# Jingliang-Duan/DSAC-v2

Measured on AMD Instinct MI355X. Metric: DSAC-T gradient steps/sec, batch=256 Humanoid (obs376/act17), higher is better.
Workload: dtype f32

## Files before the change

### dsac-v2_amd/csrc/dsact_api.hip

```cpp
#include <hip/hip_runtime.h>
#include <hip/hip_ext.h>
#include <dlfcn.h>
#include <chrono>
#include <stdarg.h>
#include <stdio.h>
#include <math.h>
#include <stdlib.h>
#include <string.h>

#include <algorithm>
#include <atomic>
#include <string>
#include <vector>

#include "../../include/dsact.h"
#include "dsact_kernels.h"
#include "dsact_chain.h"
#include "dsact_fat.h"
#include "dsact_act.h"
#include "dsact_act_batch.h"
#include "dsact_host_act.h"
#include "dsact_conv.h"

#define DSACT_KERNEL(group, ...) extern template __global__ void __VA_ARGS__;
// ... 194 lines not shown
  int debug_withhold = 0;
  unsigned long long* act_out_host = nullptr; unsigned long long* act_out_dev = nullptr;
  unsigned long long* act_h = nullptr;
  int act_call = 0;
  double act_launch_us = 0.0, act_wait_us = 0.0;
  bool env_no_fast_act = false;
  bool host_act = true;
  float* pol_host = nullptr;
  hipEvent_t pol_ev = nullptr;
  bool pol_pending = false;
  unsigned long long pol_epoch = 1;
  unsigned long long pol_copied = 0;
  float* act_buf = nullptr;
  hostact::Pool* act_pool = nullptr;
  std::vector<int> act_pin;
  int act_cpu = -1;
  unsigned act_repins = 0;
  int act_threads = 0;
  float act_scale_h[32] = {0}, act_center_h[32] = {0};
  float act_lo_h[32] = {0}, act_hi_h[32] = {0};
  double act_host_us = 0.0, act_copy_wait_us = 0.0;
  float* ab_stage = nullptr; float* ab_in = nullptr; float* ab_h[2] = {nullptr, nullptr};
  float* ab_out_host = nullptr; float* ab_out_dev = nullptr;
  unsigned long long ab_calls = 0;
  unsigned long long ab_mode_calls = 0;
  uint64_t act_seed = 0;
  unsigned long long act_dev_calls = 0;
  unsigned long long ring_commit_rows = 0;
  unsigned long long* digest_dev = nullptr;
  unsigned long long act_dev_syncs = 0;
  int* ev_ep = nullptr; double* ev_acc = nullptr; int* ev_len = nullptr;
  double* ev_returns = nullptr; int* ev_lengths = nullptr;
  int* ev_remaining = nullptr;
  int* ev_remaining_host = nullptr;
  int ev_cap_n = 0, ev_cap_e = 0;
  int ev_n = 0, ev_e = 0;
  unsigned long long act_mode_dev_calls = 0;
  unsigned long long eval_commit_calls = 0, eval_polls = 0;
  unsigned char* tk_dev = nullptr; unsigned char* tk_host = nullptr;
  int tk_cap = 0, tk_n = 0;
  unsigned long long track_commit_calls = 0, track_reads = 0;
  int mode_host_rows = kModeHostRows;
  unsigned long long act_host_calls = 0, act_copies = 0;
  bool beh_held = false;
  float* beh_dev = nullptr;
  hipEvent_t beh_ev = nullptr;
  hipStream_t act_stream = nullptr;
  float* beh_host = nullptr;
  hipEvent_t beh_host_ev = nullptr;
  bool beh_host_pending = false;
  bool beh_host_ok = false;
  bool beh_live_copy = false;
  unsigned long long beh_holds = 0, beh_acts = 0;
  bool fwd_merge = false;
  bool pi_merge = false;
  float* zobs[4];
  float* dAq[4];
  bool twin = false;
  float* X0t_net[3] = {nullptr, nullptr, nullptr};
  float* dz0row[3] = {nullptr, nullptr, nullptr};
  float* twin_part[8];
  bool twin_par = false;
  bool env_twin_seq = false;
  bool twin_merged = false;
  PipeFwd* d_fwdt[2] = {nullptr, nullptr};
  PipeFwd* fwdt_host[2] = {nullptr, nullptr};
  float* doutT[3];
  int dw2_off[4] = {0, 0, 0, 0};
  int dw2_mid = 0;
  int n_heads_parts = 0;
  static constexpr int kPipePhases = 4;
  char* pipe_ws = nullptr;
  unsigned long long* pipe_hand[2] = {nullptr, nullptr};
  int* bqt_cnt = nullptr;
  int* bqt_tab = nullptr; int bqt_tab_blocks = 0;
  bool env_no_bqt = false;
  unsigned long long* bqp_pairs[2] = {nullptr, nullptr};
  bool env_no_bqp = false;
  struct GraphSet {
    hipGraph_t graph = nullptr; hipGraphExec_t exec = nullptr;
    hipGraph_t pgraph[kPipePhases] = {nullptr, nullptr, nullptr, nullptr};
    hipGraphExec_t pexec[kPipePhases] = {nullptr, nullptr, nullptr, nullptr};
    PipeFwd* pargs[kPipePhases] = {nullptr, nullptr, nullptr, nullptr};
    bool pipe = false;
    bool merged = false;
    bool noise_table = false;
    int steps = 0; uint32_t flags = 0;
    bool present() const { return exec != nullptr || pipe; }
  };
  GraphSet active;
  std::vector<GraphSet> graph_cache;
  bool env_no_pipe_defer = false;
  std::string env_pipe_map;
  void* comm = nullptr;
  int comm_rank = 0, comm_world = 1;
  bool use_std_sums = false;
  bool auto_std_sums = false;
  float* std_sums_own = nullptr;
};

extern "C" {
static int build_graph(dsact_handle* h, int steps_per_graph, uint32_t flags, bool noise_table, bool keep_cache);
}

namespace {


struct NcclUid { char internal[128]; };
struct RcclApi {
  void* lib = nullptr;
  int (*GetUniqueId)(NcclUid*) = nullptr;
  int (*CommInitRank)(void**, int, NcclUid, int) = nullptr;
  int (*AllReduce)(const void*, void*, size_t, int, int, void*, hipStream_t) = nullptr;
  int (*CommDestroy)(void*) = nullptr;
  const char* (*GetErrorString)(int) = nullptr;
};
RcclApi g_rccl;
constexpr int kNcclFloat = 7, kNcclSum = 0, kNcclAvg = 4;

const char* rccl_load(const char* path) {
  if (g_rccl.lib) return nullptr;
  const char* cand[3] = {path && path[0] ? path : "librccl.so", "librccl.so.1", "/opt/rocm/lib/librccl.so"};
  void* lib = nullptr;
  for (int i = 0; i < 3 && !lib; ++i) lib = dlopen(cand[i], RTLD_NOW | RTLD_GLOBAL);
  if (!lib) return "librccl.so not found";
  g_rccl.GetUniqueId = (int (*)(NcclUid*))dlsym(lib, "ncclGetUniqueId");
  g_rccl.CommInitRank = (int (*)(void**, int, NcclUid, int))dlsym(lib, "ncclCommInitRank");
  g_rccl.AllReduce = (int (*)(const void*, void*, size_t, int, int, void*, hipStream_t))dlsym(lib, "ncclAllReduce");
  g_rccl.CommDestroy = (int (*)(void*))dlsym(lib, "ncclCommDestroy");
  g_rccl.GetErrorString = (const char* (*)(int))dlsym(lib, "ncclGetErrorString");
  if (!g_rccl.GetUniqueId || !g_rccl.CommInitRank || !g_rccl.AllReduce || !g_rccl.CommDestroy) return "librccl.so lacks the nccl* entry points";
  g_rccl.lib = lib;
  return nullptr;
}
const char* rccl_err(int rc) { return g_rccl.GetErrorString ? g_rccl.GetErrorString(rc) : "rccl error"; }

int fail(dsact_handle* h, int code, const char* fmt, ...) {
  if (h) {
    va_list ap;
    va_start(ap, fmt);
    vsnprintf(h->err, sizeof(h->err), fmt, ap);
    va_end(ap);
  }
  return code;
}

#define HIPCHK(h, call)                                                                          \
  do {                                                                                           \
    hipError_t e_ = (call);                                                                      \
    if (e_ != hipSuccess) return fail(h, DSACT_E_HIP, "%s failed: %s (%s:%d)", #call, hipGetErrorString(e_), __FILE__, __LINE__); \
  } while (0)

void build_net(NetDesc& d, int in0, const int* hidden, int L, int n_out, int nblk, int n_conv, const ConvGeom* cg) {
  d.n_lin = L + 1;
  d.nblk = nblk;
  d.n_conv = n_conv;
  size_t off = 0;
  for (int j = 0; j < n_conv; ++j) {
    d.cw_off[j] = off; off += (size_t)cg[j].Cout * cg[j].K;
    d.cb_off[j] = off; off += cg[j].Cout;
  }
  int in = in0;
  for (int l = 0; l <= L; ++l) {
    const int out = l < L ? nblk * hidden[l] : n_out;
    d.in[l] = in; d.out[l] = out;
    d.w_off[l] = off;
    off += (nblk == 2 && l > 0 && l < L) ? (size_t)2 * (out / 2) * (in / 2) : (size_t)in * out;
    d.b_off[l] = off; off += out;
    in = out;
  }
  d.count = off;
}

int net_act(const dsact_handle* h, int net);
// ... 2227 lines not shown
    HeadsBwdArgs a;
    a.dZ1[0] = h->dZ[kDzSlot[C_Q1P]][0]; a.dZ1[1] = h->dZ[kDzSlot[C_Q2P]][0];
    a.W1aT[0] = h->W1aT[0]; a.W1aT[1] = h->W1aT[1]; a.W0 = h->wq[0];
    a.logits_pi = h->logits_pi; a.eps_new = h->eps_new; a.log_alpha = h->online + h->n_online - 1;
    a.Wout_pi = net_params(h, N_POL) + h->pd.w_off[Lp];
    a.G_pi = h->Gb[C_PI][Lp - 1]; a.dZ_pi = h->dZ[kDzSlot[C_PI]][Lp - 1];
    a.dout_pi = h->dout_pi; a.d_new_act = h->d_new_act;
    a.WL = h->wp[Lp - 1]; a.B = B; a.O = h->F; a.A = A;
    a.inv_B = 1.0f / (float)B; a.auto_alpha = h->cfg.auto_alpha; a.alpha_fixed = h->cfg.alpha_fixed;
    a.act_scale = h->act_scale; a.lo_ls = h->cfg.min_log_std; a.hi_ls = h->cfg.max_log_std;
    a.part_loss = h->part_loss; a.n_part = B; a.target_entropy = -(float)A;
    a.grad_log_alpha = h->grads + h->n_online - 1;
    a.pi_out_act = h->cfg.policy_out_act; a.pi_out_n = h->cfg.policy_std_param ? A : 2 * A;
    a.pi_dact = h->pi_dact;
    a.timeline = tl_for(h, "heads_bwd");
    a.n_row_blocks = (B + 3) / 4;
    a.extra = h->d_tiles; a.n_extra = 0;
    a.fo = fused_opt(h, fused);
    if (ride_hb > 0) { a.extra = h->d_tiles + h->dw_off[0]; a.n_extra = ride_hb; }
    const size_t hb_lds = a.n_extra ? tile_lds_bytes(dw_k(h)) : 0;
#define CALL_HBWD(N) TRY(launch(h, "heads_bwd", k_heads_bwd<N>, dim3(a.n_row_blocks + a.n_extra), dim3(kThreads), hb_lds, a))
    NCH_DISPATCH(a.WL, CALL_HBWD);
  }
  const size_t np = h->bwdpi.size();
  if (phase == PH_DP_ACTOR) {
    for (size_t i = 0; i < np; ++i) TRY(run_stage(h, h->bwdpi[i]));
    if (h->cnn) TRY(run_stage(h, h->dfeat_pi));
    TRY(run_dw(h, h->dw_off[2], h->dw_off[3], false, false));
    if (h->cnn) TRY(enqueue_conv_backward(h, 1, false, h->nq));
    TRY(sum_parts(h, (size_t)h->nq * h->n_q, h->n_online - 1));
    return DSACT_OK;
  }
  {
    int x = h->dw_off[0] + ride_hb;
    for (size_t i = 0; i < np; ++i) {
      const int left = ride_end - x;
      const int take = i + 1 == np ? left : left / (int)(np - i);
      TRY(run_stage(h, h->bwdpi[i], x, x + take, fused));
      x += take;
    }
    if (np == 0 && ride_hb) {  }
  }
  if (h->cnn) TRY(run_stage(h, h->dfeat_pi));
  if (h->dw_chunks == 1) {
    TRY(run_dw(h, np ? ride_end : h->dw_off[0] + ride_hb, h->dw_off[3], fused, fused));
    if (h->cnn) TRY(enqueue_conv_backward(h, h->nq + 1, fused));
  } else {
    TRY(run_dw(h, np ? ride_end : h->dw_off[0] + ride_hb, h->dw_off[3], false, false));
    if (h->cnn) TRY(enqueue_conv_backward(h, h->nq + 1, false));
    if (fused) TRY(enqueue_adam(h, true));
    else TRY(sum_parts(h, 0, h->n_online - 1));
  }
  return DSACT_OK;
}

int enqueue_adam(dsact_handle* h, bool from_parts) {
  AdamArgs a;
  memset(&a, 0, sizeof(a));
  if (from_parts && h->dw_chunks > 1) {
    a.part = h->dw_parts; a.part_stride = (long long)h->dw_part_stride; a.n_part = h->dw_chunks;
    const int nets[3] = {N_Q1, N_Q2, N_POL};
    for (int i = 0; i < 3; ++i) {
      const long long b = (long long)(net_grads(h, nets[i]) - h->grads);
      a.direct_lo[i] = b; a.direct_hi[i] = b + (long long)net_desc(h, nets[i]).w_off[0];
    }
  }
  a.p = h->online; a.tgt = h->target; a.m = h->adam_m; a.v = h->adam_v; a.g = h->grads;
  a.n_q2 = (long long)(h->nq * h->n_q); a.n_online3 = (long long)(h->nq * h->n_q + h->n_pi); a.n_total = (long long)h->n_online;
  a.st = h->st;
  a.b1w = (float)(1.0 - h->cfg.adam_beta1);
  a.beta2 = (float)h->cfg.adam_beta2;
  a.b2w = (float)(1.0 - h->cfg.adam_beta2);
  a.eps = h->cfg.adam_eps;
  const double polyak = 1.0 - h->cfg.tau;
  a.polyak = (float)polyak;
  a.one_minus_polyak = (float)(1.0 - polyak);
  a.auto_alpha = h->cfg.auto_alpha;
  a.commit_ms = h->have_local_tail ? 1 : 0;
  h->have_local_tail = false;
  const int blocks = (int)((h->n_online + kThreads * 8 - 1) / (kThreads * 8));
  return launch(h, "adam_polyak", k_adam, dim3(blocks), dim3(kThreads), 0, a);
}

static void destroy_graph_set(dsact_handle::GraphSet& g) {
  if (g.exec) hipGraphExecDestroy(g.exec);
  if (g.graph) hipGraphDestroy(g.graph);
  for (int p = 0; p < dsact_handle::kPipePhases; ++p) {
    if (g.pexec[p]) hipGraphExecDestroy(g.pexec[p]);
    if (g.pgraph[p]) hipGraphDestroy(g.pgraph[p]);
    if (g.pargs[p]) hipFree(g.pargs[p]);
  }
  g = dsact_handle::GraphSet();
}
static void stash_graph(dsact_handle* h) {
  if (!h->active.present()) return;
  h->graph_cache.push_back(h->active);
  h->active = dsact_handle::GraphSet();
}
static bool activate_graph(dsact_handle* h, int steps, uint32_t flags, bool noise_table) {
  for (size_t i = 0; i < h->graph_cache.size(); ++i) {
    const dsact_handle::GraphSet& g = h->graph_cache[i];
    if (g.steps != steps || g.flags != flags || g.noise_table != noise_table) continue;
    h->active = g;
    h->graph_cache.erase(h->graph_cache.begin() + (long)i);
    return true;
  }
  return false;
}
static void drop_active_graph(dsact_handle* h) { destroy_graph_set(h->active); }
void drop_graphs(dsact_handle* h) {
  destroy_graph_set(h->active);
  for (auto& g : h->graph_cache) destroy_graph_set(g);
  h->graph_cache.clear();
}
bool have_graph(const dsact_handle* h) { return h->active.present(); }
bool any_graph(const dsact_handle* h) { return have_graph(h) || !h->graph_cache.empty(); }

int check_handoff(dsact_handle* h) {
  volatile int* const w_upd = (volatile int*)h->handoff_host;
  volatile int* const w_act = w_upd ? w_upd + 1 : nullptr;
  if (!h->handoff_host || h->in_handoff || !(*w_upd | *w_act)) return DSACT_OK;
  h->in_handoff = true;
  const hipError_t e_dev = hipSetDevice(h->device);
  const hipError_t e_sync = hipStreamSynchronize(h->stream);
  const int upd = *w_upd;
  *w_upd = 0; *w_act = 0;
  if (!upd) {
    h->in_handoff = false;
    h->handoff_failures += 1;
    return fail(h, DSACT_E_HIP, "the acting forward's layer hand-over timed out (a wave waited > 0.1 s for its input): this "
                                "call's action is invalid; parameters and optimiser state are untouched%s%s",
                e_sync != hipSuccess ? "; HIP also reported: " : "", e_sync != hipSuccess ? hipGetErrorString(e_sync) : "");
  }
  const bool had_graph = have_graph(h);
  const int steps = had_graph ? h->active.steps : h->want_graph_steps;
  const uint32_t gflags = had_graph ? h->active.flags : h->want_graph_flags;
  const bool noise_tab = h->active.noise_table;
  h->fwd_merge = false;
  h->pi_merge = false;
  h->handoff_failures += 1;
  drop_graphs(h);
  int twin_rc = DSACT_OK;
  if (h->twin_par) {
    h->env_twin_seq = true;
    h->debug_withhold = 0;
    twin_rc = build_twin_fwd(h);
  }
  hipError_t e_set = hipSuccess;
  if (h->chain_flags) e_set = hipMemset(h->chain_flags, 0, kChainFlagInts * sizeof(int));
  h->flags_dirty = false;
  int rebuilt = DSACT_E_STATE;
  const bool wanted = had_graph || steps > 0;
  if (wanted && twin_rc == DSACT_OK) {
    h->state_invalid = false;
    rebuilt = build_graph(h, steps, gflags, noise_tab, false);
  }
  h->want_graph_steps = (wanted && rebuilt != DSACT_OK) ? steps : 0;
  h->want_graph_flags = gflags;
  h->in_handoff = false;
  h->state_invalid = true;
  const hipError_t e_hip = e_dev != hipSuccess ? e_dev : e_sync != hipSuccess ? e_sync : e_set;
  return fail(h, DSACT_E_HIP,
              "an in-launch hand-over timed out: a workgroup waited > 0.1 s for its producers' ready flags, so every result "
              "since the last successful call is invalid -- parameters, optimiser moments and targets included: restore them, "
              "then acknowledge with dsact_set_state(adam_steps, mean_std), dsact_debug_set(\"ack_state\") or dsact_bind_arenas "
              "(update entry points fail until then). Merged launches are now disabled for this handle%s%s%s",
              wanted ? (rebuilt == DSACT_OK ? "; the graph was captured again without them" : "; re-capturing the graph failed (it is built again by the next replay)")
                     : "",
              e_hip != hipSuccess ? "; HIP also reported: " : "", e_hip != hipSuccess ? hipGetErrorString(e_hip) : "");
}

static int ensure_wanted_graph(dsact_handle* h) {
  if (have_graph(h) || h->want_graph_steps <= 0) return DSACT_OK;
  const int steps = h->want_graph_steps;
  h->want_graph_steps = 0;
  return dsact_graph_build(h, steps, h->want_graph_flags);
}

bool has_ring(const dsact_handle* h) { return h->rb_act != nullptr; }

int check_codes(dsact_handle* h) {
  if (!h->miss_host || !*(volatile int*)h->miss_host) return DSACT_OK;
  if (!h->miss_seen) {
    HIPCHK(h, hipSetDevice(h->device));
    HIPCHK(h, hipStreamSynchronize(h->stream));
    HIPCHK(h, hipMemcpy(&h->miss_rec, h->code_miss, sizeof(CodeMiss), hipMemcpyDeviceToHost));
    h->miss_seen = true;
  }
  uint32_t bits = h->miss_rec.bits;
  float v;
  memcpy(&v, &bits, 4);
  return fail(h, DSACT_E_INVALID, "hip_obs_codebook: %llu observation value(s) written to the coded ring are not in the codebook; "
              "first recorded: %.9g (bits 0x%08x) at ring row %lld -- the ring holds wrong codes for them",
              h->miss_rec.count, (double)v, bits, h->miss_rec.row);
}

static int check_usable(dsact_handle* h) {
  if (!h) return DSACT_E_INVALID;
  TRY(check_handoff(h));
  TRY(check_codes(h));
  if (h->state_invalid)
    return fail(h, DSACT_E_STATE, "device state is invalid after a hand-over timeout: restore parameters / optimiser state, then "
                                  "call dsact_set_state or dsact_bind_arenas");
  return DSACT_OK;
}
// ... 63 lines not shown
  if (cfg->act_dist != 0 && cfg->act_dist != 1) return fail(h, DSACT_E_INVALID, "act_dist must be 0 (TanhGaussDistribution) or 1 (GaussDistribution)");
  if (cfg->policy_std_param != 0 && cfg->policy_std_param != 1) return fail(h, DSACT_E_INVALID, "policy_std_param must be 0 (mlp_shared) or 1 (parameter)");
  if (cfg->policy_std_param && (cfg->conv_type != DSACT_CONV_NONE || cfg->algo != 0))
    return fail(h, DSACT_E_INVALID, "policy_std_type 'parameter' is built for DSAC_V2 with MLP nets");
  if (cfg->policy_twin != 0 && cfg->policy_twin != 1) return fail(h, DSACT_E_INVALID, "policy_twin must be 0 or 1 (policy_std_type mlp_separated)");
  if (cfg->policy_twin && (cfg->conv_type != DSACT_CONV_NONE || cfg->algo != 0 || cfg->policy_std_param))
    return fail(h, DSACT_E_INVALID, "policy_std_type 'mlp_separated' is built for DSAC_V2 with MLP nets (and excludes 'parameter')");
  for (int oa : {cfg->value_out_act, cfg->policy_out_act})
    if (oa != 0 && (oa < ACT_RELU || oa > ACT_TANH) && oa != OUT_ACT_GELU)
      return fail(h, DSACT_E_INVALID, "output activation must be 0 (linear), 1..5 (relu, elu, selu, sigmoid, tanh) or 6 (gelu)");
  if ((cfg->value_out_act || cfg->policy_out_act) && (cfg->conv_type != DSACT_CONV_NONE || cfg->algo != 0))
    return fail(h, DSACT_E_INVALID, "output activations other than linear are built for DSAC_V2 with MLP nets (tile-stage kernels)");
  if (h->cfg.global_batch < h->cfg.batch) h->cfg.global_batch = h->cfg.batch;
  HIPCHK(h, hipSetDevice(device));
  h->O = cfg->obs_dim; h->A = cfg->act_dim; h->L = cfg->n_hidden; h->B = cfg->batch;
  h->F = h->O;
  h->Brows = h->B > kActRows ? h->B : kActRows;
  int nblk = 1;
  if (cfg->conv_type != DSACT_CONV_NONE) {
    static const int k1[] = {8, 4, 3}, c1[] = {32, 64, 64}, s1[] = {4, 2, 1};
    static const int k2[] = {4, 3, 3, 3, 3, 3}, c2[] = {8, 16, 32, 64, 128, 256}, s2[] = {2, 2, 2, 2, 1, 1};
    if (cfg->conv_type != DSACT_CONV_TYPE_1 && cfg->conv_type != DSACT_CONV_TYPE_2) return fail(h, DSACT_E_INVALID, "conv_type must be 0, 1 (type_1) or 2 (type_2)");
    const bool t1 = cfg->conv_type == DSACT_CONV_TYPE_1;
    const int* ks = t1 ? k1 : k2; const int* cs = t1 ? c1 : c2; const int* ss = t1 ? s1 : s2;
    h->n_conv = t1 ? 3 : 6;
    if (cfg->img_c < 1 || cfg->img_h < 1 || cfg->img_w < 1 || (long long)cfg->img_c * cfg->img_h * cfg->img_w != cfg->obs_dim)
      return fail(h, DSACT_E_INVALID, "obs_dim must equal img_c*img_h*img_w for CNN nets");
    if (cfg->obs_dim % 4) return fail(h, DSACT_E_INVALID, "img_c*img_h*img_w must be a multiple of 4");
    int C = cfg->img_c, H = cfg->img_h, W = cfg->img_w;
    for (int j = 0; j < h->n_conv; ++j) {
      ConvGeom& g = h->cg[j];
      g.H = H; g.W = W; g.Cin = C; g.KS = ks[j]; g.stride = ss[j]; g.Cout = cs[j];
      g.OH = (H - g.KS) / g.stride + 1; g.OW = (W - g.KS) / g.stride + 1;
      if (H < g.KS || W < g.KS || g.OH < 1 || g.OW < 1) return fail(h, DSACT_E_INVALID, "image %dx%d too small for conv layer %d", cfg->img_h, cfg->img_w, j);
      g.K = g.KS * g.KS * g.Cin; g.KWC = g.KS * g.Cin; g.rowskip = g.W * g.Cin - g.KWC;
      g.inv_kwc = 1.0f / (float)g.KWC;
      if (g.KWC % 4) return fail(h, DSACT_E_INVALID, "kernel_width*channels of conv layer %d must be a multiple of 4 (got %d)", j, g.KWC);
      C = g.Cout; H = g.OH; W = g.OW;
    }
    h->cnn = true;
    h->cP = H * W;
    h->F = C * H * W;
    nblk = 2;
  }
  int pol_hidden[DSACT_MAX_HIDDEN_LAYERS] = {0};
  bool unequal = false;
  h->Lq = cfg->n_hidden;
  h->Lp = cfg->policy_n_hidden > 0 ? cfg->policy_n_hidden : cfg->n_hidden;
  if (h->Lp > DSACT_MAX_HIDDEN_LAYERS) return fail(h, DSACT_E_INVALID, "policy_n_hidden must be 0 (= n_hidden) or 1..%d", DSACT_MAX_HIDDEN_LAYERS);
  if (h->Lp != h->Lq && cfg->conv_type != DSACT_CONV_NONE) return fail(h, DSACT_E_INVALID, "policy_n_hidden: the CNN nets' MLP widths are fixed by conv_type");
  unequal = h->Lp != h->Lq;
  h->L = h->Lp > h->Lq ? h->Lp : h->Lq;
  for (int l = 0; l < h->Lp; ++l) {
    pol_hidden[l] = cfg->policy_hidden[l] > 0 ? cfg->policy_hidden[l] : (l < h->Lq ? cfg->hidden[l] : 0);
    if (pol_hidden[l] < 1 || pol_hidden[l] > kMaxWidth) return fail(h, DSACT_E_INVALID, "policy hidden width of layer %d must be 1..%d", l, kMaxWidth);
    unequal = unequal || l >= h->Lq || pol_hidden[l] != cfg->hidden[l];
  }
  if (unequal && (cfg->conv_type != DSACT_CONV_NONE || cfg->algo != 0))
    return fail(h, DSACT_E_INVALID, "value_hidden_sizes != policy_hidden_sizes is built for DSAC_V2 with MLP nets (tile-stage kernels)");
  const int nblk_pol = cfg->policy_twin ? 2 : nblk;
  h->unequal_widths = unequal || nblk_pol != nblk;
  for (int l = 0; l < h->L; ++l) {
    h->wq[l] = l < h->Lq ? nblk * cfg->hidden[l] : 0; h->wp[l] = l < h->Lp ? nblk_pol * pol_hidden[l] : 0;
    h->w[l] = h->wq[l] > h->wp[l] ? h->wq[l] : h->wp[l];
  }
  for (int l = 0; l < h->L; ++l)
    if (h->w[l] > kMaxWidth) return fail(h, DSACT_E_INVALID, "activation row width %d exceeds %d", h->w[l], kMaxWidth);
  h->ldx = (h->F + h->A + 3) & ~3;
  h->use_w1p = (size_t)4 * nblk * cfg->hidden[0] * h->ldx <= ((size_t)4 << 20);
  build_net(h->qd, h->F + h->A, cfg->hidden, h->Lq, 2, nblk, h->n_conv, h->cg);
  build_net(h->pd, h->F, pol_hidden, h->Lp, 2 * h->A, nblk_pol, h->n_conv, h->cg);
  h->n_q = h->qd.count; h->n_pi = h->pd.count;
  if (cfg->algo != DSACT_ALGO_DSAC_V2 && cfg->algo != DSACT_ALGO_DSAC_V1) return fail(h, DSACT_E_INVALID, "algo must be 0 (DSAC_V2) or 1 (DSAC_V1)");
  h->nq = cfg->algo == DSACT_ALGO_DSAC_V1 ? 1 : 2;
  h->n_online = h->nq * h->n_q + h->n_pi + 1;
  h->n_target = h->nq * h->n_q + h->n_pi;
  h->n_heads_wg = (h->B + 3) / 4;
  h->n_loss_wg = (h->B + 3) / 4;
  h->loss_rows = 4;
  h->auto_std_sums = h->B > 1024;
  if (const char* v = getenv("DSACT_TIMELINE_STAGE")) h->env_timeline_stage = v;
  { int v = 0; if (hipDeviceGetAttribute(&v, hipDeviceAttributeMultiprocessorCount, h->device) == hipSuccess && v > 0) h->n_cu = v; (void)hipGetLastError(); }
  h->env_no_pipe_defer = getenv("DSACT_NO_PIPE_DEFER") != nullptr;
  h->env_no_bqt = getenv("DSACT_NO_BQT_MERGE") != nullptr;
  h->env_no_bqp = getenv("DSACT_NO_BQP_MERGE") != nullptr;
  if (const char* v = getenv("DSACT_PIPE_MAP")) h->env_pipe_map = v;
  h->env_no_dcol_ident = getenv("DSACT_NO_DCOL_IDENT") != nullptr;
  h->env_no_fat_stage = getenv("DSACT_NO_FAT_STAGE") != nullptr;
  h->dw_chunks = (h->B > 448 && h->B % 256 == 0) ? h->B / 256 : 1;
  h->dw_part_stride = (h->n_online + 2 + 63) & ~(size_t)63;
  {
    const int R = 4 * h->cRG;
    bool ok = h->B % R == 0 && h->B % 16 == 0 && (h->B <= 256 || h->B % 256 == 0) &&
              getenv("DSACT_NO_CHAIN") == nullptr && !(h->nq == 1 && getenv("DSACT_NO_CHAIN_V1") != nullptr) &&
              !(h->cnn && (getenv("DSACT_NO_CHAIN_CNN") != nullptr || h->B > 1024));
    ok = ok && h->L <= kChMaxL;
    ok = ok && !h->unequal_widths;
    ok = ok && cfg->value_out_act != OUT_ACT_GELU && cfg->policy_out_act != OUT_ACT_GELU;
    for (int l = 0; l < h->L; ++l) ok = ok && cfg->hidden[l] == cfg->hidden[0];
    const int W0 = cfg->hidden[0];
    ok = ok && (W0 == 64 || W0 == 128 || W0 == 256);
    h->s_obs = roundup((h->F + 3) / 4, kPD);
    h->s_act = roundup((h->A + 3) / 4, kPD);
    h->SoT = roundup((2 * h->A + 3) / 4, kPD);
    ok = ok && (size_t)chain_lds(4 * (h->s_obs + h->s_act), W0, R).total * sizeof(float) <= 150 * 1024;
    h->chain_ok = ok;
    h->twin = ok && h->cnn;
    h->env_twin_seq = getenv("DSACT_TWIN_SEQ") != nullptr;
    if (ok) {
      const int per = (h->B > 1024 && h->B % 1024 == 0) ? 1024 : 256;
      h->dw_chunks = h->B > 1024 ? h->B / per : 1;
    }
    h->cW = W0; h->cNT = W0 / 64; h->n_slices = h->B / R;
    h->rg4_ok = ok && h->B % 16 == 0 &&
                (size_t)chain_lds(4 * (h->s_obs + h->s_act), W0, 16).total * sizeof(float) <= 150 * 1024;
    h->c_obs = (h->F + 15) / 16; h->c_act = (h->A + 15) / 16; h->c_out = (2 * h->A + 15) / 16;
    {
      const char* fm = getenv("DSACT_FAT_MIN");
      const int fat_min = fm ? atoi(fm) : 1024;
      h->fat = ok && !h->cnn && h->nq == 2 && h->B >= fat_min && h->B % 32 == 0 && (W0 == 128 || W0 == 256) &&
               cfg->value_out_act == 0 && cfg->policy_out_act == 0;
      h->fat_bwd = h->fat && h->B >= 4096;
      if (const char* v = getenv("DSACT_FAT_RT")) h->env_fat_rt = atoi(v) == 2 ? 2 : 1;
    }
    h->fwd_merge = ok && !h->cnn && h->B <= 256 && h->B / 4 <= kChainFlagSlices && chain_rg(h, 4) == 1 && getenv("DSACT_NO_FWD_MERGE") == nullptr;
    h->pi_merge = ok && !h->cnn && h->B <= 512 && !h->fat_bwd && getenv("DSACT_NO_PI_MERGE") == nullptr;
  }
  Carver c0;
  carve(h, c0, h->sets[0], SET_WS);
  h->ws_bytes = c0.off + 256;
  HIPCHK(h, hipMalloc(&h->ws, h->ws_bytes));
  HIPCHK(h, hipMemset(h->ws, 0, h->ws_bytes));
  Carver c1;
  c1.base = h->ws;
  carve(h, c1, h->sets[0], SET_WS);
  {
    DevState st0;
    memset(&st0, 0, sizeof(st0));
    st0.b1p_q = st0.b2p_q = st0.b1p_pi = st0.b2p_pi = st0.b1p_alpha = st0.b2p_alpha = 1.0;
    HIPCHK(h, hipMemcpy(h->st, &st0, sizeof(st0), hipMemcpyHostToDevice));
  }
  {
    std::vector<float> ones(h->B, 1.0f);
    HIPCHK(h, hipMemcpy(h->ones, ones.data(), h->B * sizeof(float), hipMemcpyHostToDevice));
  }
  if (h->cnn) {
    for (int j = 0; j < h->n_conv; ++j) {
      const ConvGeom& g = h->cg[j];
      if ((size_t)h->Brows * g.H * g.W * g.Cin > 2147483647ull || (size_t)h->Brows * g.OH * g.OW >= (1u << 24))
        return fail(h, DSACT_E_INVALID, "batch x image too large for the conv index arithmetic (layer %d)", j);
    }
    std::vector<int> iota(h->Brows);
    for (int i = 0; i < h->Brows; ++i) iota[i] = i;
    HIPCHK(h, hipMemcpy(h->idx_iota, iota.data(), iota.size() * sizeof(int), hipMemcpyHostToDevice));
  }
  HIPCHK(h, hipStreamCreateWithFlags(&h->stream, hipStreamNonBlocking));
  h->own_stream = true;
  {
    const int max_lds = (int)tile_lds_bytes(BK * kMaxPrefetchTiles);
    HIPCHK(h, hipFuncSetAttribute((const void*)k_stage<false, false, EPI_GELU>, hipFuncAttributeMaxDynamicSharedMemorySize, max_lds));
    HIPCHK(h, hipFuncSetAttribute((const void*)k_stage<false, false, EPI_GELU, 4>, hipFuncAttributeMaxDynamicSharedMemorySize, max_lds));
    HIPCHK(h, hipFuncSetAttribute((const void*)k_stage<false, false, EPI_GELU, 2>, hipFuncAttributeMaxDynamicSharedMemorySize, max_lds));
    HIPCHK(h, hipFuncSetAttribute((const void*)k_stage<false, true, EPI_MULG, 4>, hipFuncAttributeMaxDynamicSharedMemorySize, max_lds));
    HIPCHK(h, hipFuncSetAttribute((const void*)k_stage<false, true, EPI_MULG, 2>, hipFuncAttributeMaxDynamicSharedMemorySize, max_lds));
    HIPCHK(h, hipFuncSetAttribute((const void*)k_stage<false, true, EPI_MULG>, hipFuncAttributeMaxDynamicSharedMemorySize, max_lds));
    HIPCHK(h, hipFuncSetAttribute((const void*)k_stage_table, hipFuncAttributeMaxDynamicSharedMemorySize, max_lds));
// ... 82 lines not shown
    const size_t la = (size_t)chain_lds(4 * (h->s_obs + h->s_act), h->cW, 4 * chain_rg(h, 6)).total * sizeof(float);
    const void* fn = h->cNT == 1 ? (const void*)k_chain_fwd2<1> : h->cNT == 2 ? (const void*)k_chain_fwd2<2> : (const void*)k_chain_fwd2<4>;
    if (hipOccupancyMaxActiveBlocksPerMultiprocessor(&per_cu, fn, 64 * h->cNT, la) != hipSuccess || per_cu < 2) h->fwd_merge = false;
    (void)hipGetLastError();
  }
  for (int i = 0; i < 8; ++i) {
    HIPCHK(h, hipHostMalloc((void**)&h->h_idx[i], (size_t)h->B * sizeof(int), hipHostMallocDefault));
    HIPCHK(h, hipEventCreateWithFlags(&h->h_idx_ev[i], hipEventDisableTiming));
  }
  return DSACT_OK;
}

int dsact_destroy(dsact_handle* h) {
  if (!h) return DSACT_E_INVALID;
  hipSetDevice(h->device);
  if (h->stream) hipStreamSynchronize(h->stream);
  drop_graphs(h);
  if (h->comm && g_rccl.CommDestroy) { g_rccl.CommDestroy(h->comm); h->comm = nullptr; }
  for (auto& r : h->prof) { hipEventDestroy(r.e0); hipEventDestroy(r.e1); }
  if (h->tev0) { hipEventDestroy(h->tev0); hipEventDestroy(h->tev1); }
  if (h->uev0) { hipEventDestroy(h->uev0); hipEventDestroy(h->uev1); }
  for (int i = 0; i < 8; ++i) {
    if (h->h_idx[i]) hipHostFree(h->h_idx[i]);
    if (h->h_idx_ev[i]) hipEventDestroy(h->h_idx_ev[i]);
  }
  if (h->handoff_host) hipHostFree(h->handoff_host);
  if (h->act_h) hipFree(h->act_h);
  if (h->ab_stage) hipHostFree(h->ab_stage);
  if (h->ab_out_host) hipHostFree(h->ab_out_host);
  if (h->ab_in) hipFree(h->ab_in);
  for (void* p : {(void*)h->ev_ep, (void*)h->ev_acc, (void*)h->ev_len, (void*)h->ev_returns, (void*)h->ev_lengths, (void*)h->ev_remaining})
    if (p) hipFree(p);
  if (h->ev_remaining_host) hipHostFree(h->ev_remaining_host);
  if (h->tk_dev) hipFree(h->tk_dev);
  if (h->digest_dev) hipFree(h->digest_dev);
  if (h->tk_host) hipHostFree(h->tk_host);
  for (int i = 0; i < 2; ++i) if (h->ab_h[i]) hipFree(h->ab_h[i]);
  if (h->pol_host) hipHostFree(h->pol_host);
  if (h->pol_ev) hipEventDestroy(h->pol_ev);
  if (h->act_stream) { hipStreamSynchronize(h->act_stream); hipStreamDestroy(h->act_stream); }
  if (h->beh_dev) hipFree(h->beh_dev);
  if (h->beh_host) hipHostFree(h->beh_host);
  if (h->beh_ev) hipEventDestroy(h->beh_ev);
  if (h->beh_host_ev) hipEventDestroy(h->beh_host_ev);
  free(h->act_buf);
  delete h->act_pool;
  for (int k : {0, (int)dsact_handle::kAltSet}) if (h->sets[k].d_tiles) hipFree(h->sets[k].d_tiles);
  if (h->alt_ws) hipFree(h->alt_ws);
  if (h->pipe_ws) hipFree(h->pipe_ws);
  if (h->bqt_cnt) hipFree(h->bqt_cnt);
  if (h->bqt_tab) hipFree(h->bqt_tab);
  for (int i = 0; i < 2; ++i) if (h->bqp_pairs[i]) hipFree(h->bqp_pairs[i]);
  if (h->pk_ws) hipFree(h->pk_ws);
  for (int i = 0; i < 2; ++i) { if (h->d_fwdt[i]) hipFree(h->d_fwdt[i]); delete h->fwdt_host[i]; }
  if (h->d_mir) hipFree(h->d_mir);
  if (h->d_apjobs) hipFree(h->d_apjobs);
  if (h->d_pack) hipFree(h->d_pack);
  if (h->idx_table) hipFree(h->idx_table);
  if (h->noise_table) hipFree(h->noise_table);
  for (int i = 0; i < 4; ++i) {
    if (h->grp_pin[i]) hipHostFree(h->grp_pin[i]);
    if (h->grp_ev[i]) hipEventDestroy(h->grp_ev[i]);
  }
  if (h->stage_dev) hipFree(h->stage_dev);
  for (int i = 0; i < 2; ++i) {
    if (h->stage_pin[i]) hipHostFree(h->stage_pin[i]);
    if (h->stage_ev[i]) hipEventDestroy(h->stage_ev[i]);
  }
  if (h->logp_stage) hipFree(h->logp_stage);
  if (h->stage_img) hipFree(h->stage_img);
  for (float* p : {h->rb_obs, h->rb_obs2, h->rb_act, h->rb_rew, h->rb_done, h->rb_logp})
    if (p) hipFree(p);
  if (h->rb_code) hipFree(h->rb_code);
  if (h->code_book) hipFree(h->code_book);
  if (h->code_miss) hipFree(h->code_miss);
  if (h->miss_host) hipHostFree(h->miss_host);
  if (h->ws) hipFree(h->ws);
  if (h->own_stream && h->stream) hipStreamDestroy(h->stream);
  delete h;
  return DSACT_OK;
}

int dsact_set_stream(dsact_handle* h, void* s) {
  if (!h) return DSACT_E_INVALID;
  HIPCHK(h, hipSetDevice(h->device));
  if (any_graph(h)) return fail(h, DSACT_E_STATE, "cannot change stream after dsact_graph_build");
  if (h->stream) HIPCHK(h, hipStreamSynchronize(h->stream));
  if (h->own_stream && h->stream) { hipStreamDestroy(h->stream); h->stream = nullptr; }
  if (s) { h->stream = (hipStream_t)s; h->own_stream = false; }
  else { HIPCHK(h, hipStreamCreateWithFlags(&h->stream, hipStreamNonBlocking)); h->own_stream = true; }
  return DSACT_OK;
}

void* dsact_get_stream(const dsact_handle* h) { return h ? (void*)h->stream : nullptr; }

int dsact_sync(dsact_handle* h) {
  if (!h) return DSACT_E_INVALID;
  HIPCHK(h, hipSetDevice(h->device));
  HIPCHK(h, hipStreamSynchronize(h->stream));
  return check_handoff(h);
}

size_t dsact_online_count(const dsact_handle* h) { return h ? h->n_online : 0; }
size_t dsact_target_count(const dsact_handle* h) { return h ? h->n_target : 0; }
size_t dsact_q_count(const dsact_handle* h) { return h ? h->n_q : 0; }
size_t dsact_pi_count(const dsact_handle* h) { return h ? h->n_pi : 0; }

int dsact_bind_arenas(dsact_handle* h, float* online, float* target, float* adam_m, float* adam_v, float* grads) {
  if (!h) return DSACT_E_INVALID;
  if (!online || !target || !adam_m || !adam_v || !grads) return fail(h, DSACT_E_INVALID, "null arena pointer");
  HIPCHK(h, hipSetDevice(h->device));
  if (any_graph(h)) return fail(h, DSACT_E_STATE, "cannot rebind arenas after dsact_graph_build");
  h->online = online; h->target = target; h->adam_m = adam_m; h->adam_v = adam_v; h->grads = grads;
  TRY(build_chain(h));
  TRY(build_pack_jobs(h));
  if (h->chain_ok && !h->twin) TRY(build_adam_pack_jobs(h));
  TRY(build_tasks(h));
  if (h->twin) TRY(build_twin_fwd(h));
  if (h->chain_ok) (void)dw2_args(h, false);
  if (!h->cnn) {
    TRY(alloc_alt_set(h));
    select_set(h, dsact_handle::kAltSet);
    int rc = build_tasks(h);
    select_set(h, 0);
    TRY(rc);
  }
  h->state_invalid = false;
  h->pol_epoch++;
  return DSACT_OK;
}

int dsact_set_action_limits(dsact_handle* h, const float* high, const float* low) {
  if (!h || !high || !low) return DSACT_E_INVALID;
  HIPCHK(h, hipSetDevice(h->device));
  std::vector<float> s(h->A), c(h->A);
  for (int j = 0; j < h->A; ++j) {
    if (!(high[j] > low[j])) return fail(h, DSACT_E_INVALID, "action_high_limit must exceed action_low_limit");
    s[j] = (high[j] - low[j]) / 2;
    c[j] = (high[j] + low[j]) / 2;
    if (h->cfg.act_dist == 1) { s[j] = 0.0f; c[j] = 0.0f; }
  }
  HIPCHK(h, hipStreamSynchronize(h->stream));
  HIPCHK(h, hipMemcpy(h->act_scale, s.data(), h->A * sizeof(float), hipMemcpyHostToDevice));
  HIPCHK(h, hipMemcpy(h->act_center, c.data(), h->A * sizeof(float), hipMemcpyHostToDevice));
  HIPCHK(h, hipMemcpy(h->act_lo, low, h->A * sizeof(float), hipMemcpyHostToDevice));
  HIPCHK(h, hipMemcpy(h->act_hi, high, h->A * sizeof(float), hipMemcpyHostToDevice));
  for (int j = 0; j < h->A && j < 32; ++j) {
    h->act_scale_h[j] = s[j]; h->act_center_h[j] = c[j];
    h->act_lo_h[j] = low[j]; h->act_hi_h[j] = high[j];
  }
  h->limits_set = true;
  return DSACT_OK;
}

int dsact_get_state(dsact_handle* h, int32_t adam_steps[3], float mean_std[2]) {
  if (!h) return DSACT_E_INVALID;
  HIPCHK(h, hipSetDevice(h->device));
  HIPCHK(h, hipStreamSynchronize(h->stream));
  DevState st;
  HIPCHK(h, hipMemcpy(&st, h->st, sizeof(st), hipMemcpyDeviceToHost));
  TRY(check_handoff(h));
  if (adam_steps) { adam_steps[0] = st.t_q; adam_steps[1] = st.t_pi; adam_steps[2] = st.t_alpha; }
  if (mean_std) { mean_std[0] = st.ms_init ? st.ms1 : -1.0f; mean_std[1] = st.ms_init ? st.ms2 : -1.0f; }
  return DSACT_OK;
}

int dsact_set_state(dsact_handle* h, const int32_t adam_steps[3], const float mean_std[2]) {
  if (!h) return DSACT_E_INVALID;
  HIPCHK(h, hipSetDevice(h->device));
  HIPCHK(h, hipStreamSynchronize(h->stream));
  DevState st;
  HIPCHK(h, hipMemcpy(&st, h->st, sizeof(st), hipMemcpyDeviceToHost));
  if (adam_steps) {
    st.t_q = adam_steps[0]; st.t_pi = adam_steps[1]; st.t_alpha = adam_steps[2];
    const double b1 = h->cfg.adam_beta1, b2 = h->cfg.adam_beta2;
    st.b1p_q = pow(b1, st.t_q); st.b2p_q = pow(b2, st.t_q);
    st.b1p_pi = pow(b1, st.t_pi); st.b2p_pi = pow(b2, st.t_pi);
    st.b1p_alpha = pow(b1, st.t_alpha); st.b2p_alpha = pow(b2, st.t_alpha);
  }
  if (mean_std) {
    st.ms_init = (mean_std[0] >= 0.0f && mean_std[1] >= 0.0f) ? 1 : 0;
    st.ms1 = mean_std[0]; st.ms2 = mean_std[1];
  }
  HIPCHK(h, hipMemcpy(h->st, &st, sizeof(st), hipMemcpyHostToDevice));
  if (adam_steps && mean_std) h->state_invalid = false;
  return DSACT_OK;
}

int dsact_set_hyper(dsact_handle* h, int32_t which, double value) {
  if (!h) return DSACT_E_INVALID;
  if (!(value == value)) return fail(h, DSACT_E_INVALID, "hyper-parameter is NaN");
  switch (which) {
    case DSACT_HYPER_GAMMA: h->cfg.gamma = value; break;
    case DSACT_HYPER_TAU:
      if (value < 0.0 || value > 1.0) return fail(h, DSACT_E_INVALID, "tau outside [0, 1]");
      h->cfg.tau = value; break;
    case DSACT_HYPER_TAU_B:
      if (value < 0.0 || value > 1.0) return fail(h, DSACT_E_INVALID, "tau_b outside [0, 1]");
      h->cfg.tau_b = value; break;
    case DSACT_HYPER_AUTO_ALPHA: h->cfg.auto_alpha = value != 0.0 ? 1 : 0; break;
    case DSACT_HYPER_ALPHA: h->cfg.alpha_fixed = value; break;
    case DSACT_HYPER_DELAY_UPDATE:
      if (value < 1.0 || value != (double)(int32_t)value) return fail(h, DSACT_E_INVALID, "delay_update must be a positive integer");
      h->cfg.delay_update = (int32_t)value; break;
    case DSACT_HYPER_TD_BOUND:
      if (h->cfg.algo != 1) return fail(h, DSACT_E_INVALID, "TD_bound is a DSAC_V1 parameter");
      h->cfg.td_bound = value; break;
    case DSACT_HYPER_V1_BOUND:
      if (h->cfg.algo != 1) return fail(h, DSACT_E_INVALID, "bound is a DSAC_V1 parameter");
      h->cfg.v1_unbounded = value != 0.0 ? 0 : 1; break;
    default: return fail(h, DSACT_E_INVALID, "unknown hyper-parameter %d", (int)which);
  }
  HIPCHK(h, hipSetDevice(h->device));
  HIPCHK(h, hipStreamSynchronize(h->stream));
  drop_graphs(h);
  return DSACT_OK;
}

namespace {
int create_scalar_columns(dsact_handle* h, int64_t capacity) {
  const size_t N = (size_t)capacity;
  HIPCHK(h, hipMalloc(&h->rb_act, N * h->A * sizeof(float)));
  HIPCHK(h, hipMalloc(&h->rb_rew, N * sizeof(float)));
  HIPCHK(h, hipMalloc(&h->rb_done, N * sizeof(float)));
  HIPCHK(h, hipMalloc(&h->rb_logp, N * sizeof(float)));
  HIPCHK(h, hipMemsetAsync(h->rb_act, 0, N * h->A * sizeof(float), h->stream));
  HIPCHK(h, hipMemsetAsync(h->rb_rew, 0, N * sizeof(float), h->stream));
  HIPCHK(h, hipMemsetAsync(h->rb_done, 0, N * sizeof(float), h->stream));
  HIPCHK(h, hipMemsetAsync(h->rb_logp, 0, N * sizeof(float), h->stream));
  h->cap = capacity; h->ptr = 0; h->size = 0;
  return DSACT_OK;
}
}

int dsact_buffer_create(dsact_handle* h, int64_t capacity) {
  if (!h || capacity < 1) return DSACT_E_INVALID;
  if (capacity > 2147483647LL) return fail(h, DSACT_E_INVALID, "capacity must fit int32 (device indices)");
  HIPCHK(h, hipSetDevice(h->device));
  if (has_ring(h)) return fail(h, DSACT_E_STATE, "buffer already created");
  const size_t N = (size_t)capacity;
  HIPCHK(h, hipMalloc(&h->rb_obs, N * h->O * sizeof(float)));
  HIPCHK(h, hipMalloc(&h->rb_obs2, N * h->O * sizeof(float)));
  HIPCHK(h, hipMemsetAsync(h->rb_obs, 0, N * h->O * sizeof(float), h->stream));
  HIPCHK(h, hipMemsetAsync(h->rb_obs2, 0, N * h->O * sizeof(float), h->stream));
  return create_scalar_columns(h, capacity);
}

int dsact_buffer_create_coded(dsact_handle* h, int64_t capacity, const float* codebook, int32_t n_codes) {
  if (!h || capacity < 1 || !codebook) return DSACT_E_INVALID;
  if (capacity > 2147483647LL) return fail(h, DSACT_E_INVALID, "capacity must fit int32 (device indices)");
  if (n_codes < 1 || n_codes > 256) return fail(h, DSACT_E_INVALID, "hip_obs_codebook: %d entries (1 .. 256)", (int)n_codes);
  for (int i = 0; i < n_codes; ++i) {
    if (!(codebook[i] == codebook[i])) return fail(h, DSACT_E_INVALID, "hip_obs_codebook: entry %d is NaN", i);
    if (i && !(codebook[i - 1] < codebook[i]))
      return fail(h, DSACT_E_INVALID, "hip_obs_codebook: entries %d, %d are not strictly ascending (%.9g, %.9g)", i - 1, i,
                  (double)codebook[i - 1], (double)codebook[i]);
  }
  if (!h->cnn) return fail(h, DSACT_E_INVALID, "hip_obs_codebook: codes are for image observations (C, H, W); this handle has flat ones");
  const int C = h->cfg.img_c, HW = h->cfg.img_h * h->cfg.img_w;
  if (HW % 16 || C > 16)
    return fail(h, DSACT_E_INVALID, "hip_obs_codebook: a coded ring needs H * W %% 16 == 0 and C <= 16 (got C %d, H * W %d)", C, HW);
  HIPCHK(h, hipSetDevice(h->device));
  if (has_ring(h)) return fail(h, DSACT_E_STATE, "buffer already created");
  const size_t N = (size_t)capacity, O = (size_t)h->O;
  HIPCHK(h, hipMalloc(&h->rb_code, 2 * N * O));
  HIPCHK(h, hipMemsetAsync(h->rb_code, 0, 2 * N * O, h->stream));
  float book[256] = {};
  memcpy(book, codebook, (size_t)n_codes * sizeof(float));
  HIPCHK(h, hipMalloc(&h->code_book, sizeof(book)));
  HIPCHK(h, hipMemcpy(h->code_book, book, sizeof(book), hipMemcpyHostToDevice));
  h->n_codes = n_codes;
  HIPCHK(h, hipMalloc(&h->code_miss, sizeof(CodeMiss)));
  HIPCHK(h, hipMemset(h->code_miss, 0, sizeof(CodeMiss)));
  HIPCHK(h, hipHostMalloc((void**)&h->miss_host, 64, hipHostMallocMapped | hipHostMallocCoherent));
  *(volatile int*)h->miss_host = 0;
  HIPCHK(h, hipHostGetDevicePointer((void**)&h->miss_dev, h->miss_host, 0));
  if (coded_gather_lds(C) > 64 * 1024)
    HIPCHK(h, hipFuncSetAttribute((const void*)k_gather_img_coded<0>, hipFuncAttributeMaxDynamicSharedMemorySize, (int)coded_gather_lds(C)));
  return create_scalar_columns(h, capacity);
}

int dsact_buffer_check(dsact_handle* h) {
  if (!h) return DSACT_E_INVALID;
  if (!has_ring(h)) return fail(h, DSACT_E_STATE, "buffer not created");
  HIPCHK(h, hipSetDevice(h->device));
  HIPCHK(h, hipStreamSynchronize(h->stream));
  return check_codes(h);
}

int64_t dsact_buffer_bytes(const dsact_handle* h) {
  if (!h) return -1;
  if (!has_ring(h)) return 0;
  const int64_t O = h->O, A = h->A;
  const int64_t obs_bytes = h->rb_code ? 2 * O : 4 * 2 * O;
  return h->cap * (obs_bytes + 4 * (A + 3));
}

int64_t dsact_buffer_size(const dsact_handle* h) { return h ? h->size : -1; }
int64_t dsact_buffer_ptr(const dsact_handle* h) { return h ? h->ptr : -1; }

namespace {
int enqueue_ring_encode(dsact_handle* h, const float* s_obs, const float* s_obs2, long long ptr, long long n) {
  CodedScatterArgs e;
  e.s_obs = s_obs; e.s_obs2 = s_obs2;
  e.code0 = h->rb_code; e.code1 = h->rb_code + (size_t)h->cap * h->O;
  e.book = h->code_book; e.n_codes = h->n_codes; e.miss = h->code_miss; e.miss_flag = h->miss_dev;
  e.ptr = ptr; e.cap = h->cap; e.n = (int)n; e.O = h->O;
  e.wide = (h->O % 4 == 0) && ((uintptr_t)s_obs % 16 == 0) && ((uintptr_t)s_obs2 % 16 == 0);
  const long long per_row = e.wide ? h->O / 4 : h->O;
  const unsigned gx = (unsigned)std::min<long long>((per_row + kThreads - 1) / kThreads, 64);
  const unsigned rows = (unsigned)(n < 65535 ? n : 65535);
  return launch(h, "ring_write_img_coded", k_ring_write_img_coded, dim3(gx, rows, 2), dim3(kThreads), 0, e);
}
}

int dsact_buffer_add(dsact_handle* h, int64_t n, const float* obs, const float* act, const float* rew,
                     const float* obs2, const float* done, const float* logp) {
  if (!h || n < 0 || !obs || !act || !rew || !obs2 || !done) return DSACT_E_INVALID;
  if (!has_ring(h)) return fail(h, DSACT_E_STATE, "buffer not created");
  TRY(check_codes(h));
  if (n == 0) return DSACT_OK;
  HIPCHK(h, hipSetDevice(h->device));
  const size_t O = h->O, A = h->A;
  const size_t row_f = 2 * O + A + 3;
  if ((size_t)n > h->stage_rows) {
    HIPCHK(h, hipStreamSynchronize(h->stream));
    if (h->stage_dev) hipFree(h->stage_dev);
    for (int i = 0; i < 2; ++i)
      if (h->stage_pin[i]) { hipHostFree(h->stage_pin[i]); h->stage_pin[i] = nullptr; }
    h->stage_rows = (size_t)n < 64 ? 64 : (size_t)n;
    HIPCHK(h, hipMalloc(&h->stage_dev, h->stage_rows * row_f * sizeof(float)));
    for (int i = 0; i < 2; ++i) {
      HIPCHK(h, hipHostMalloc((void**)&h->stage_pin[i], h->stage_rows * row_f * sizeof(float), hipHostMallocDefault));
      if (!h->stage_ev[i]) HIPCHK(h, hipEventCreateWithFlags(&h->stage_ev[i], hipEventDisableTiming));
    }
  }
  const int slot = (int)(h->stage_k++ & 1);
  HIPCHK(h, hipEventSynchronize(h->stage_ev[slot]));
  float* pin = h->stage_pin[slot];
  size_t off = 0;
  auto put = [&](const float* src, size_t count) {
    if (src) memcpy(pin + off, src, count * sizeof(float));
    off += count;
  };
  put(obs, (size_t)n * O); put(obs2, (size_t)n * O); put(act, (size_t)n * A); put(rew, (size_t)n); put(done, (size_t)n);
  put(logp, (size_t)n);
  const size_t R = (size_t)n;
  float* s_obs = h->stage_dev;
  float* s_obs2 = s_obs + R * O;
  float* s_act = s_obs2 + R * O;
  float* s_rew = s_act + R * A;
  float* s_done = s_rew + R;
  float* s_logp = s_done + R;
  HIPCHK(h, hipMemcpyAsync(h->stage_dev, pin, off * sizeof(float), hipMemcpyHostToDevice, h->stream));
  HIPCHK(h, hipEventRecord(h->stage_ev[slot], h->stream));
  long long first = 0, cnt = n;
  if (n > h->cap) { first = n - h->cap; cnt = h->cap; }
  ScatterArgs a;
  a.s_obs = s_obs + first * O; a.s_obs2 = s_obs2 + first * O; a.s_act = s_act + first * A;
  a.s_rew = s_rew + first; a.s_done = s_done + first; a.s_logp = logp ? s_logp + first : nullptr;
  a.rb_obs = h->rb_obs; a.rb_obs2 = h->rb_obs2; a.rb_act = h->rb_act; a.rb_rew = h->rb_rew; a.rb_done = h->rb_done; a.rb_logp = h->rb_logp;
  a.ptr = (h->ptr + first) % h->cap; a.cap = h->cap; a.n = (int)cnt; a.O = h->O; a.A = h->A;
  if (h->rb_code) {
    TRY(enqueue_ring_encode(h, a.s_obs, a.s_obs2, a.ptr, cnt));
    a.O = 0;
  } else if (h->cnn) {
    ImgScatterArgs w;
    w.s_obs = a.s_obs; w.s_obs2 = a.s_obs2; w.rb_obs = h->rb_obs; w.rb_obs2 = h->rb_obs2;
    w.ptr = a.ptr; w.cap = h->cap; w.n = (int)cnt; w.O = h->O;
    TRY(launch(h, "ring_write_img", k_ring_write_img, dim3(8, (unsigned)cnt), dim3(kThreads), 0, w));
    a.O = 0;
  }
  TRY(launch(h, "ring_write", k_ring_write, dim3((unsigned)((cnt + 3) / 4)), dim3(kThreads), 0, a));
  h->ptr = (h->ptr + n) % h->cap;
  h->size = h->size + n > h->cap ? h->cap : h->size + n;
  return DSACT_OK;
}

int dsact_buffer_fill_device(dsact_handle* h, int64_t row0, int64_t n, const float* obs, const float* act,
                             const float* rew, const float* obs2, const float* done) {
  if (!h || row0 < 0 || n < 0) return DSACT_E_INVALID;
  if (!has_ring(h)) return fail(h, DSACT_E_STATE, "buffer not created");
  if (row0 + n > h->cap) return fail(h, DSACT_E_INVALID, "fill exceeds capacity");
  TRY(check_codes(h));
  HIPCHK(h, hipSetDevice(h->device));
  const size_t O = h->O, A = h->A;
  if (h->rb_code) {
    if (n > 0) TRY(enqueue_ring_encode(h, obs, obs2, row0, n));
  } else {
    HIPCHK(h, hipMemcpyAsync(h->rb_obs + row0 * O, obs, n * O * sizeof(float), hipMemcpyDeviceToDevice, h->stream));
    HIPCHK(h, hipMemcpyAsync(h->rb_obs2 + row0 * O, obs2, n * O * sizeof(float), hipMemcpyDeviceToDevice, h->stream));
  }
  HIPCHK(h, hipMemcpyAsync(h->rb_act + row0 * A, act, n * A * sizeof(float), hipMemcpyDeviceToDevice, h->stream));
  HIPCHK(h, hipMemcpyAsync(h->rb_rew + row0, rew, n * sizeof(float), hipMemcpyDeviceToDevice, h->stream));
  HIPCHK(h, hipMemcpyAsync(h->rb_done + row0, done, n * sizeof(float), hipMemcpyDeviceToDevice, h->stream));
  HIPCHK(h, hipStreamSynchronize(h->stream));
  if (row0 + n > h->size) h->size = row0 + n;
  h->ptr = (row0 + n) % h->cap;
  return check_codes(h);
}

static bool on_handle_gpu(const dsact_handle* h, const void* p) {
  hipPointerAttribute_t at;
  if (hipPointerGetAttributes(&at, p) != hipSuccess) { (void)hipGetLastError(); return false; }
  return at.type == hipMemoryTypeDevice && at.device == h->device;
}
static int check_handoff_counted(dsact_handle* h) {
  const unsigned long long before = h->handoff_failures;
  const int rc = check_handoff(h);
  if (h->handoff_failures != before) h->act_dev_syncs++;
  return rc;
}

int dsact_buffer_add_device(dsact_handle* h, int64_t n, const float* obs, const float* act, const float* rew, const float* obs2,
                            const uint8_t* terminated, const uint8_t* truncated, const float* logp, double reward_scale) {
  if (!h || n < 0 || !obs || !act || !rew || !obs2 || !terminated || !truncated || !logp) return DSACT_E_INVALID;
  if (!has_ring(h)) return fail(h, DSACT_E_STATE, "buffer not created");
  if (h->rb_code) return fail(h, DSACT_E_INVALID, "dsact_buffer_add_device serves the fp32 MLP ring (coded rings: dsact_buffer_add)");
  if (h->cnn) return fail(h, DSACT_E_INVALID, "dsact_buffer_add_device serves the fp32 MLP ring (image rings: dsact_buffer_add)");
  if (n > h->cap) return fail(h, DSACT_E_INVALID, "dsact_buffer_add_device: n = %lld exceeds the capacity %lld", (long long)n, (long long)h->cap);
  if (n == 0) return DSACT_OK;
  HIPCHK(h, hipSetDevice(h->device));
  const void* ptrs[7] = {obs, act, rew, obs2, terminated, truncated, logp};
  for (const void* p : ptrs)
    if (!on_handle_gpu(h, p))
      return fail(h, DSACT_E_INVALID, "dsact_buffer_add_device takes device pointers on the handle's GPU (host rows: dsact_buffer_add)");
  TRY(check_handoff_counted(h));
  RingCommitArgs a;
  a.s_obs = obs; a.s_act = act; a.s_rew = rew; a.s_obs2 = obs2; a.s_term = terminated; a.s_trunc = truncated; a.s_logp = logp;
  a.rb_obs = h->rb_obs; a.rb_obs2 = h->rb_obs2; a.rb_act = h->rb_act; a.rb_rew = h->rb_rew; a.rb_done = h->rb_done; a.rb_logp = h->rb_logp;
  a.ptr = h->ptr; a.cap = h->cap; a.n = (int)n; a.O = h->O; a.A = h->A;
  a.wide = (h->O % 4 == 0) && ((uintptr_t)obs % 16 == 0) && ((uintptr_t)obs2 % 16 == 0) && ((uintptr_t)h->rb_obs % 16 == 0) &&
           ((uintptr_t)h->rb_obs2 % 16 == 0);
  a.reward_scale = (float)reward_scale;
  TRY(launch(h, "ring_commit", k_ring_commit, dim3((unsigned)((n + 3) / 4)), dim3(kThreads), 0, a));
  h->ptr = (h->ptr + n) % h->cap;
  h->size = h->size + n > h->cap ? h->cap : h->size + n;
  h->ring_commit_rows += (unsigned long long)n;
  return DSACT_OK;
}

namespace {
struct RingColumn { char* base; size_t row_bytes; };
void ring_columns(const dsact_handle* h, RingColumn c[6]) {
  const size_t O = (size_t)h->O, A = (size_t)h->A;
  if (h->rb_code) {
    c[0] = {(char*)h->rb_code, O};
    c[1] = {(char*)h->rb_code + (size_t)h->cap * O, O};
  } else {
    c[0] = {(char*)h->rb_obs, O * sizeof(float)};
    c[1] = {(char*)h->rb_obs2, O * sizeof(float)};
  }
  c[2] = {(char*)h->rb_act, A * sizeof(float)};
  c[3] = {(char*)h->rb_rew, sizeof(float)};
  c[4] = {(char*)h->rb_done, sizeof(float)};
  c[5] = {(char*)h->rb_logp, sizeof(float)};
}
int ring_entry(dsact_handle* h, const char* what) {
  if (!has_ring(h)) return fail(h, DSACT_E_STATE, "%s: buffer not created", what);
  hipStreamCaptureStatus cap = hipStreamCaptureStatusNone;
  HIPCHK(h, hipStreamIsCapturing(h->stream, &cap));
  if (cap != hipStreamCaptureStatusNone) return fail(h, DSACT_E_STATE, "%s under stream capture", what);
  return DSACT_OK;
}
int ring_drain(dsact_handle* h) {
  HIPCHK(h, hipSetDevice(h->device));
  TRY(check_handoff(h));
  HIPCHK(h, hipStreamSynchronize(h->stream));
  TRY(check_handoff(h));
  return check_codes(h);
}
}

int dsact_buffer_export(dsact_handle* h, int64_t row0, int64_t n, void* obs, void* obs2, float* act, float* rew, float* done,
                        float* logp) {
  if (!h) return DSACT_E_INVALID;
  TRY(ring_entry(h, "dsact_buffer_export"));
  if (row0 < 0 || n < 0 || row0 > h->size || n > h->size - row0)
    return fail(h, DSACT_E_INVALID, "dsact_buffer_export: rows [%lld, %lld + %lld) are not inside the %lld live rows", (long long)row0,
                (long long)row0, (long long)n, h->size);
  TRY(ring_drain(h));
  if (n == 0) return DSACT_OK;
  RingColumn c[6];
  ring_columns(h, c);
  void* dst[6] = {obs, obs2, act, rew, done, logp};
  for (int k = 0; k < 6; ++k)
    if (dst[k]) HIPCHK(h, hipMemcpy(dst[k], c[k].base + (size_t)row0 * c[k].row_bytes, (size_t)n * c[k].row_bytes, hipMemcpyDeviceToHost));
  return DSACT_OK;
}

int dsact_buffer_import(dsact_handle* h, int64_t row0, int64_t n, const void* obs, const void* obs2, const float* act,
                        const float* rew, const float* done, const float* logp) {
  if (!h) return DSACT_E_INVALID;
  TRY(ring_entry(h, "dsact_buffer_import"));
  if (!obs || !obs2 || !act || !rew || !done || !logp) return fail(h, DSACT_E_INVALID, "dsact_buffer_import: a source column is NULL");
  if (row0 < 0 || n < 0 || row0 > h->cap || n > h->cap - row0)
    return fail(h, DSACT_E_INVALID, "dsact_buffer_import: rows [%lld, %lld + %lld) are not inside the capacity %lld", (long long)row0,
                (long long)row0, (long long)n, h->cap);
  if (h->rb_code && h->n_codes < 256) {
    const size_t cnt = (size_t)n * (size_t)h->O;
    const unsigned char* src[2] = {(const unsigned char*)obs, (const unsigned char*)obs2};
    for (int w = 0; w < 2; ++w)
      for (size_t i = 0; i < cnt; ++i)
        if (src[w][i] >= h->n_codes)
          return fail(h, DSACT_E_INVALID, "dsact_buffer_import: %s code %d at row %lld, element %lld is not below the codebook's %d entries",
                      w ? "obs2" : "obs", (int)src[w][i], (long long)(row0 + (int64_t)(i / (size_t)h->O)), (long long)(i % (size_t)h->O), h->n_codes);
  }
  TRY(ring_drain(h));
  if (n == 0) return DSACT_OK;
  RingColumn c[6];
  ring_columns(h, c);
  const void* src[6] = {obs, obs2, act, rew, done, logp};
  for (int k = 0; k < 6; ++k)
    HIPCHK(h, hipMemcpy(c[k].base + (size_t)row0 * c[k].row_bytes, src[k], (size_t)n * c[k].row_bytes, hipMemcpyHostToDevice));
  return DSACT_OK;
}

int dsact_buffer_set_cursor(dsact_handle* h, int64_t size, int64_t ptr) {
  if (!h) return DSACT_E_INVALID;
  TRY(ring_entry(h, "dsact_buffer_set_cursor"));
  const bool ok = size >= 0 && size <= h->cap && (size < h->cap ? ptr == size % h->cap : (ptr >= 0 && ptr < h->cap));
  if (!ok)
    return fail(h, DSACT_E_INVALID, "dsact_buffer_set_cursor: (size %lld, ptr %lld) is no state a ring of %lld rows reaches", (long long)size,
                (long long)ptr, h->cap);
  TRY(ring_drain(h));
  h->size = size; h->ptr = ptr;
  return DSACT_OK;
}

int dsact_buffer_digest(dsact_handle* h, int64_t row0, int64_t n, uint64_t out[6]) {
  if (!h) return DSACT_E_INVALID;
  TRY(ring_entry(h, "dsact_buffer_digest"));
  if (!out) return fail(h, DSACT_E_INVALID, "dsact_buffer_digest: out is NULL");
  if (row0 < 0 || n < 0 || row0 > h->size || n > h->size - row0)
    return fail(h, DSACT_E_INVALID, "dsact_buffer_digest: rows [%lld, %lld + %lld) are not inside the %lld live rows", (long long)row0,
                (long long)row0, (long long)n, h->size);
  TRY(ring_drain(h));
  for (int k = 0; k < 6; ++k) out[k] = 0;
  if (n == 0) return DSACT_OK;
  if (!h->digest_dev) HIPCHK(h, hipMalloc(&h->digest_dev, 6 * sizeof(unsigned long long)));
  RingColumn c[6];
  ring_columns(h, c);
  RingDigestArgs a;
  unsigned long long most = 0;
  for (int k = 0; k < 6; ++k) {
    const int eb = (k < 2 && h->rb_code) ? 1 : 4;
    const unsigned long long w = (unsigned long long)(c[k].row_bytes / (size_t)eb);
    a.col[k].base = c[k].base;
    a.col[k].g0 = (unsigned long long)row0 * w;
    a.col[k].count = (unsigned long long)n * w;
    a.col[k].elem_bytes = eb;
    const unsigned long long loads = a.col[k].count / (eb == 4 ? 4u : 16u);
    if (loads > most) most = loads;
  }
  a.out = h->digest_dev;
  unsigned long long gx = (most + kThreads - 1) / kThreads;
  const unsigned long long gmax = (unsigned long long)(h->n_cu > 0 ? h->n_cu : 256) * 8;
  if (gx > gmax) gx = gmax;
  if (gx < 1) gx = 1;
  HIPCHK(h, hipMemsetAsync(h->digest_dev, 0, 6 * sizeof(unsigned long long), h->stream));
  TRY(launch(h, "ring_digest", k_ring_digest, dim3((unsigned)gx, 6), dim3(kThreads), 0, a));
  unsigned long long got[6];
  HIPCHK(h, hipMemcpyAsync(got, h->digest_dev, sizeof(got), hipMemcpyDeviceToHost, h->stream));
  HIPCHK(h, hipStreamSynchronize(h->stream));
  for (int k = 0; k < 6; ++k) out[k] = (uint64_t)got[k];
  return check_handoff(h);
}

int dsact_gather(dsact_handle* h, const int64_t* idx_host, int32_t batch) {
  if (!h) return DSACT_E_INVALID;
  if (!has_ring(h)) return fail(h, DSACT_E_STATE, "buffer not created");
  TRY(check_codes(h));
  if (batch != h->B) return fail(h, DSACT_E_INVALID, "batch %d != configured batch %d", batch, h->B);
  if (h->size == 0) return fail(h, DSACT_E_STATE, "buffer empty");
  HIPCHK(h, hipSetDevice(h->device));
  if (!idx_host) {
    if (h->idx_seed == 0 || !h->idx_table) return fail(h, DSACT_E_STATE, "idx_host == NULL gathers the row dsact_draw_indices drew: call dsact_set_index_rng and dsact_draw_indices first");
    HIPCHK(h, hipMemcpyAsync(h->idx_eager, h->idx_table, batch * sizeof(int), hipMemcpyDeviceToDevice, h->stream));
  } else {
    const int slot = h->h_idx_slot;
    h->h_idx_slot = (slot + 1) & 7;
    HIPCHK(h, hipEventSynchronize(h->h_idx_ev[slot]));
    for (int i = 0; i < batch; ++i) {
      if (idx_host[i] < 0 || idx_host[i] >= h->size) return fail(h, DSACT_E_INVALID, "index %lld out of range [0,%lld)", (long long)idx_host[i], h->size);
      h->h_idx[slot][i] = (int)idx_host[i];
    }
    HIPCHK(h, hipMemcpyAsync(h->idx_eager, h->h_idx[slot], batch * sizeof(int), hipMemcpyHostToDevice, h->stream));
    HIPCHK(h, hipEventRecord(h->h_idx_ev[slot], h->stream));
  }
  if (h->cnn) {
    TRY(enqueue_gather_ring_img(h, h->idx_eager, 1, 0));
    h->have_batch = true;
    return DSACT_OK;
  }
  GatherArgs a;
  memset(&a, 0, sizeof(a));
  a.rb_obs = h->rb_obs; a.rb_obs2 = h->rb_obs2; a.rb_act = h->rb_act; a.rb_rew = h->rb_rew; a.rb_done = h->rb_done;
  a.idx_table = h->idx_eager; a.idx_rows = 1; a.use_dev = 0; a.host_it = 0; a.host_row = 0;
  a.X0 = h->X0; a.XP = h->XP; a.X2 = h->X2; a.rew = h->rew; a.done = h->done;
  a.B = h->B; a.O = h->O; a.A = h->A; a.ldx = h->ldx; a.st = h->st; a.bookkeeping = 0; a.advance_counters = 0;
  a.hp = step_hyper(h); a.nz = noise_args(h); a.nz.seed = 0;
  a.n_gather_blocks = (h->B + 3) / 4;
  a.rp = repack_args(h, 0);
  TRY(launch(h, "gather", k_gather, dim3((h->B + 3) / 4), dim3(kThreads), 0, a));
  h->have_batch = true;
  return DSACT_OK;
}

int dsact_read_batch(dsact_handle* h, float* obs, float* act, float* rew, float* obs2, float* done, float* logp) {
  if (!h) return DSACT_E_INVALID;
  if (!h->have_batch) return fail(h, DSACT_E_STATE, "no minibatch staged");
  HIPCHK(h, hipSetDevice(h->device));
  HIPCHK(h, hipStreamSynchronize(h->stream));
  const size_t B = h->B, O = h->O, A = h->A, ld = h->ldx;
  if (h->cnn) {
    const size_t C = h->cfg.img_c, HW = (size_t)h->cfg.img_h * h->cfg.img_w;
    std::vector<float> tmp(B * O);
    for (int w = 0; w < 2; ++w) {
      float* dst = w == 0 ? obs : obs2;
      if (!dst) continue;
      HIPCHK(h, hipMemcpy(tmp.data(), h->img[w], B * O * 4, hipMemcpyDeviceToHost));
      for (size_t b = 0; b < B; ++b)
        for (size_t p = 0; p < HW; ++p)
          for (size_t c = 0; c < C; ++c) dst[b * O + c * HW + p] = tmp[b * O + p * C + c];
    }
    if (act) HIPCHK(h, hipMemcpy2D(act, A * 4, h->Xc[C_Q1C] + h->F, ld * 4, A * 4, B, hipMemcpyDeviceToHost));
  } else {
    if (obs) HIPCHK(h, hipMemcpy2D(obs, O * 4, h->X0, ld * 4, O * 4, B, hipMemcpyDeviceToHost));
    if (obs2) HIPCHK(h, hipMemcpy2D(obs2, O * 4, h->X2, ld * 4, O * 4, B, hipMemcpyDeviceToHost));
    if (act) HIPCHK(h, hipMemcpy2D(act, A * 4, h->X0 + O, ld * 4, A * 4, B, hipMemcpyDeviceToHost));
  }
  if (rew) HIPCHK(h, hipMemcpy(rew, h->rew, B * 4, hipMemcpyDeviceToHost));
  if (done) HIPCHK(h, hipMemcpy(done, h->done, B * 4, hipMemcpyDeviceToHost));
  if (logp) {
    if (!h->rb_logp) return fail(h, DSACT_E_STATE, "buffer not created");
    if (!h->logp_stage) HIPCHK(h, hipMalloc(&h->logp_stage, B * sizeof(float)));
    TakeArgs t;
    t.src = h->rb_logp; t.idx = h->idx_eager; t.dst = h->logp_stage; t.n = (int)B;
    TRY(launch(h, "take_logp", k_take, dim3((unsigned)((B + kThreads - 1) / kThreads)), dim3(kThreads), 0, t));
    HIPCHK(h, hipMemcpyAsync(logp, h->logp_stage, B * sizeof(float), hipMemcpyDeviceToHost, h->stream));
    HIPCHK(h, hipStreamSynchronize(h->stream));
  }
  return DSACT_OK;
}

int dsact_load_batch(dsact_handle* h, const float* obs, const float* act, const float* rew, const float* obs2, const float* done) {
  if (!h || !obs || !act || !rew || !obs2 || !done) return DSACT_E_INVALID;
  HIPCHK(h, hipSetDevice(h->device));
  const size_t B = h->B, O = h->O, A = h->A, ld = h->ldx;
  hipStream_t s = h->stream;
  if (h->cnn) {
    const size_t R = h->Brows;
    if (!h->stage_img) HIPCHK(h, hipMalloc(&h->stage_img, 2 * R * O * sizeof(float)));
    HIPCHK(h, hipMemcpyAsync(h->stage_img, obs, B * O * 4, hipMemcpyDefault, s));
    HIPCHK(h, hipMemcpyAsync(h->stage_img + R * O, obs2, B * O * 4, hipMemcpyDefault, s));
    TRY(enqueue_gather_img(h, h->stage_img, h->stage_img + R * O, h->idx_iota, 1, 0, false, h->img[0], h->img[1], h->B));
    HIPCHK(h, hipMemcpy2DAsync(h->Xc[C_Q1C] + h->F, ld * 4, act, A * 4, A * 4, B, hipMemcpyDefault, s));
    HIPCHK(h, hipMemcpy2DAsync(h->Xc[C_Q2C] + h->F, ld * 4, act, A * 4, A * 4, B, hipMemcpyDefault, s));
    HIPCHK(h, hipMemcpyAsync(h->rew, rew, B * 4, hipMemcpyDefault, s));
    HIPCHK(h, hipMemcpyAsync(h->done, done, B * 4, hipMemcpyDefault, s));
    HIPCHK(h, hipStreamSynchronize(s));
    h->have_batch = true;
    return DSACT_OK;
  }
  HIPCHK(h, hipMemcpy2DAsync(h->X0, ld * 4, obs, O * 4, O * 4, B, hipMemcpyDefault, s));
  HIPCHK(h, hipMemcpy2DAsync(h->XP, ld * 4, h->X0, ld * 4, O * 4, B, hipMemcpyDeviceToDevice, s));
  HIPCHK(h, hipMemcpy2DAsync(h->X2, ld * 4, obs2, O * 4, O * 4, B, hipMemcpyDefault, s));
  HIPCHK(h, hipMemcpy2DAsync(h->X0 + O, ld * 4, act, A * 4, A * 4, B, hipMemcpyDefault, s));
  HIPCHK(h, hipMemcpyAsync(h->rew, rew, B * 4, hipMemcpyDefault, s));
  HIPCHK(h, hipMemcpyAsync(h->done, done, B * 4, hipMemcpyDefault, s));
  HIPCHK(h, hipStreamSynchronize(s));
  h->have_batch = true;
  return DSACT_OK;
}

int dsact_upload_index_table(dsact_handle* h, const int64_t* idx_host, int32_t rows) {
  if (!h || !idx_host || rows < 1) return DSACT_E_INVALID;
  if (!has_ring(h)) return fail(h, DSACT_E_STATE, "buffer not created");
  HIPCHK(h, hipSetDevice(h->device));
  HIPCHK(h, hipStreamSynchronize(h->stream));
  const size_t n = (size_t)rows * h->B;
  std::vector<int> tmp(n);
  for (size_t i = 0; i < n; ++i) {
    if (idx_host[i] < 0 || idx_host[i] >= h->size) return fail(h, DSACT_E_INVALID, "index out of range");
    tmp[i] = (int)idx_host[i];
  }
  if (any_graph(h) && rows != h->idx_rows) return fail(h, DSACT_E_STATE, "index table shape is baked into the captured graph");
  if (!h->idx_table || rows != h->idx_rows) {
    drop_graphs(h);
    if (h->idx_table) hipFree(h->idx_table);
    if (h->noise_table) { hipFree(h->noise_table); h->noise_table = nullptr; }
    HIPCHK(h, hipMalloc(&h->idx_table, n * sizeof(int)));
    h->idx_rows = rows;
  }
  HIPCHK(h, hipMemcpy(h->idx_table, tmp.data(), n * sizeof(int), hipMemcpyHostToDevice));
  return DSACT_OK;
}

int dsact_set_noise(dsact_handle* h, const float* eps_new, const float* eps_2, const float* z5, const float* z6) {
  if (!h || !eps_new || !eps_2 || !z5 || !z6) return DSACT_E_INVALID;
  HIPCHK(h, hipSetDevice(h->device));
  const size_t B = h->B, A = h->A;
  HIPCHK(h, hipMemcpyAsync(h->eps_new, eps_new, B * A * 4, hipMemcpyHostToDevice, h->stream));
  HIPCHK(h, hipMemcpyAsync(h->eps_2, eps_2, B * A * 4, hipMemcpyHostToDevice, h->stream));
  HIPCHK(h, hipMemcpyAsync(h->z5, z5, B * 4, hipMemcpyHostToDevice, h->stream));
  HIPCHK(h, hipMemcpyAsync(h->z6, z6, B * 4, hipMemcpyHostToDevice, h->stream));
  HIPCHK(h, hipStreamSynchronize(h->stream));
  h->rng_seed = 0;
  return DSACT_OK;
}

int dsact_set_device_rng(dsact_handle* h, uint64_t seed) {
  if (!h) return DSACT_E_INVALID;
  if (any_graph(h)) return fail(h, DSACT_E_STATE, "rng mode is baked into the captured graph");
  h->rng_seed = seed;
  return DSACT_OK;
}

int dsact_set_index_rng(dsact_handle* h, uint64_t seed) {
  if (!h) return DSACT_E_INVALID;
  h->idx_seed = seed;
  return DSACT_OK;
}

int dsact_draw_indices(dsact_handle* h, int64_t first_iteration, int32_t n) {
  if (!h || n < 1) return DSACT_E_INVALID;
  if (!has_ring(h)) return fail(h, DSACT_E_STATE, "buffer not created");
  if (h->idx_seed == 0) return fail(h, DSACT_E_STATE, "no index seed (dsact_set_index_rng)");
  if (h->size == 0) return fail(h, DSACT_E_STATE, "buffer empty");
  TRY(check_codes(h));
  HIPCHK(h, hipSetDevice(h->device));
  TRY(ensure_group_tables(h, n));
  return enqueue_draw_indices(h, first_iteration, n);
}

int dsact_read_indices(dsact_handle* h, int64_t* out, int32_t rows) {
  if (!h || !out || rows < 1) return DSACT_E_INVALID;
  if (!h->idx_table || rows > h->idx_rows) return fail(h, DSACT_E_STATE, "the index table holds %d rows, %d asked for", h->idx_table ? h->idx_rows : 0, rows);
  HIPCHK(h, hipSetDevice(h->device));
  const size_t n = (size_t)rows * h->B;
  std::vector<int> tmp(n);
  HIPCHK(h, hipMemcpyAsync(tmp.data(), h->idx_table, n * sizeof(int), hipMemcpyDeviceToHost, h->stream));
  HIPCHK(h, hipStreamSynchronize(h->stream));
  for (size_t i = 0; i < n; ++i) out[i] = tmp[i];
  return DSACT_OK;
}

static int enqueue_policy_copy(dsact_handle* h) {
  HIPCHK(h, hipMemcpyAsync(h->pol_host, net_params(h, N_POL), (size_t)h->n_pi * sizeof(float), hipMemcpyDeviceToHost, h->stream));
  HIPCHK(h, hipEventRecord(h->pol_ev, h->stream));
  h->pol_pending = true;
  h->pol_copied = h->pol_epoch;
  h->act_copies++;
  return DSACT_OK;
}
static int policy_moved(dsact_handle* h) {
  h->pol_epoch++;
  if (h->pol_host && h->host_act && (!h->beh_held || h->beh_live_copy)) return enqueue_policy_copy(h);
  return DSACT_OK;
}
static bool act_fast_ok(const dsact_handle* h);
static bool act_host_ok(const dsact_handle* h) { return h->host_act && act_fast_ok(h); }
static int wait_snapshot(dsact_handle* h, hipEvent_t ev, std::chrono::steady_clock::time_point t0) {
  hipError_t q = hipErrorNotReady;
  while ((q = hipEventQuery(ev)) == hipErrorNotReady) {
    if (std::chrono::steady_clock::now() - t0 > std::chrono::milliseconds(5)) break;
  }
  if (q != hipSuccess) HIPCHK(h, hipEventSynchronize(ev));
  TRY(check_handoff(h));
  h->act_copy_wait_us = std::chrono::duration<double, std::micro>(std::chrono::steady_clock::now() - t0).count();
  return DSACT_OK;
}
static int act_forward_host(dsact_handle* h, const float* obs_host, const float* eps, float* out, float* logp, bool behaviour = false) {
  TRY(check_handoff(h));
  const auto t0 = std::chrono::steady_clock::now();
  if (!h->act_buf) {
    h->act_buf = (float*)malloc((size_t)(2 * (kMaxWidth + 64) + 128) * sizeof(float));
    if (!h->act_buf) return fail(h, DSACT_E_HIP, "out of host memory");
  }
  const float* P = h->beh_host;
  if (behaviour) {
    if (h->beh_host_pending) {
      TRY(wait_snapshot(h, h->beh_host_ev, t0));
      h->beh_host_pending = false;
    }
  } else {
    if (!h->pol_host) {
      HIPCHK(h, hipHostMalloc((void**)&h->pol_host, ((size_t)h->n_pi + 64) * sizeof(float), hipHostMallocDefault));
      HIPCHK(h, hipEventCreateWithFlags(&h->pol_ev, hipEventDisableTiming));
    }
    if (h->pol_copied != h->pol_epoch) TRY(enqueue_policy_copy(h));
    if (h->pol_pending) {
      TRY(wait_snapshot(h, h->pol_ev, t0));
      h->pol_pending = false;
    }
    P = h->pol_host;
  }
  hostact::Layer ly[kActMaxLayers];
  for (int l = 0; l <= h->Lp; ++l) {
    ly[l].W = P + h->pd.w_off[l]; ly[l].b = P + h->pd.b_off[l];
    ly[l].K = h->pd.in[l]; ly[l].N = h->pd.out[l]; ly[l].half = 0;
    if (h->pd.nblk == 2 && l > 0 && l < h->Lp) { ly[l].K = h->pd.in[l] / 2; ly[l].half = h->pd.out[l] / 2; }
  }
  float* b0 = h->act_buf; float* b1 = b0 + kMaxWidth + 64; float* raw = b1 + kMaxWidth + 64;
  if (h->act_threads == 0) {
    const char* ev = getenv("DSACT_HOST_ACT_THREADS");
    int t = 1;
    std::vector<int> pin;
#if defined(__linux__)
    const int cpu = sched_getcpu();
    if (cpu >= 0) pin = hostact::llc_sibling_cores(cpu);
#endif
    if (ev) t = atoi(ev);
    else if ((int)std::thread::hardware_concurrency() >= 16 && h->pd.out[0] >= 128 && pin.size() >= 3) t = 4;
    t = t < 1 ? 1 : (t > 16 ? 16 : t);
    if (t > 1) {
      h->act_pool = new hostact::Pool(t, pin);
      if (!ev && h->act_pool->pinned() < t - 1) { delete h->act_pool; h->act_pool = nullptr; t = 1; }
    }
    h->act_threads = t;
#if defined(__linux__)
    h->act_pin = pin; h->act_cpu = cpu;
#endif
  }
#if defined(__linux__)
  if (h->act_pool && h->act_pool->pinned() > 0 && (h->act_host_calls & 255) == 255) {
    const int cpu = sched_getcpu();
    if (cpu >= 0 && cpu != h->act_cpu) {
      h->act_cpu = cpu;
      const std::vector<int> pin = hostact::llc_sibling_cores(cpu);
      const size_t need = (size_t)h->act_threads - 1;
      bool same = pin.size() >= need && h->act_pin.size() >= need;
      for (size_t i = 0; same && i < need; ++i) same = pin[i] == h->act_pin[i];
      if (!same && pin.size() >= need) { h->act_pool->repin(pin); h->act_pin = pin; h->act_repins++; }
    }
  }
#endif
  const auto t1 = std::chrono::steady_clock::now();
  hostact::forward(ly, h->Lp + 1, h->cfg.policy_act, obs_host, b0, b1, raw, h->act_pool);
  hostact::head(raw, h->A, h->cfg.min_log_std, h->cfg.max_log_std, eps, h->act_scale_h, h->act_center_h, out, logp,
                h->cfg.policy_out_act, h->cfg.policy_std_param ? h->A : 2 * h->A);
  h->act_host_us = std::chrono::duration<double, std::micro>(std::chrono::steady_clock::now() - t1).count();
  h->act_host_calls++;
  return DSACT_OK;
}

static int mark_update(dsact_handle* h, bool end) {
  if (!h->uev0) {
    HIPCHK(h, hipEventCreate(&h->uev0));
    HIPCHK(h, hipEventCreate(&h->uev1));
  }
  HIPCHK(h, hipEventRecord(end ? h->uev1 : h->uev0, h->stream));
  h->uev_valid = end;
  return DSACT_OK;
}

int dsact_compute_grads(dsact_handle* h, int64_t iteration, uint32_t flags) {
  TRY(check_ready(h, true));
  HIPCHK(h, hipSetDevice(h->device));
  TRY(mark_update(h, false));
  TRY(enqueue_prologue(h, 0, iteration, 0, 1));
  TRY(enqueue_grads(h, !(flags & DSACT_F_SKIP_ACTOR_ON_OFF_ITERS) || (iteration % h->cfg.delay_update) == 0, false));
  return mark_update(h, true);
}

int dsact_apply_update(dsact_handle* h, int64_t iteration) {
  TRY(check_ready(h, false));
  HIPCHK(h, hipSetDevice(h->device));
  TRY(enqueue_prologue(h, 0, iteration, 1, 0));
  TRY(enqueue_adam(h));
  return (iteration % h->cfg.delay_update) == 0 ? policy_moved(h) : DSACT_OK;
}

int dsact_step(dsact_handle* h, int64_t iteration, uint32_t flags) {
  TRY(check_ready(h, true));
  HIPCHK(h, hipSetDevice(h->device));
  TRY(mark_update(h, false));
  TRY(enqueue_prologue(h, 0, iteration, 1, 1));
  TRY(enqueue_grads(h, !(flags & DSACT_F_SKIP_ACTOR_ON_OFF_ITERS) || (iteration % h->cfg.delay_update) == 0, true));
  TRY(mark_update(h, true));
  return (iteration % h->cfg.delay_update) == 0 ? policy_moved(h) : DSACT_OK;
}

static int enqueue_allreduce(dsact_handle* h, float* buf, size_t count, int op) {
  if (!h->comm) return fail(h, DSACT_E_STATE, "no communicator (dsact_comm_init)");
  const int rc = g_rccl.AllReduce(buf, buf, count, kNcclFloat, op, h->comm, h->stream);
  if (rc != 0) return fail(h, DSACT_E_HIP, "ncclAllReduce failed: %s", rccl_err(rc));
  return DSACT_OK;
}

static int enqueue_graph_step_dp(dsact_handle* h) {
  TRY(enqueue_gather(h, h->idx_table, h->idx_rows, 1, 0, 0));
  if (h->use_std_sums) {
    TRY(enqueue_grads(h, true, false, PH_FORWARD));
    TRY(enqueue_allreduce(h, h->std_sums, 2, kNcclSum));
    TRY(enqueue_grads(h, true, false, PH_BACKWARD));
  } else {
    TRY(enqueue_grads(h, true, false));
  }
  TRY(enqueue_allreduce(h, h->grads, h->n_online + 2, kNcclAvg));
  TRY(enqueue_prologue(h, 1, 0, 1, 0));
  return enqueue_adam(h);
}

static int enqueue_graph_step(dsact_handle* h, long long iteration, uint32_t flags) {
  if (flags & DSACT_F_DATA_PARALLEL) return enqueue_graph_step_dp(h);
  TRY(enqueue_gather(h, h->idx_table, h->idx_rows, 1, 0, 1));
  const bool actor = !(flags & DSACT_F_SKIP_ACTOR_ON_OFF_ITERS) || (iteration % h->cfg.delay_update) == 0;
  return enqueue_grads(h, actor, true);
}

static int capture_updates(dsact_handle* h, int n, uint32_t flags, bool merged, hipGraph_t* graph, hipGraphExec_t* exec) {
  HIPCHK(h, hipStreamBeginCapture(h->stream, hipStreamCaptureModeThreadLocal));
  int rc = DSACT_OK;
  if (!merged) {
    for (int s = 0; s < n && rc == DSACT_OK; ++s) rc = enqueue_graph_step(h, s, flags);
  } else {
    static_assert(dsact_handle::kAltSet == 1, "the plain graph alternates between sets 0 and kAltSet by parity");
    h->mirror_w0 = true;
    select_set(h, (n - 1) & 1);
    rc = enqueue_gather(h, h->idx_table, h->idx_rows, 1, 0, 1, 0);
    for (int s = 0; s < n && rc == DSACT_OK; ++s) {
      const int set = (n - 1 - s) & 1;
      RideArgs ride;
      memset(&ride, 0, sizeof(ride));
      select_set(h, set ^ 1);
      ride.g = gather_args(h, h->idx_table, h->idx_rows, 1, 0, 1);
      ride.g.lookahead = 1;
      ride.n_gather = s + 1 < n ? ride.g.n_gather_blocks : 0;
      ride.bookkeeping = 1;
      select_set(h, set);
      const bool actor = !(flags & DSACT_F_SKIP_ACTOR_ON_OFF_ITERS) || (s % h->cfg.delay_update) == 0;
      if (flags & DSACT_F_DATA_PARALLEL) {
        rc = enqueue_grads(h, true, false, PH_ALL, &ride);
        if (rc == DSACT_OK) rc = enqueue_allreduce(h, h->grads, h->n_online + 2, kNcclAvg);
        if (rc == DSACT_OK) rc = enqueue_adam_pack(h);
      } else {
        rc = enqueue_grads(h, actor, true, PH_ALL, &ride);
      }
    }
    select_set(h, 0);
    h->mirror_w0 = false;
  }
  hipError_t e = hipStreamEndCapture(h->stream, graph);
  if (rc != DSACT_OK) return rc;
  if (e != hipSuccess) return fail(h, DSACT_E_HIP, "hipStreamEndCapture: %s", hipGetErrorString(e));
  HIPCHK(h, hipGraphInstantiate(exec, *graph, nullptr, nullptr, 0));
  return DSACT_OK;
}

struct PipePlan {
  std::vector<PipeFwd> host; std::vector<char> pre, dop;
  std::vector<BwdForm> form;
  std::vector<BwdPiArgs> bp;
  std::vector<int> bp_rg;
  bool dp = false;
  bool skip = false;
  std::vector<char> leaves;
};
static int plan_updates_pipe(dsact_handle* h, int n, int phase, PipePlan& plan, PipeFwd* dev_args, uint32_t flags = 0) {
  const int D = h->cfg.delay_update;
  auto set_of = [&](int s) { return dsact_handle::pipe_set((s - (n - 1)) & (dsact_handle::kPipeSets - 1)); };
  plan.host.resize((size_t)n); plan.pre.resize((size_t)n); plan.dop.resize((size_t)n);
  plan.form.assign((size_t)n, BWD_PLAIN); plan.bp.resize((size_t)n); plan.bp_rg.assign((size_t)n, 2);
  const int rg_pi = h->B >= 8 ? h->cRG : 1;
  const bool can_defer = h->pi_merge && h->dw_chunks == 1 && !h->fat_bwd && rg_pi <= 2 && !h->env_no_pipe_defer;
  plan.dp = (flags & DSACT_F_DATA_PARALLEL) != 0;
  plan.skip = (flags & DSACT_F_SKIP_ACTOR_ON_OFF_ITERS) != 0 && !plan.dp;
  plan.leaves.assign((size_t)n, 0);
  const bool bqt = bqt_ok(h);
  const bool bqp = bqt && h->nq == 2 && !h->env_no_bqp && chain_rg(h, 4, true) == 1 && rg_pi == 2;
  if (bqt) TRY(build_bqt(h));
  bool pre = false;
  int rc = DSACT_OK;
  h->mirror_w0 = true;
  for (int s = 0; s < n && rc == DSACT_OK; ++s) {
    const bool leaves_policy = ((phase + s) % D) != 0;
    const bool do_pre = s + 1 < n && leaves_policy;
    plan.leaves[(size_t)s] = leaves_policy;
    const BwdPiArgs* bp = nullptr;
    if (s > 0 && defers_pi(plan.form[(size_t)s - 1])) {
      select_set(h, set_of(s - 1));
      BwdPiArgs& a = plan.bp[(size_t)s];
      bwd_pi_args(h, h->dw2_off[2], h->dw2_off[2], false, a, plan.bp_rg[(size_t)s], true);
      a.finalize = 0;
      a.dw.store_g = 0;
      bp = &a;
    }
    const bool defer = do_pre && can_defer && !plan.skip;
    const BwdForm form = defer ? (bqt ? BWD_QT : BWD_DEFER_PI) : (!leaves_policy && bqp) ? BWD_QPT : BWD_PLAIN;
    plan.form[(size_t)s] = form;
    rc = pipe_fwd_build(h, set_of(s), set_of(s + 1), pre, do_pre, plan.host[(size_t)s], bp, merged_bwd(form));
    plan.pre[(size_t)s] = pre; plan.dop[(size_t)s] = do_pre;
    pre = do_pre;
  }
  h->mirror_w0 = false;
  select_set(h, 0);
  TRY(rc);
  HIPCHK(h, hipMemcpy(dev_args, plan.host.data(), (size_t)n * sizeof(PipeFwd), hipMemcpyHostToDevice));
  return DSACT_OK;
}
static int enqueue_updates_pipe(dsact_handle* h, int n, const PipePlan& plan, PipeFwd* dev_args) {
  auto set_of = [&](int s) { return dsact_handle::pipe_set((s - (n - 1)) & (dsact_handle::kPipeSets - 1)); };
  const std::vector<PipeFwd>& host = plan.host;
  const std::vector<char>&pre_v = plan.pre, &do_v = plan.dop;
  int rc = DSACT_OK;
  h->mirror_w0 = true;
  {
    Gather2Args g;
    select_set(h, set_of(0));
    g.a = gather_args(h, h->idx_table, h->idx_rows, 1, 0, 1);
    g.a.bookkeeping = 0;
    g.a.rp = repack_args(h, repack_blocks(h));
    g.b = g.a;
    g.b.n_gather_blocks = 0;
    if (n > 1) {
      select_set(h, set_of(1));
      g.b = gather_args(h, h->idx_table, h->idx_rows, 1, 0, 1);
      g.b.bookkeeping = 0; g.b.lookahead = 1;
      g.b.rp = repack_args(h, 0);
    }
    rc = launch(h, "gather", k_gather2, dim3(g.a.n_gather_blocks + g.b.n_gather_blocks + g.a.rp.n_blocks), dim3(kThreads), 0, g);
  }
  for (int s = 0; s < n && rc == DSACT_OK; ++s) {
    select_set(h, set_of(s));
    const bool carries = s > 0 && defers_pi(plan.form[(size_t)s - 1]);
    rc = launch_chain_fwd_pipe(h, pipe_fwd_name(pre_v[(size_t)s], do_v[(size_t)s]), host[(size_t)s], dev_args + s,
                               carries ? &plan.bp[(size_t)s] : nullptr, plan.bp_rg[(size_t)s]);
    if (rc != DSACT_OK) break;
    RideArgs ride;
    memset(&ride, 0, sizeof(ride));
    if (s + 2 < n) {
      select_set(h, set_of(s + 2));
      ride.g = gather_args(h, h->idx_table, h->idx_rows, 1, 0, 1);
      ride.g.lookahead = 2;
      ride.n_gather = ride.g.n_gather_blocks;
      select_set(h, set_of(s));
    } else {
      ride.g = gather_args(h, h->idx_table, h->idx_rows, 1, 0, 1);
      ride.n_gather = 0;
    }
    const BwdForm form = plan.form[(size_t)s];
    ride.bookkeeping = merged_bwd(form) ? 0 : 1;
    if (plan.dp) {
      rc = enqueue_grads(h, true, false, PH_BACKWARD, &ride, form);
      if (rc == DSACT_OK) rc = enqueue_allreduce(h, h->grads, h->n_online + 2, kNcclAvg);
      if (rc == DSACT_OK) rc = enqueue_adam_pack(h);
      continue;
    }
    rc = enqueue_grads(h, !(plan.skip && plan.leaves[(size_t)s]), true, PH_BACKWARD, &ride, form);
  }
  select_set(h, 0);
  h->mirror_w0 = false;
  h->n_heads_parts = h->B / 4;
  return rc;
}

static int capture_updates_pipe(dsact_handle* h, int n, int phase, hipGraph_t* graph, hipGraphExec_t* exec, PipeFwd** dev_args, uint32_t flags) {
  HIPCHK(h, hipMalloc((void**)dev_args, (size_t)n * sizeof(PipeFwd)));
  PipePlan plan;
  TRY(plan_updates_pipe(h, n, phase, plan, *dev_args, flags));
  HIPCHK(h, hipStreamBeginCapture(h->stream, hipStreamCaptureModeThreadLocal));
  const int rc = enqueue_updates_pipe(h, n, plan, *dev_args);
  hipError_t e = hipStreamEndCapture(h->stream, graph);
  if (rc != DSACT_OK) return rc;
  if (e != hipSuccess) return fail(h, DSACT_E_HIP, "hipStreamEndCapture: %s", hipGetErrorString(e));
  HIPCHK(h, hipGraphInstantiate(exec, *graph, nullptr, nullptr, 0));
  return DSACT_OK;
}

static bool pipe_eligible(const dsact_handle* h, int steps_per_graph, uint32_t flags) {
  const int D = h->cfg.delay_update;
  const bool merged = !h->cnn && h->use_w1p && h->dw_chunks == 1 && !h->use_std_sums && h->alt_ws != nullptr;
  return merged && h->chain_ok && !h->fat && h->fwd_merge && h->B % 4 == 0 && (h->rng_seed != 0 || h->noise_table_on) &&
         (!(flags & DSACT_F_DATA_PARALLEL) || h->comm != nullptr) && D >= 2 &&
         D <= dsact_handle::kPipePhases && steps_per_graph >= 2;
}

static int build_graph(dsact_handle* h, int steps_per_graph, uint32_t flags, bool noise_table, bool keep_cache) {
  TRY(check_ready(h, false));
  if (steps_per_graph < 1) return fail(h, DSACT_E_INVALID, "steps_per_graph must be >= 1");
  if (!h->idx_table) return fail(h, DSACT_E_STATE, "upload an index table first (dsact_upload_index_table)");
  HIPCHK(h, hipSetDevice(h->device));
  if ((flags & DSACT_F_SKIP_ACTOR_ON_OFF_ITERS) && steps_per_graph % h->cfg.delay_update)
    return fail(h, DSACT_E_INVALID, "with DSACT_F_SKIP_ACTOR_ON_OFF_ITERS steps_per_graph must be a multiple of delay_update");
  if ((flags & DSACT_F_DATA_PARALLEL) && !h->comm) return fail(h, DSACT_E_STATE, "DSACT_F_DATA_PARALLEL needs dsact_comm_init");
  HIPCHK(h, hipStreamSynchronize(h->stream));
  if (keep_cache) stash_graph(h); else drop_graphs(h);
  h->want_graph_steps = 0;
  if (h->flags_dirty && h->chain_flags) {
    HIPCHK(h, hipMemset(h->chain_flags, 0, kChainFlags * sizeof(int)));
    h->flags_dirty = false;
  }
  const bool merged = !h->cnn && h->use_w1p && h->dw_chunks == 1 && !h->use_std_sums && h->alt_ws != nullptr &&
                      (!(flags & DSACT_F_DATA_PARALLEL) || h->chain_ok);
  const int D = h->cfg.delay_update;
  dsact_handle::GraphSet& g = h->active;
  h->noise_table_on = noise_table;
  const bool pipe = pipe_eligible(h, steps_per_graph, flags);
  const bool was_prof = h->profiling;
  h->profiling = false;
  int rc = DSACT_OK;
  if (pipe) {
    rc = alloc_pipe_sets(h);
    for (int ph = 0; ph < D && rc == DSACT_OK; ++ph) rc = capture_updates_pipe(h, steps_per_graph, ph, &g.pgraph[ph], &g.pexec[ph], &g.pargs[ph], flags);
    g.pipe = rc == DSACT_OK;
    if (rc != DSACT_OK) {
      drop_active_graph(h);
      (void)hipGetLastError();
      select_set(h, 0);
      rc = DSACT_OK;
    }
  }
  if (!g.pipe) {
    rc = capture_updates(h, steps_per_graph, flags, merged, &g.graph, &g.exec);
  }
  h->profiling = was_prof;
  h->noise_table_on = false;
  if (rc != DSACT_OK) { if (keep_cache) drop_active_graph(h); else drop_graphs(h); return rc; }
  g.merged = merged; g.noise_table = noise_table;
  g.steps = steps_per_graph;
  g.flags = flags;
  h->have_batch = true;
  return DSACT_OK;
}

int dsact_graph_build(dsact_handle* h, int32_t steps_per_graph, uint32_t flags) { return build_graph(h, steps_per_graph, flags, false, false); }

static int launch_groups(dsact_handle* h, int64_t first_iteration, int64_t n_groups) {
  h->uev_valid = false;
  int64_t i = 0;
  const dsact_handle::GraphSet& g = h->active;
  if (g.pipe) {
    const int D = h->cfg.delay_update;
    for (; i < n_groups; ++i) {
      const int ph = (int)(((first_iteration + i * g.steps) % D + D) % D);
      HIPCHK(h, hipGraphLaunch(g.pexec[ph], h->stream));
    }
    return DSACT_OK;
  }
  for (; i < n_groups; ++i) HIPCHK(h, hipGraphLaunch(g.exec, h->stream));
  return DSACT_OK;
}

static int set_device_iteration(dsact_handle* h, long long it) {
  if (h->dev_it_next == it) return DSACT_OK;
  HIPCHK(h, hipMemcpyAsync(&h->st->it_next, &it, sizeof(long long), hipMemcpyHostToDevice, h->stream));
  HIPCHK(h, hipStreamSynchronize(h->stream));
  h->dev_it_next = it;
  return DSACT_OK;
}

int dsact_graph_run(dsact_handle* h, int64_t first_iteration, int64_t n_steps) {
  TRY(check_usable(h));
  TRY(ensure_wanted_graph(h));
  if (!have_graph(h)) return fail(h, DSACT_E_STATE, "dsact_graph_build first");
  if (n_steps % h->active.steps) return fail(h, DSACT_E_INVALID, "n_steps must be a multiple of steps_per_graph");
  if ((h->active.flags & DSACT_F_SKIP_ACTOR_ON_OFF_ITERS) && first_iteration % h->cfg.delay_update)
    return fail(h, DSACT_E_INVALID, "first_iteration must be a multiple of delay_update for a graph captured with DSACT_F_SKIP_ACTOR_ON_OFF_ITERS");
  HIPCHK(h, hipSetDevice(h->device));
  TRY(set_device_iteration(h, first_iteration));
  TRY(launch_groups(h, first_iteration, n_steps / h->active.steps));
  h->dev_it_next = first_iteration + n_steps;
  return policy_moved(h);
}

int dsact_run_group(dsact_handle* h, int64_t first_iteration, int32_t n_steps, const int64_t* idx, const float* noise, uint32_t flags) {
  if (!h || n_steps < 1) return DSACT_E_INVALID;
  TRY(check_ready(h, false));
  if (!has_ring(h)) return fail(h, DSACT_E_STATE, "buffer not created");
  if (h->size == 0) return fail(h, DSACT_E_STATE, "buffer empty");
  if (!idx && h->idx_seed == 0)
    return fail(h, DSACT_E_STATE, "no index rows: pass idx, or call dsact_set_index_rng to have the device draw them");
  if (!noise && h->rng_seed == 0) return fail(h, DSACT_E_STATE, "no noise source: pass the noise rows or call dsact_set_device_rng");
  if ((flags & DSACT_F_SKIP_ACTOR_ON_OFF_ITERS) && (n_steps % h->cfg.delay_update || first_iteration % h->cfg.delay_update))
    return fail(h, DSACT_E_INVALID, "with DSACT_F_SKIP_ACTOR_ON_OFF_ITERS a group must cover whole delay_update periods");
  HIPCHK(h, hipSetDevice(h->device));
  const size_t B = (size_t)h->B, A = (size_t)h->A;
  const size_t n_idx = (size_t)n_steps * B, nz_row = 2 * B * A + 2 * B;
  for (size_t i = 0; idx && i < n_idx; ++i)
    if (idx[i] < 0 || idx[i] >= h->size) return fail(h, DSACT_E_INVALID, "index %lld out of range [0,%lld)", (long long)idx[i], h->size);
  TRY(ensure_group_tables(h, n_steps));
  if (noise && !h->noise_table) {
    HIPCHK(h, hipMalloc(&h->noise_table, (size_t)h->idx_rows * nz_row * sizeof(float)));
    HIPCHK(h, hipMemset(h->noise_table, 0, (size_t)h->idx_rows * nz_row * sizeof(float)));
  }
  const bool want_table = noise != nullptr;
  const dsact_handle::GraphSet& g = h->active;
  if (!(g.present() && g.steps == n_steps && g.flags == flags && g.noise_table == want_table)) {
    stash_graph(h);
    if (!activate_graph(h, n_steps, flags, want_table)) TRY(build_graph(h, n_steps, flags, want_table, true));
  }
  const size_t idx_bytes = idx ? n_idx * sizeof(int) : 0;
  const size_t need = idx_bytes + (noise ? (size_t)n_steps * nz_row * sizeof(float) : 0);
  if (!idx) TRY(enqueue_draw_indices(h, first_iteration, n_steps));
  if (need) {
    if (need > h->grp_pin_bytes) {
      HIPCHK(h, hipStreamSynchronize(h->stream));
      size_t cap = need < (1u << 16) ? (1u << 16) : need;
      for (int i = 0; i < 4; ++i) {
        if (h->grp_pin[i]) { hipHostFree(h->grp_pin[i]); h->grp_pin[i] = nullptr; }
        HIPCHK(h, hipHostMalloc((void**)&h->grp_pin[i], cap, hipHostMallocDefault));
        if (!h->grp_ev[i]) HIPCHK(h, hipEventCreateWithFlags(&h->grp_ev[i], hipEventDisableTiming));
      }
      h->grp_pin_bytes = cap;
    }
    const int slot = (int)(h->grp_k++ & 3);
    HIPCHK(h, hipEventSynchronize(h->grp_ev[slot]));
    if (idx) {
      int* pin_idx = (int*)h->grp_pin[slot];
      for (size_t i = 0; i < n_idx; ++i) pin_idx[i] = (int)idx[i];
      HIPCHK(h, hipMemcpyAsync(h->idx_table, pin_idx, n_idx * sizeof(int), hipMemcpyHostToDevice, h->stream));
    }
    if (noise) {
      float* pin_nz = (float*)(h->grp_pin[slot] + idx_bytes);
      memcpy(pin_nz, noise, (size_t)n_steps * nz_row * sizeof(float));
      HIPCHK(h, hipMemcpyAsync(h->noise_table, pin_nz, (size_t)n_steps * nz_row * sizeof(float), hipMemcpyHostToDevice, h->stream));
    }
    HIPCHK(h, hipEventRecord(h->grp_ev[slot], h->stream));
  }
  hipLaunchKernelGGL(k_set_counters, dim3(1), dim3(64), 0, h->stream, h->st, (long long)first_iteration, 0LL);
  if (hipGetLastError() != hipSuccess) return fail(h, DSACT_E_HIP, "launch k_set_counters failed");
  TRY(launch_groups(h, first_iteration, 1));
  h->dev_it_next = first_iteration + n_steps;
  h->have_batch = true;
  return policy_moved(h);
}

int dsact_dp_begin(dsact_handle* h, int64_t first_iteration) {
  if (!h) return DSACT_E_INVALID;
  HIPCHK(h, hipSetDevice(h->device));
  return set_device_iteration(h, first_iteration);
}

int dsact_dp_enqueue_grads(dsact_handle* h, uint32_t flags) {
  TRY(check_ready(h, false));
  if (!h->idx_table) return fail(h, DSACT_E_STATE, "upload an index table first");
  HIPCHK(h, hipSetDevice(h->device));
  (void)flags;
  TRY(enqueue_gather(h, h->idx_table, h->idx_rows, 1, 0, 0));
  h->have_batch = true;
  return enqueue_grads(h, true, false);
}

int dsact_dp_enqueue_grads_critic(dsact_handle* h, uint32_t flags) {
  TRY(check_ready(h, false));
  if (!h->idx_table) return fail(h, DSACT_E_STATE, "upload an index table first");
  if (h->use_std_sums) return fail(h, DSACT_E_STATE, "the split gradient halves are for the one-collective mode (strict mode has its own halves)");
  HIPCHK(h, hipSetDevice(h->device));
  (void)flags;
  TRY(enqueue_gather(h, h->idx_table, h->idx_rows, 1, 0, 0));
  h->have_batch = true;
  return enqueue_grads(h, true, false, PH_DP_CRITIC);
}

int dsact_dp_enqueue_grads_actor(dsact_handle* h, uint32_t flags) {
  TRY(check_ready(h, true));
  HIPCHK(h, hipSetDevice(h->device));
  (void)flags;
  return enqueue_grads(h, true, false, PH_DP_ACTOR);
}

int dsact_dp_set_strict(dsact_handle* h, float* std_sums_dev) {
  if (!h) return DSACT_E_INVALID;
  HIPCHK(h, hipSetDevice(h->device));
  HIPCHK(h, hipStreamSynchronize(h->stream));
  if (any_graph(h)) return fail(h, DSACT_E_STATE, "data-parallel mode is baked into the captured graph");
  if (!h->std_sums_own) h->std_sums_own = h->std_sums;
  h->use_std_sums = std_sums_dev != nullptr;
  h->std_sums = std_sums_dev ? std_sums_dev : h->std_sums_own;
  return DSACT_OK;
}

int dsact_dp_enqueue_forward(dsact_handle* h, uint32_t flags) {
  TRY(check_ready(h, false));
  if (!h->idx_table) return fail(h, DSACT_E_STATE, "upload an index table first");
  if (!h->use_std_sums) return fail(h, DSACT_E_STATE, "dsact_dp_set_strict first");
  HIPCHK(h, hipSetDevice(h->device));
  (void)flags;
  TRY(enqueue_gather(h, h->idx_table, h->idx_rows, 1, 0, 0));
  h->have_batch = true;
  return enqueue_grads(h, true, false, PH_FORWARD);
}

int dsact_dp_enqueue_backward(dsact_handle* h, uint32_t flags) {
  TRY(check_ready(h, true));
  if (!h->use_std_sums) return fail(h, DSACT_E_STATE, "dsact_dp_set_strict first");
  HIPCHK(h, hipSetDevice(h->device));
  (void)flags;
  return enqueue_grads(h, true, false, PH_BACKWARD);
}

int dsact_dp_enqueue_apply(dsact_handle* h) {
  TRY(check_ready(h, false));
  HIPCHK(h, hipSetDevice(h->device));
  TRY(enqueue_prologue(h, 1, 0, 1, 0));
  TRY(enqueue_adam(h));
  return policy_moved(h);
}

int dsact_comm_unique_id(const char* rccl_path, uint8_t id[128]) {
  if (!id) return DSACT_E_INVALID;
  if (rccl_load(rccl_path)) return DSACT_E_STATE;
  NcclUid u;
  memset(&u, 0, sizeof(u));
  if (g_rccl.GetUniqueId(&u) != 0) return DSACT_E_HIP;
  memcpy(id, u.internal, 128);
  return DSACT_OK;
}

int dsact_comm_init(dsact_handle* h, int32_t rank, int32_t world, const uint8_t id[128], const char* rccl_path) {
  if (!h || !id || world < 1 || rank < 0 || rank >= world) return DSACT_E_INVALID;
  HIPCHK(h, hipSetDevice(h->device));
  if (any_graph(h)) return fail(h, DSACT_E_STATE, "the communicator is baked into the captured graph");
  if (const char* e = rccl_load(rccl_path)) return fail(h, DSACT_E_STATE, "%s", e);
  if (h->comm) { g_rccl.CommDestroy(h->comm); h->comm = nullptr; }
  NcclUid u;
  memcpy(u.internal, id, 128);
  const int rc = g_rccl.CommInitRank(&h->comm, world, u, rank);
  if (rc != 0) { h->comm = nullptr; return fail(h, DSACT_E_HIP, "ncclCommInitRank failed: %s", rccl_err(rc)); }
  h->comm_rank = rank; h->comm_world = world;
  return DSACT_OK;
}

int dsact_comm_destroy(dsact_handle* h) {
  if (!h) return DSACT_E_INVALID;
  if (h->comm) {
    hipSetDevice(h->device);
    if (h->stream) hipStreamSynchronize(h->stream);
    g_rccl.CommDestroy(h->comm);
    h->comm = nullptr;
  }
  return DSACT_OK;
}

int dsact_dp_enqueue_allreduce(dsact_handle* h) {
  TRY(check_ready(h, false));
  HIPCHK(h, hipSetDevice(h->device));
  return enqueue_allreduce(h, h->grads, h->n_online + 2, kNcclAvg);
}

static int enqueue_stats(dsact_handle* h, float* dst) {
  StatsArgs a;
  a.part_loss = h->part_loss; a.n_loss = h->B; a.part_heads = h->part_heads; a.n_heads = h->chain_ok ? h->n_heads_parts : h->n_heads_wg;
  a.log_alpha = h->online + h->n_online - 1; a.st = h->st;
  a.inv_B = 1.0f / (float)h->B; a.inv_BA = 1.0f / ((float)h->B * (float)h->A);
  a.auto_alpha = h->cfg.auto_alpha; a.alpha_fixed = h->cfg.alpha_fixed; a.out = dst;
  a.ms_tail = h->have_local_tail && h->cfg.algo == 0 ? h->grads + h->n_online : nullptr;
  a.spin_timeout = nullptr;
  const bool was_prof = h->profiling;
  h->profiling = false;
  int rc = launch(h, "stats", k_stats, dim3(1), dim3(64), 0, a);
  h->profiling = was_prof;
  return rc;
}

int dsact_read_stats(dsact_handle* h, float out[16]) {
  if (!h || !out) return DSACT_E_INVALID;
  TRY(check_ready(h, false));
  HIPCHK(h, hipSetDevice(h->device));
  TRY(enqueue_stats(h, h->stats));
  HIPCHK(h, hipMemcpyAsync(out, h->stats, 16 * sizeof(float), hipMemcpyDeviceToHost, h->stream));
  HIPCHK(h, hipStreamSynchronize(h->stream));
  TRY(check_handoff(h));
  out[15] = -1.0f;
  if (h->uev_valid) {
    float ms = 0.f;
    if (hipEventElapsedTime(&ms, h->uev0, h->uev1) == hipSuccess) out[15] = ms;
  }
  return DSACT_OK;
}

int dsact_stats_snapshot(dsact_handle* h, int32_t slot) {
  if (!h || slot < 0 || slot >= DSACT_STATS_SLOTS) return DSACT_E_INVALID;
  TRY(check_ready(h, false));
  HIPCHK(h, hipSetDevice(h->device));
  return enqueue_stats(h, h->stats + 16 * (1 + slot));
}

int dsact_stats_read(dsact_handle* h, int32_t slot, float out[16]) {
  if (!h || !out || slot < 0 || slot >= DSACT_STATS_SLOTS) return DSACT_E_INVALID;
  HIPCHK(h, hipSetDevice(h->device));
  HIPCHK(h, hipMemcpyAsync(out, h->stats + 16 * (1 + slot), 16 * sizeof(float), hipMemcpyDeviceToHost, h->stream));
  HIPCHK(h, hipStreamSynchronize(h->stream));
  return check_handoff(h);
}

int dsact_time_steps(dsact_handle* h, int64_t first_iteration, int64_t n_steps, uint32_t flags, int32_t use_graph, float* ms_total) {
  if (!h || !ms_total || n_steps < 1) return DSACT_E_INVALID;
  const long long shadow = h->dev_it_next;
  TRY(check_ready(h, false));
  if (use_graph) h->dev_it_next = shadow;
  HIPCHK(h, hipSetDevice(h->device));
  if (!h->idx_table) return fail(h, DSACT_E_STATE, "upload an index table first");
  if (!h->tev0) {
    HIPCHK(h, hipEventCreate(&h->tev0));
    HIPCHK(h, hipEventCreate(&h->tev1));
  }
  TRY(set_device_iteration(h, first_iteration));
  HIPCHK(h, hipEventRecord(h->tev0, h->stream));
  if (use_graph) {
    TRY(ensure_wanted_graph(h));
    if (!have_graph(h)) return fail(h, DSACT_E_STATE, "dsact_graph_build first");
    if (n_steps % h->active.steps) return fail(h, DSACT_E_INVALID, "n_steps must be a multiple of steps_per_graph");
    if ((h->active.flags & DSACT_F_SKIP_ACTOR_ON_OFF_ITERS) && first_iteration % h->cfg.delay_update)
      return fail(h, DSACT_E_INVALID, "first_iteration must be a multiple of delay_update");
    TRY(launch_groups(h, first_iteration, n_steps / h->active.steps));
    h->dev_it_next = first_iteration + n_steps;
  } else {
    h->dev_it_next = -1;
    for (int64_t i = 0; i < n_steps; ++i) TRY(enqueue_graph_step(h, first_iteration + i, flags));
  }
  HIPCHK(h, hipEventRecord(h->tev1, h->stream));
  {
    hipError_t q = hipErrorNotReady;
    const auto t_poll = std::chrono::steady_clock::now();
    while ((q = hipEventQuery(h->tev1)) == hipErrorNotReady) {
      if (std::chrono::steady_clock::now() - t_poll > std::chrono::milliseconds(5)) break;
    }
    if (q != hipSuccess) HIPCHK(h, hipEventSynchronize(h->tev1));
  }
  HIPCHK(h, hipEventElapsedTime(ms_total, h->tev0, h->tev1));
  h->have_batch = true;
  h->pol_epoch++;
  return check_handoff(h);
}

int dsact_time_stage(dsact_handle* h, int32_t stage, int32_t reps, float* ms_total, double* macs) {
  if (!h || !ms_total || reps < 1) return DSACT_E_INVALID;
  TRY(check_ready(h, false));
  const int L = h->L;
  if (stage < 0 || stage >= 2 * L || (stage >= L && stage - L >= (int)h->fwd2.size()))
    return fail(h, DSACT_E_INVALID, "stage must be in 0..%d (group B has %d layers)", 2 * L - 1, (int)h->fwd2.size());
  HIPCHK(h, hipSetDevice(h->device));
  const Stage& s = stage < L ? h->fwd1[stage] : h->fwd2[stage - L];
  if (macs) {
    double m = 0;
    for (int i = 0; i < s.args.n_prob; ++i) m += (double)s.args.p[i].M * s.args.p[i].N * s.args.p[i].K;
    *macs = m;
  }
  const bool was_prof = h->profiling;
  h->profiling = false;
  hipEvent_t e0, e1;
  HIPCHK(h, hipEventCreate(&e0));
  HIPCHK(h, hipEventCreate(&e1));
  for (int i = 0; i < 20; ++i) TRY(run_stage(h, s));
  HIPCHK(h, hipEventRecord(e0, h->stream));
  for (int i = 0; i < reps; ++i) TRY(run_stage(h, s));
  HIPCHK(h, hipEventRecord(e1, h->stream));
  HIPCHK(h, hipEventSynchronize(e1));
  HIPCHK(h, hipEventElapsedTime(ms_total, e0, e1));
  hipEventDestroy(e0);
  hipEventDestroy(e1);
  h->profiling = was_prof;
  return DSACT_OK;
}

int dsact_profile_step(dsact_handle* h, int64_t iteration, uint32_t flags, dsact_kernel_time* out, int32_t cap, int32_t* n) {
  if (!h || !out || !n) return DSACT_E_INVALID;
  h->pol_epoch++;
  TRY(check_ready(h, false));
  if (!h->idx_table) return fail(h, DSACT_E_STATE, "upload an index table first");
  HIPCHK(h, hipSetDevice(h->device));
  TRY(set_device_iteration(h, iteration));
  for (auto& r : h->prof) { hipEventDestroy(r.e0); hipEventDestroy(r.e1); }
  h->prof.clear();
  h->profiling = true;
  int rc = enqueue_graph_step(h, iteration, flags);
  h->profiling = false;
  TRY(rc);
  HIPCHK(h, hipStreamSynchronize(h->stream));
  int cnt = 0;
  for (auto& r : h->prof) {
    if (cnt >= cap) break;
    float ms = 0.f;
    HIPCHK(h, hipEventElapsedTime(&ms, r.e0, r.e1));
    memset(&out[cnt], 0, sizeof(out[cnt]));
    strncpy(out[cnt].name, r.name.c_str(), sizeof(out[cnt].name) - 1);
    out[cnt].ms = ms;
    out[cnt].blocks = r.blocks;
    ++cnt;
  }
  *n = cnt;
  return DSACT_OK;
}

int dsact_profile_steps(dsact_handle* h, int64_t first_iteration, int32_t n_steps, uint32_t flags, dsact_kernel_time* out, int32_t cap, int32_t* n) {
  if (!h || !out || !n || n_steps < 1) return DSACT_E_INVALID;
  h->pol_epoch++;
  TRY(check_ready(h, false));
  if (!h->idx_table) return fail(h, DSACT_E_STATE, "upload an index table first");
  HIPCHK(h, hipSetDevice(h->device));
  TRY(set_device_iteration(h, first_iteration));
  h->dev_it_next = -1;
  for (auto& r : h->prof) { hipEventDestroy(r.e0); hipEventDestroy(r.e1); }
  h->prof.clear();
  int rc = DSACT_OK;
  if (pipe_eligible(h, n_steps, flags)) {
    const int D = h->cfg.delay_update;
    PipeFwd* dev = nullptr;
    TRY(alloc_pipe_sets(h));
    HIPCHK(h, hipMalloc((void**)&dev, (size_t)n_steps * sizeof(PipeFwd)));
    PipePlan plan;
    rc = plan_updates_pipe(h, n_steps, (int)((first_iteration % D + D) % D), plan, dev, flags);
    if (rc == DSACT_OK) {
      h->profiling = true;
      rc = enqueue_updates_pipe(h, n_steps, plan, dev);
      h->profiling = false;
    }
    hipStreamSynchronize(h->stream);
    hipFree(dev);
  } else {
    h->profiling = true;
    for (int i = 0; i < n_steps && rc == DSACT_OK; ++i) rc = enqueue_graph_step(h, first_iteration + i, flags);
    h->profiling = false;
  }
  TRY(rc);
  HIPCHK(h, hipStreamSynchronize(h->stream));
  h->have_batch = true;
  int cnt = 0;
  for (auto& r : h->prof) {
    if (cnt >= cap) break;
    float ms = 0.f;
    HIPCHK(h, hipEventElapsedTime(&ms, r.e0, r.e1));
    memset(&out[cnt], 0, sizeof(out[cnt]));
    strncpy(out[cnt].name, r.name.c_str(), sizeof(out[cnt].name) - 1);
    out[cnt].ms = ms;
    out[cnt].blocks = r.blocks;
    ++cnt;
  }
  *n = cnt;
  return check_handoff(h);
}

int dsact_chain_active(const dsact_handle* h) { return h && h->chain_ok ? 1 : 0; }

const char* dsact_debug_names(void) {
  return "X0,XP,X2,rew,done,eps_new,eps_2,z5,z6,logits_pi,logits_pit,logp_new,logp2,"
         "qout_c0,qout_c1,qout_t0,qout_t1,qout_p0,qout_p1,dout0,dout1,dout2,dout3,dout_pi,d_new_act,"
         "part_loss,part_heads,H.<chain>.<l>,G.<chain>.<l>,dZ.<chain>.<l> (chains: pi,pit,q1c,q2c,q1t,q2t,q1p,q2p)";
}

int dsact_debug_read(dsact_handle* h, const char* name, float* out, size_t cap, size_t* n) {
  if (!h || !name || !out || !n) return DSACT_E_INVALID;
  HIPCHK(h, hipSetDevice(h->device));
  const size_t B = h->B, A = h->A;
  const float* src = nullptr;
  size_t cnt = 0;
  int unpack_w = 0;
  std::string s(name);
  struct E { const char* k; const float* p; size_t c; };
  const E tab[] = {
      {"X0", h->X0, B * h->ldx}, {"XP", h->XP, B * h->ldx}, {"X2", h->X2, B * h->ldx}, {"rew", h->rew, B}, {"done", h->done, B},
      {"eps_new", h->eps_new, B * A}, {"eps_2", h->eps_2, B * A}, {"z5", h->z5, B}, {"z6", h->z6, B},
      {"logits_pi", h->logits_pi, B * 2 * A}, {"logits_pit", h->logits_pit, B * 2 * A}, {"logp_new", h->logp_new, B}, {"logp2", h->logp2, B},
      {"qout_c0", h->qout_c[0], 2 * B}, {"qout_c1", h->qout_c[1], 2 * B}, {"qout_t0", h->qout_t[0], 2 * B}, {"qout_t1", h->qout_t[1], 2 * B},
      {"qout_p0", h->qout_p[0], 2 * B}, {"qout_p1", h->qout_p[1], 2 * B},
      {"dout0", h->dout[0], 2 * B}, {"dout1", h->dout[1], 2 * B}, {"dout2", h->dout[2], 2 * B}, {"dout3", h->dout[3], 2 * B},
      {"dout_pi", h->dout_pi, B * 2 * A}, {"d_new_act", h->d_new_act, B * A},
      {"part_loss", h->part_loss, (size_t)h->B * kLossPart}, {"part_heads", h->part_heads, (size_t)h->n_heads_wg * 2},
      {"timeline", (const float*)h->timeline, (size_t)1024 * 16 * 2},
  };
  for (const E& e : tab) if (s == e.k) { src = e.p; cnt = e.c; }
  if (!src && s.size() > 4 && (s[0] == 'H' || s[0] == 'G' || s.compare(0, 2, "dZ") == 0)) {
    const size_t d1 = s.find('.'), d2 = s.rfind('.');
    if (d1 != std::string::npos && d2 != d1) {
      const std::string kind = s.substr(0, d1), chn = s.substr(d1 + 1, d2 - d1 - 1);
      const int l = atoi(s.c_str() + d2 + 1);
      int ch = -1;
      for (int c = 0; c < N_CHAIN; ++c) if (chn == kChainName[c]) ch = c;
      if (ch >= 0 && l >= 0 && l < chain_L(h, ch)) {
        const int wch = (kChainNet[ch] == N_POL || kChainNet[ch] == N_POLT) ? h->wp[l] : h->wq[l];
        cnt = B * wch;
        if (kind == "H") src = h->Hb[ch][l];
        else if (kind == "G") src = h->Gb[ch][l];
        else if (kind == "dZ" && kDzSlot[ch] >= 0) src = h->dZ[kDzSlot[ch]][l];
        unpack_w = h->chain_ok ? wch : 0;
      }
    }
  }
  if (!src && h->cnn && (s.compare(0, 5, "cact.") == 0 || s.compare(0, 4, "cdy.") == 0 || s.compare(0, 6, "dfeat.") == 0)) {
    const size_t d1 = s.find('.'), d2 = s.rfind('.');
    const int st = atoi(s.c_str() + d1 + 1), j = d2 != d1 ? atoi(s.c_str() + d2 + 1) : 0;
    if (st >= 0 && st < N_STACK && j >= 0 && j < h->n_conv) {
      const ConvGeom& g = h->cg[j];
      cnt = B * g.OH * g.OW * g.Cout;
      if (s[1] == 'a') src = h->cact[st][j];
      else if (s[1] == 'd' && st < 3) src = h->cdy[st][j];
      else if (s[1] == 'f' && st < 3) { src = h->dfeat[st]; cnt = B * h->F; }
    }
  }
  if (!src) return fail(h, DSACT_E_INVALID, "unknown debug buffer '%s'", name);
  if (cnt > cap) return fail(h, DSACT_E_INVALID, "debug buffer '%s' needs %zu floats, cap %zu", name, cnt, cap);
  HIPCHK(h, hipStreamSynchronize(h->stream));
  if (unpack_w) {
    std::vector<float> raw(cnt);
    HIPCHK(h, hipMemcpy(raw.data(), src, cnt * sizeof(float), hipMemcpyDeviceToHost));
    const int C = h->B / 16;
    for (int b = 0; b < h->B; ++b)
      for (int f = 0; f < unpack_w; ++f) out[(size_t)b * unpack_w + f] = raw[pk_index(f, b, C)];
  } else {
    HIPCHK(h, hipMemcpy(out, src, cnt * sizeof(float), hipMemcpyDeviceToHost));
  }
  *n = cnt;
  return DSACT_OK;
}

namespace {
__global__ void k_debug_fill(float* p, long long rows, long long ld, int col0, int ncols, float v) {
  const long long i = (long long)blockIdx.x * blockDim.x + threadIdx.x;
  if (i >= rows * ncols) return;
  p[(i / ncols) * ld + col0 + (i % ncols)] = v;
}
int debug_fill(dsact_handle* h, float* p, long long rows, long long ld, int col0, int ncols, float v) {
  if (!p || rows * ncols <= 0) return DSACT_OK;
  const long long n = rows * ncols;
  hipLaunchKernelGGL(k_debug_fill, dim3((unsigned)((n + 255) / 256)), dim3(256), 0, h->stream, p, rows, ld, col0, ncols, v);
  return hipGetLastError() == hipSuccess ? DSACT_OK : fail(h, DSACT_E_HIP, "debug fill failed");
}
}

int dsact_debug_set(dsact_handle* h, const char* name, double value) {
  if (!h || !name) return DSACT_E_INVALID;
  HIPCHK(h, hipSetDevice(h->device));
  if (!strcmp(name, "withhold_flag")) {
    HIPCHK(h, hipStreamSynchronize(h->stream));
    drop_graphs(h);
    h->debug_withhold = (int)value;
    if (h->twin && h->online) TRY(build_twin_fwd(h));
    return DSACT_OK;
  }
  if (!strcmp(name, "raise_handoff_word")) {
    if (!h->handoff_host) return fail(h, DSACT_E_STATE, "no hand-off words");
    HIPCHK(h, hipStreamSynchronize(h->stream));
    if ((int)value & 1) ((volatile int*)h->handoff_host)[0] = 1;
    if ((int)value & 2) ((volatile int*)h->handoff_host)[1] = 1;
    return DSACT_OK;
  }
  if (!strcmp(name, "mode_host_rows")) {
    h->mode_host_rows = (int)value;
    return DSACT_OK;
  }
  if (!strcmp(name, "host_act")) {
    h->host_act = value != 0.0;
    h->pol_epoch++;
    return DSACT_OK;
  }
  if (!strcmp(name, "beh_live_copy")) {
    h->beh_live_copy = value != 0.0;
    return DSACT_OK;
  }
  if (!strcmp(name, "policy_dirty")) {
    h->pol_epoch++;
    return DSACT_OK;
  }
  if (!strcmp(name, "ack_state")) {
    h->state_invalid = false;
    return DSACT_OK;
  }
  if (!strcmp(name, "poison_handover")) {
    const float v = (float)value;
    for (int i = 0; i < 4; ++i) TRY(debug_fill(h, h->zobs[i], 1, 0, 0, h->B * h->w[0], v));
    const BatchBufs& alt = h->sets[dsact_handle::kAltSet];
    float* rows[4] = {h->XP, h->X2, alt.XP, alt.X2};
    for (float* r : rows) TRY(debug_fill(h, r, h->B, h->ldx, h->F, h->A, v));
    for (int i = 0; i < 2; ++i) TRY(debug_fill(h, h->dAq[i], 1, 0, 0, h->B * 32, v));
    if (h->chain_ok) for (int l = 0; l < h->L; ++l) TRY(debug_fill(h, h->dZ[kDzSlot[C_PI]][l], 1, 0, 0, h->B * h->w[l], v));
    if (h->chain_ok && !h->twin)
      for (int i = 0; i < h->nq; ++i) {
        for (int l = 0; l < h->L; ++l) TRY(debug_fill(h, h->dZ[kDzSlot[i == 0 ? C_Q1C : C_Q2C]][l], 1, 0, 0, h->B * h->w[l], v));
        TRY(debug_fill(h, h->doutT[i], 1, 0, 0, 32 * h->B, v));
      }
    return DSACT_OK;
  }
  if (!strcmp(name, "fwd_merge")) {
    HIPCHK(h, hipStreamSynchronize(h->stream));
    drop_graphs(h);
    h->fwd_merge = value != 0.0 && h->chain_ok && !h->cnn && h->B <= 256 && h->B / 4 <= kChainFlagSlices && chain_rg(h, 4) == 1;
    return DSACT_OK;
  }
  if (!strcmp(name, "pi_merge")) {
    HIPCHK(h, hipStreamSynchronize(h->stream));
    drop_graphs(h);
    h->pi_merge = value != 0.0 && h->chain_ok && !h->cnn && h->B <= 512 && !h->fat_bwd;
    if (h->chain_flags) HIPCHK(h, hipMemset(h->chain_flags, 0, kChainFlagInts * sizeof(int)));
    h->flags_dirty = false;
    return DSACT_OK;
  }
  return fail(h, DSACT_E_INVALID, "dsact_debug_set: unknown name '%s'", name);
}

int dsact_debug_get(const dsact_handle* h, const char* name, double* value) {
  if (!h || !name || !value) return DSACT_E_INVALID;
  if (!strcmp(name, "fwd_merge")) *value = h->fwd_merge ? 1.0 : 0.0;
  else if (!strcmp(name, "pi_merge")) *value = h->pi_merge ? 1.0 : 0.0;
  else if (!strcmp(name, "dcol_ident")) {
    int n = 0;
    for (int j = 1; j < h->n_conv; ++j) {
      const ConvGeom& g = h->cg[j];
      if (g.OH == 1 && g.OW == 1 && g.H == g.KS && g.W == g.KS && !h->env_no_dcol_ident && g.Cin > 16) ++n;
    }
    *value = (double)n;
  }
  else if (!strcmp(name, "act_launch_us")) *value = h->act_launch_us;
  else if (!strcmp(name, "act_host")) *value = act_host_ok(h) ? 1.0 : 0.0;
  else if (!strcmp(name, "act_host_us")) *value = h->act_host_us;
  else if (!strcmp(name, "act_host_threads")) *value = (double)h->act_threads;
  else if (!strcmp(name, "act_host_pinned")) *value = h->act_pool ? (double)h->act_pool->pinned() : 0.0;
  else if (!strcmp(name, "act_host_repins")) *value = (double)h->act_repins;
  else if (!strcmp(name, "act_host_isa")) *value = (double)hostact::cpu_isa();
  else if (!strcmp(name, "act_copy_wait_us")) *value = h->act_copy_wait_us;
  else if (!strcmp(name, "act_host_calls")) *value = (double)h->act_host_calls;
  else if (!strcmp(name, "act_copies")) *value = (double)h->act_copies;
  else if (!strcmp(name, "beh_held")) *value = h->beh_held ? 1.0 : 0.0;
  else if (!strcmp(name, "beh_holds")) *value = (double)h->beh_holds;
  else if (!strcmp(name, "beh_acts")) *value = (double)h->beh_acts;
  else if (!strcmp(name, "beh_live_copy")) *value = h->beh_live_copy ? 1.0 : 0.0;
  else if (!strcmp(name, "act_wait_us")) *value = h->act_wait_us;
  else if (!strcmp(name, "fat")) *value = (h->fat ? 1.0 : 0.0) + (h->fat_bwd ? 2.0 : 0.0);
  else if (!strcmp(name, "handoff_failures")) *value = (double)h->handoff_failures;
  else if (!strcmp(name, "graph_steps")) *value = (double)h->active.steps;
  else if (!strcmp(name, "pipe_graph")) *value = h->active.pipe ? 1.0 : 0.0;
  else if (!strcmp(name, "merged_graph")) *value = h->active.merged ? 1.0 : 0.0;
  else if (!strcmp(name, "state_invalid")) *value = h->state_invalid ? 1.0 : 0.0;
  else if (!strcmp(name, "act_batch_calls")) *value = (double)h->ab_calls;
  else if (!strcmp(name, "act_mode_calls")) *value = (double)h->ab_mode_calls;
  else if (!strcmp(name, "mode_host_rows")) *value = (double)h->mode_host_rows;
  else if (!strcmp(name, "act_dev_calls")) *value = (double)h->act_dev_calls;
  else if (!strcmp(name, "ring_commit_rows")) *value = (double)h->ring_commit_rows;
  else if (!strcmp(name, "act_dev_syncs")) *value = (double)h->act_dev_syncs;
  else if (!strcmp(name, "act_mode_dev_calls")) *value = (double)h->act_mode_dev_calls;
  else if (!strcmp(name, "eval_commit_calls")) *value = (double)h->eval_commit_calls;
  else if (!strcmp(name, "eval_polls")) *value = (double)h->eval_polls;
  else if (!strcmp(name, "track_commit_calls")) *value = (double)h->track_commit_calls;
  else if (!strcmp(name, "track_reads")) *value = (double)h->track_reads;
  else if (!strcmp(name, "act_fast")) *value = act_fast_ok(h) ? 1.0 : 0.0;
  else if (!strcmp(name, "graph_cache")) *value = (double)h->graph_cache.size();
  else if (!strcmp(name, "graph_noise_table")) *value = h->active.noise_table ? 1.0 : 0.0;
  else if (!strcmp(name, "twin_par")) *value = (h->twin_par ? 1.0 : 0.0) + (h->twin_merged ? 2.0 : 0.0);
  else return DSACT_E_INVALID;
  return DSACT_OK;
}

static int act_forward_fast(dsact_handle* h, const float* obs_host, const float* eps, float* out_host) {
  TRY(check_handoff(h));
  ActArgs a;
  a.n_layers = h->Lp + 1;
  const float* base = net_params(h, N_POL);
  int wg = 0;
  for (int l = 0; l <= h->Lp; ++l) {
    a.ly[l].W = base + h->pd.w_off[l]; a.ly[l].b = base + h->pd.b_off[l];
    a.ly[l].K = h->pd.in[l]; a.ly[l].N = h->pd.out[l]; a.ly[l].half = 0;
    if (h->pd.nblk == 2 && l > 0 && l < h->Lp) { a.ly[l].K = h->pd.in[l] / 2; a.ly[l].half = h->pd.out[l] / 2; }
    a.wg_begin[l] = wg;
    wg += ((l == h->Lp && eps ? h->A : h->pd.out[l]) + 3) / 4;
  }
  a.wg_begin[h->Lp + 1] = wg;
  if (h->act_call >= 0x7ffffff0) {
    HIPCHK(h, hipStreamSynchronize(h->stream));
    HIPCHK(h, hipMemset(h->act_h, 0, (size_t)kActMaxLayers * kMaxWidth * sizeof(unsigned long long)));
    memset(h->act_out_host, 0, 64 * sizeof(unsigned long long));
    h->act_call = 0;
  }
  a.h = h->act_h; a.call = ++h->act_call;
  a.A = h->A; a.lo_ls = h->cfg.min_log_std; a.hi_ls = h->cfg.max_log_std; a.act = h->cfg.policy_act;
  a.out = h->act_out_dev; a.timeout = h->handoff_dev + 1;
  a.sample = eps ? 1 : 0; a.act_scale = h->act_scale; a.act_center = h->act_center;
  a.out_act = h->cfg.policy_out_act; a.out_n = h->cfg.policy_std_param ? h->A : 2 * h->A;
  if (eps) memcpy(a.eps, eps, (size_t)h->A * sizeof(float));
  memcpy(a.x, obs_host, (size_t)h->O * sizeof(float));
  const auto tl = std::chrono::steady_clock::now();
  TRY(launch(h, "act_mlp", k_act_mlp, dim3(wg), dim3(256), 0, a));
  const auto t0 = std::chrono::steady_clock::now();
  h->act_launch_us = std::chrono::duration<double, std::micro>(t0 - tl).count();
  const int n_out = 2 * h->A;
  const unsigned want = (unsigned)a.call;
  unsigned polls = 0;
  for (int k = 0; k < n_out;) {
    const unsigned long long pr = ((volatile unsigned long long*)h->act_out_host)[k];
    if ((unsigned)(pr >> 32) == want) {
      const unsigned bits = (unsigned)pr;
      memcpy(out_host + k, &bits, sizeof(float));
      ++k;
      continue;
    }
    if ((++polls & 0xFFFF) == 0 && std::chrono::steady_clock::now() - t0 > std::chrono::seconds(10)) {
      HIPCHK(h, hipStreamSynchronize(h->stream));
      TRY(check_handoff(h));
      return fail(h, DSACT_E_HIP, "acting forward did not complete");
    }
  }
  h->act_wait_us = std::chrono::duration<double, std::micro>(std::chrono::steady_clock::now() - t0).count();
  return check_handoff(h);
}
static bool act_fast_ok(const dsact_handle* h) {
  return !h->cnn && h->O <= kActMaxObs && h->Lp + 1 <= kActMaxLayers && !h->env_no_fast_act && h->A <= 32;
}

static int act_batch_gpu(dsact_handle* h, const float* obs, int32_t n, const float* eps, float* action_host, float* logp_host,
                        const float* base, hipStream_t stream);
int dsact_act_sample(dsact_handle* h, const float* obs_host, const float* eps_host, float* action_host, float* logp_host) {
  if (!h || !obs_host || !eps_host || !action_host || !logp_host) return DSACT_E_INVALID;
  if (!h->online) return fail(h, DSACT_E_STATE, "arenas not bound");
  if (!h->limits_set) return fail(h, DSACT_E_STATE, "action limits not set (dsact_set_action_limits)");
  if (!act_fast_ok(h)) return fail(h, DSACT_E_INVALID, "dsact_act_sample serves MLP policies with obs <= %d floats", kActMaxObs);
  HIPCHK(h, hipSetDevice(h->device));
  if (h->beh_held) {
    h->beh_acts++;
    if (act_host_ok(h) && h->beh_host_ok) return act_forward_host(h, obs_host, eps_host, action_host, logp_host, true);
    return act_batch_gpu(h, obs_host, 1, eps_host, action_host, logp_host, h->beh_dev, h->act_stream);
  }
  if (act_host_ok(h)) return act_forward_host(h, obs_host, eps_host, action_host, logp_host);
  float out[64];
  TRY(act_forward_fast(h, obs_host, eps_host, out));
  const int A = h->A;
  float lp = 0.0f;
  for (int d = 0; d < A; ++d) { action_host[d] = out[d]; lp += out[A + d]; }
  *logp_host = lp;
  return DSACT_OK;
// ... 444 lines not shown
```

### dsac-v2_amd/dsac_v2_hip.py

```python
__all__ = ["ApproxContainer", "DSAC_V2_HIP", "TanhGaussDistribution", "GaussDistribution"]

import copy
import math
import os
import sys
import time
from typing import Dict, Tuple

import numpy as np
import torch
import torch.nn as nn

_PKG = os.path.dirname(os.path.abspath(__file__))
if _PKG not in sys.path:
    sys.path.insert(0, _PKG)

from dsact.engine import STAT_KEYS, DsactEngine, register_engine
from dsact.layout import CONV_TYPES, ArenaLayout, CnnArenaLayout

ALG_TIME_KEY = "Time/Algorithm time [ms]-RL iter"
_LOG_EPS = 1e-6


class TanhGaussDistribution:
# ... 245 lines not shown
        raise NotImplementedError("policy_std_type=%r is built for the MLP approximators only" % st)


class ApproxContainer(nn.Module):

    def __init__(self, **kwargs):
        super().__init__()
        _check_supported(kwargs)
        hidden = _hidden_sizes(kwargs)
        ct = _conv_type(kwargs)
        A = int(kwargs["action_dim"])
        O = tuple(int(v) for v in kwargs["obsv_dim"]) if ct else int(kwargs["obsv_dim"])
        hi = np.asarray(kwargs["action_high_limit"], dtype=np.float32)
        lo = np.asarray(kwargs["action_low_limit"], dtype=np.float32)
        mn = kwargs.get("policy_min_log_std", -20.0)
        mx = kwargs.get("policy_max_log_std", 2.0)
        va, pa = kwargs.get("value_hidden_activation", "gelu"), kwargs.get("policy_hidden_activation", "gelu")
        if ct:
            self.q1 = HipCnnActionValueDistri(O, A, ct, va)
            self.q2 = HipCnnActionValueDistri(O, A, ct, va)
        else:
            vo = kwargs.get("value_output_activation", "linear")
            self.q1 = HipActionValueDistri(O, A, hidden, va, vo)
            self.q2 = HipActionValueDistri(O, A, hidden, va, vo)
        self.q1_target = copy.deepcopy(self.q1)
        self.q2_target = copy.deepcopy(self.q2)
        if ct:
            self.policy = HipCnnStochaPolicy(O, A, ct, hi, lo, mn, mx, pa)
        else:
            self.policy = HipStochaPolicy(O, A, _policy_hidden_sizes(kwargs) or hidden, hi, lo, mn, mx, pa,
                                          kwargs.get("policy_std_type", "mlp_shared"), kwargs.get("policy_output_activation", "linear"))
        self.policy.action_distribution_cls = ACT_DISTRIBUTIONS[kwargs.get("policy_act_distribution", "TanhGaussDistribution")][1]
        self.policy_target = copy.deepcopy(self.policy)
        for net in (self.policy_target, self.q1_target, self.q2_target):
            for p in net.parameters():
                p.requires_grad = False
        self.log_alpha = nn.Parameter(torch.tensor(1, dtype=torch.float32))
        object.__setattr__(self, "_engine", None)
        object.__setattr__(self, "_layout", CnnArenaLayout(O, A, ct) if ct else
                           ArenaLayout(O, A, hidden, policy_std_type=kwargs.get("policy_std_type", "mlp_shared"),
                                       policy_hidden=_policy_hidden_sizes(kwargs)))

    def create_action_distributions(self, logits):
        return self.policy.get_act_dist(logits)

    def _named_param_slots(self):
        lay = self._layout
        out = []
        for net in lay.all_nets:
            mod = getattr(self, net)
            params = dict(mod.named_parameters())
            for suffix, arena, off, shape, strides in lay.param_views(net):
                out.append((params[suffix], arena, off, shape, strides))
        out.append((self.log_alpha, "online", lay.log_alpha_offset, (), ()))
        return out

    def attach(self, engine: DsactEngine):
        arenas = {"online": engine.online, "target": engine.target}
        if isinstance(engine.layout, type(self._layout)):
            object.__setattr__(self, "_layout", engine.layout)
        with torch.no_grad():
            for p, arena, off, shape, strides in self._named_param_slots():
                view = torch.as_strided(arenas[arena], shape, strides, off)
                assert tuple(view.shape) == tuple(p.shape), (tuple(view.shape), tuple(p.shape))
                view.copy_(p.data.to(view.device))
                p.data = view
            for net in ("policy", "policy_target"):
                zr = getattr(self._layout, "zero_rows", lambda _n: None)(net)
                if zr is not None:
                    arenas[zr[0]][zr[1]:zr[1] + zr[2]].zero_()
                for arena, off, shape, strides in getattr(self._layout, "zero_blocks", lambda _n: [])(net):
                    torch.as_strided(arenas[arena], shape, strides, off).zero_()
            for pol in (self.policy, self.policy_target):
                pol.act_high_lim = pol.act_high_lim.to(engine.device)
                pol.act_low_lim = pol.act_low_lim.to(engine.device)
        torch.cuda.current_stream(engine.device).synchronize()
        object.__setattr__(self, "_engine", engine)
        self.policy._engine = engine
        for child in self.children():
            if child is not self.policy and not getattr(child, "_dsact_sync_hook", False):
                child.register_forward_pre_hook(lambda _m, _a, _e=engine: _e.sync())
                child._dsact_sync_hook = True
        engine.set_action_limits(self.policy.act_high_lim.cpu().numpy(), self.policy.act_low_lim.cpu().numpy())

    def _apply(self, fn, *a, **k):
        if self._engine is not None:
            return self
        return super()._apply(fn, *a, **k)

    def load_state_dict(self, state_dict, strict=True, **kw):
        if self._engine is not None:
            self._engine.sync()
            state_dict = {k: v.to(self._engine.device) for k, v in state_dict.items()}
        out = super().load_state_dict(state_dict, strict=strict, **kw)
        if self._engine is not None:
            torch.cuda.current_stream(self._engine.device).synchronize()
            self._engine.set_action_limits(self.policy.act_high_lim.cpu().numpy(),
                                           self.policy.act_low_lim.cpu().numpy())
            self._engine.policy_dirty()
        return out

    def state_dict(self, *a, **k):
        if self._engine is not None:
            self._engine.sync()
        return super().state_dict(*a, **k)


class LazyTbInfo(dict):
    def __init__(self, alg, serial, alg_time_ms):
        super().__init__()
        self._alg, self._serial, self._done = alg, serial, False
        dict.__setitem__(self, ALG_TIME_KEY, alg_time_ms)

    def _stats(self):
        alg = self._alg
        if alg._serial == self._serial:
            return alg.engine.read_stats()
        if 0 < alg._serial - self._serial < alg.engine.STATS_SLOTS:
            return alg.engine.read_stats(slot=self._serial)
        raise RuntimeError("tb_info of update %d was read %d updates later; device statistics are kept for the last "
                           "%d updates only" % (self._serial, alg._serial - self._serial, alg.engine.STATS_SLOTS))

    def _materialize(self):
        if self._done:
            return
        stats = self._stats()
        for k in STAT_KEYS:
            v = stats[k]
            if k in ("DSAC2/mean_std1", "DSAC2/mean_std2"):
                v = torch.tensor(v)
            dict.__setitem__(self, k, v)
        t = dict.pop(self, ALG_TIME_KEY)
        dev = stats.get("_device_ms", -1.0)
        dict.__setitem__(self, ALG_TIME_KEY, dev if dev >= 0.0 and dev > t else t)
        self._done = True

    def __getitem__(self, k):
        if k != ALG_TIME_KEY:
            self._materialize()
        return dict.__getitem__(self, k)

    def get(self, k, default=None):
        self._materialize()
        return dict.get(self, k, default)

    def __contains__(self, k):
        return k == ALG_TIME_KEY or k in STAT_KEYS

    def keys(self):
        self._materialize()
        return dict.keys(self)

    def values(self):
        self._materialize()
        return dict.values(self)

    def items(self):
        self._materialize()
        return dict.items(self)

    def __iter__(self):
        self._materialize()
        return dict.__iter__(self)

    def __len__(self):
        return len(STAT_KEYS) + 1


class HipBatch(dict):

    def __init__(self, engine, idxs, drawn=None):
        super().__init__()
        self.engine, self._drawn = engine, drawn
        self._idxs = None if idxs is None else np.array(idxs, dtype=np.int64, copy=True)
        assert (self._idxs is None) != (drawn is None)
        self.serial = engine.stage_serial
        self._ptr0, self._added0 = engine.buffer_ptr, engine.rows_added
        self._fill_epoch0 = engine.fill_epoch

    @property
    def idxs(self):
        if self._idxs is None:
# ... 339 lines not shown
```

### dsac-v2_amd/dsact/dp.py

```python
import contextlib

import torch
import torch.distributed as dist


F_DATA_PARALLEL = 2


def rank_index_seed(seed: int, rank: int) -> int:
    base = (int(seed or 0) * 0xD1342543DE82EF95 + 0x2545F4914F6CDD1D) % (1 << 63)
    return (base + int(rank) * 0x9E3779B97F4A7C15) % (1 << 63) or 1


class DataParallelUpdater:
    def __init__(self, engine, group=None, broadcast_tensors=(), strict=False, overlap=False, native=False):
        if not dist.is_initialized():
            raise RuntimeError("torch.distributed is not initialised")
        self.engine, self.group = engine, group
        self.world = dist.get_world_size(group)
        self.rank = dist.get_rank(group)
        self._avg = dist.get_backend(group) == "nccl"
        self.force_collective = False
        self.strict = bool(strict)
        if self.strict:
            engine.dp_set_strict(True)
        self.native = bool(native)
        if self.native:
            ids = [engine.comm_unique_id() if self.rank == 0 else None]
            dist.broadcast_object_list(ids, src=0, group=group)
            engine.comm_init(self.rank, self.world, ids[0])
        self.overlap = bool(overlap) and not self.strict and hasattr(engine, "dp_grads_critic")
        self.graph_mode = False
        with self._on_engine_stream():
            for t in broadcast_tensors:
                dist.broadcast(t, src=0, group=group)
        if hasattr(engine, "policy_dirty"):
            engine.policy_dirty()

    def _on_engine_stream(self):
        ts = getattr(self.engine, "torch_stream", None)
        return torch.cuda.stream(ts) if ts is not None else contextlib.nullcontext()

    def build_graph(self, steps_per_graph: int, fallback: bool = True) -> bool:
        if not self.native:
            raise RuntimeError("the graph-captured data-parallel update needs native=True (dsact_comm_init)")
        import sys

        ok, err = 1, None
        try:
            if self.world > 1 or self.force_collective:
                self.engine.dp_allreduce()
                self.engine.sync()
            self.engine.graph_build(steps_per_graph, F_DATA_PARALLEL)
        except Exception as ex:
            if not fallback:
                raise
            ok, err = 0, ex
        if self.world > 1:
            try:
                cpu_group = "gloo" in str(dist.get_backend(self.group)).lower()
            except Exception:
                cpu_group = True
            t = torch.tensor([ok], dtype=torch.int32, device="cpu" if cpu_group else getattr(self.engine, "device", "cpu"))
            dist.all_reduce(t, op=dist.ReduceOp.MIN, group=self.group)
            all_ok = int(t.item())
        else:
            all_ok = ok
        self.graph_mode = bool(all_ok)
        if not all_ok:
            sys.stderr.write("dsact.dp: rank %d: the data-parallel hipGraph could NOT be captured (%s) -- falling back to the "
                             "EAGER coordinator on every rank (same RCCL communicator, one launch sequence per update)\n"
                             % (self.rank, repr(err) if err is not None else "another rank failed"))
            try:
                self.engine.sync()
            except Exception:
                pass
        return self.graph_mode

    def run(self, first_iteration: int, n_steps: int):
        if getattr(self, "graph_mode", False):
            return self.run_graph(first_iteration, n_steps)
        self.engine.dp_begin(first_iteration)
        for _ in range(n_steps):
            self.step()

    def run_graph(self, first_iteration: int, n_steps: int):
        self.engine.graph_run(first_iteration, n_steps)

    def seed_indices(self, seed: int) -> int:
        key = rank_index_seed(seed, self.rank)
        self.engine.set_index_rng(key)
        return key

    def draw_indices(self, first_iteration: int, n_steps: int):
        self.engine.draw_indices(first_iteration, n_steps)

    def allreduce_grads(self):
        g = self.engine.grads
        if self.world == 1 and not self.force_collective:
            return
        if self.native:
            self.engine.dp_allreduce()
            return
        with self._on_engine_stream():
            if self._avg:
                dist.all_reduce(g, op=dist.ReduceOp.AVG, group=self.group)
            else:
                dist.all_reduce(g, op=dist.ReduceOp.SUM, group=self.group)
                g.div_(self.world)

    def _reduce_async(self, t):
        if self._avg:
            return dist.all_reduce(t, op=dist.ReduceOp.AVG, group=self.group, async_op=True)
        return dist.all_reduce(t, op=dist.ReduceOp.SUM, group=self.group, async_op=True)

    def step_overlapped(self):
        e = self.engine
        g, n_c = e.grads, e.critic_grad_count
        with self._on_engine_stream():
            e.dp_grads_critic()
# ... 23 lines not shown
```

### dsac-v2_amd/dsact/engine.py

```python
import ctypes as C
import os
from typing import Dict, List, Optional, Sequence

import numpy as np

from . import _ffi
from ._ffi import DsactError
from .layout import ArenaLayout, CnnArenaLayout

STAT_KEYS = [
    "DSAC2/critic_avg_q1-RL iter", "DSAC2/critic_avg_q2-RL iter",
    "DSAC2/critic_avg_std1-RL iter", "DSAC2/critic_avg_std2-RL iter",
    "DSAC2/critic_avg_min_std1-RL iter", "DSAC2/critic_avg_min_std2-RL iter",
    "Loss/Actor loss-RL iter", "Loss/Critic loss-RL iter",
    "DSAC2/policy_mean-RL iter", "DSAC2/policy_std-RL iter", "DSAC2/entropy-RL iter",
    "DSAC2/alpha-RL iter", "DSAC2/mean_std1", "DSAC2/mean_std2",
]


def _f32(a):
    return np.ascontiguousarray(np.asarray(a, dtype=np.float32))


RING_COLUMNS = ("obs", "obs2", "act", "rew", "done", "logp")
_M64 = (1 << 64) - 1


def ring_digest_reference(cols, row0, widths=None):
    out = []
    u = np.uint64
    with np.errstate(over="ignore"):
        for c, key in enumerate(RING_COLUMNS):
            a = np.ascontiguousarray(cols[key])
            n = int(a.shape[0])
            if a.dtype == np.uint8:
                v = a.reshape(-1).astype(np.uint64)
            elif a.dtype == np.float32:
                v = a.reshape(-1).view(np.uint32).astype(np.uint64)
            else:
                raise ValueError("ring column %s must be float32 or uint8 (got %s)" % (key, a.dtype))
            w = int(widths[c]) if widths is not None else (v.size // n if n else 1)
            if v.size != n * w:
                raise ValueError("ring column %s holds %d elements, expected %d rows x %d" % (key, v.size, n, w))
            g = u((int(row0) * w) & _M64) + np.arange(v.size, dtype=np.uint64)
            x = g * u(0x9E3779B97F4A7C15) + ((u(c + 1) << u(32)) | v)
            x ^= x >> u(30)
            x *= u(0xBF58476D1CE4E5B9)
            x ^= x >> u(27)
            x *= u(0x94D049BB133111EB)
            x ^= x >> u(31)
            out.append(int(x.sum(dtype=np.uint64)) & _M64)
    return tuple(out)


class DsactEngine:
    def __init__(self, obs_dim: int, act_dim: int, hidden: Sequence[int], batch: int, *,
                 gamma=0.99, tau=0.005, tau_b=None, auto_alpha=True, alpha=0.2, delay_update=2,
                 lr_q=1e-4, lr_pi=1e-4, lr_alpha=3e-4, min_log_std=-20.0, max_log_std=0.5,
                 global_batch: Optional[int] = None, device: int = 0, conv_type: Optional[str] = None,
                 algo: str = "DSAC_V2", td_bound: float = 20.0, v1_bound: bool = True, value_act: int = 0, policy_act: int = 0, act_dist: int = 0,
                 policy_std_type: str = "mlp_shared", value_out_act: int = 0, policy_out_act: int = 0,
                 policy_hidden: Optional[Sequence[int]] = None, pad_widths: bool = False):
        kw = dict(gamma=gamma, tau=tau, tau_b=tau_b, auto_alpha=auto_alpha, alpha=alpha, delay_update=delay_update, lr_q=lr_q, lr_pi=lr_pi,
                  lr_alpha=lr_alpha, min_log_std=min_log_std, max_log_std=max_log_std, global_batch=global_batch, device=device,
                  conv_type=conv_type, algo=algo, td_bound=td_bound, v1_bound=v1_bound, value_act=value_act, policy_act=policy_act,
                  act_dist=act_dist, policy_std_type=policy_std_type, value_out_act=value_out_act, policy_out_act=policy_out_act,
                  policy_hidden=policy_hidden)
        pad = self._pad_width(hidden, policy_hidden, batch, obs_dim, **{k: v for k, v in kw.items() if k != "policy_hidden"}) if pad_widths else None
        self._init(obs_dim, act_dim, hidden, batch, pad_to=pad, **kw)
        if pad and not self.chain_active:
            self.close()
            self._init(obs_dim, act_dim, hidden, batch, pad_to=None, **kw)

    @staticmethod
    def _pad_width(hidden, policy_hidden, batch, obs_dim, *, conv_type=None, algo="DSAC_V2", policy_std_type="mlp_shared", value_act=0,
                   policy_act=0, **_):
        ph = list(policy_hidden) if policy_hidden is not None else list(hidden)
        widths = list(hidden) + ph
        if conv_type or policy_std_type == "mlp_separated" or len(ph) != len(hidden) or len(hidden) > 4:
            return None
        if len(set(widths)) == 1 and widths[0] in (64, 128, 256):
            return None
        if max(widths) > 256 or 4 in (int(value_act), int(policy_act)):
            return None
        if batch % 16 or (batch > 256 and batch % 256):
            return None
        return 64 if max(widths) <= 64 else (128 if max(widths) <= 128 else 256)

    def _init(self, obs_dim, act_dim, hidden, batch, *, pad_to=None,
              gamma=0.99, tau=0.005, tau_b=None, auto_alpha=True, alpha=0.2, delay_update=2,
              lr_q=1e-4, lr_pi=1e-4, lr_alpha=3e-4, min_log_std=-20.0, max_log_std=0.5,
              global_batch=None, device=0, conv_type=None,
              algo="DSAC_V2", td_bound=20.0, v1_bound=True, value_act=0, policy_act=0, act_dist=0,
              policy_std_type="mlp_shared", value_out_act=0, policy_out_act=0, policy_hidden=None):
        import torch

        self._lib = _ffi.load()
        if not torch.cuda.is_available():
            raise DsactError("DsactEngine needs an MI355X (torch.cuda.is_available() is False); "
                             "the DSAC-T update has no CPU fallback")
        self.torch = torch
        self.conv_type = conv_type
        self.algo = algo
        if algo not in ("DSAC_V2", "DSAC_V1"):
            raise DsactError("algo must be DSAC_V2 or DSAC_V1")
        if conv_type and policy_std_type != "mlp_shared":
            raise DsactError("policy_std_type %r is built for the MLP nets only" % policy_std_type)
        if conv_type:
            self.layout = CnnArenaLayout(obs_dim, act_dim, conv_type, n_critics=2 if algo == "DSAC_V2" else 1)
            if list(hidden) != self.layout.hidden:
                raise DsactError("conv_type %s fixes the MLP widths to %s" % (conv_type, self.layout.hidden))
            self.obs_shape = self.layout.obs_shape
            obs_dim = self.layout.obs_dim
        else:
            self.layout = ArenaLayout(obs_dim, act_dim, list(hidden), n_critics=2 if algo == "DSAC_V2" else 1,
                                      policy_std_type=policy_std_type, policy_hidden=policy_hidden, pad_to=pad_to)
            self.obs_shape = (int(obs_dim),)
        self.obs_dim, self.act_dim, self.batch = int(obs_dim), int(act_dim), int(batch)
        self.device_index = int(device)
        self.device = torch.device("cuda", self.device_index)
        cfg = _ffi.Config()
        cfg.obs_dim, cfg.act_dim, cfg.n_hidden = obs_dim, act_dim, len(hidden)
        if len(hidden) > _ffi.MAX_HIDDEN:
            raise DsactError("at most %d hidden layers" % _ffi.MAX_HIDDEN)
        for i, w in enumerate(hidden):
            cfg.hidden[i] = int(pad_to or w)
        cfg.batch = batch
        cfg.global_batch = int(global_batch or batch)
        cfg.auto_alpha = 1 if auto_alpha else 0
        cfg.delay_update = int(delay_update)
        cfg.gamma, cfg.tau = gamma, tau
        cfg.tau_b = tau if tau_b is None else tau_b
        cfg.lr_q, cfg.lr_pi, cfg.lr_alpha = lr_q, lr_pi, lr_alpha
        cfg.alpha_fixed = alpha
        cfg.min_log_std, cfg.max_log_std = min_log_std, max_log_std
        cfg.adam_beta1, cfg.adam_beta2, cfg.adam_eps = 0.9, 0.999, 1e-8
        if conv_type:
            cfg.conv_type = self.layout.conv_id
            cfg.img_c, cfg.img_h, cfg.img_w = self.obs_shape
        cfg.algo = 0 if algo == "DSAC_V2" else 1
        cfg.td_bound = float(td_bound)
        cfg.v1_unbounded = 0 if v1_bound else 1
        cfg.value_act, cfg.policy_act = int(value_act), int(policy_act)
        cfg.policy_std_param = 1 if policy_std_type == "parameter" else 0
        cfg.policy_twin = 1 if policy_std_type == "mlp_separated" else 0
        if policy_hidden is not None and list(policy_hidden) != list(hidden) and not pad_to:
            if conv_type or not 1 <= len(policy_hidden) <= _ffi.MAX_HIDDEN:
                raise DsactError("policy_hidden needs the MLP nets and 1..%d layers" % _ffi.MAX_HIDDEN)
            for i, w in enumerate(policy_hidden):
                cfg.policy_hidden[i] = int(w)
            if len(policy_hidden) != len(hidden):
                cfg.policy_n_hidden = len(policy_hidden)
        cfg.value_out_act, cfg.policy_out_act = int(value_out_act), int(policy_out_act)
        cfg.act_dist = int(act_dist)
        self.cfg = cfg
        self._h = C.c_void_p()
        rc = self._lib.dsact_create(C.byref(cfg), self.device_index, C.byref(self._h))
        if rc != 0:
            msg = self._lib.dsact_last_error(self._h).decode() if self._h else ""
            if self._h:
                self._lib.dsact_destroy(self._h)
                self._h = C.c_void_p()
            raise DsactError("dsact_create failed (%s): %s" % (_ffi.E_NAMES.get(rc, rc), msg))
        lay = self.layout
        assert self._lib.dsact_online_count(self._h) == lay.n_online, (self._lib.dsact_online_count(self._h), lay.n_online)
        assert self._lib.dsact_target_count(self._h) == lay.n_target
        assert self._lib.dsact_q_count(self._h) == lay.n_q and self._lib.dsact_pi_count(self._h) == lay.n_pi
        dev = self.device
        self.online = torch.zeros(lay.n_online, dtype=torch.float32, device=dev)
        self.target = torch.zeros(lay.n_target, dtype=torch.float32, device=dev)
        self.adam_m = torch.zeros(lay.n_online, dtype=torch.float32, device=dev)
        self.adam_v = torch.zeros(lay.n_online, dtype=torch.float32, device=dev)
        self.grads = torch.zeros(lay.n_online + 2, dtype=torch.float32, device=dev)
        self._chk(self._lib.dsact_bind_arenas(
            self._h, self.online.data_ptr(), self.target.data_ptr(), self.adam_m.data_ptr(),
            self.adam_v.data_ptr(), self.grads.data_ptr()))
        self._graph_steps = 0
        self.stage_serial = 0
        self.buffer_capacity = 0
        self.buffer_coded = False
        self.rows_added = 0
        self.fill_epoch = 0
        self.index_seed = 0

    def _chk(self, rc):
        if rc != 0:
            raise DsactError("%s: %s" % (_ffi.E_NAMES.get(rc, rc), self._lib.dsact_last_error(self._h).decode()))

    def close(self):
        if getattr(self, "_h", None):
            self._lib.dsact_destroy(self._h)
            self._h = C.c_void_p()

    def __del__(self):
        try:
            self.close()
        except Exception:
            pass

    def use_torch_stream(self):
        s = self.torch.cuda.current_stream(self.device).cuda_stream
        if not s:
            raise DsactError("torch's current stream is the legacy default stream (handle 0); run torch work under "
                             "`with torch.cuda.stream(engine.torch_stream):` instead")
        self._chk(self._lib.dsact_set_stream(self._h, C.c_void_p(s)))
        self._torch_stream = None

    @property
    def stream_ptr(self) -> int:
        return int(self._lib.dsact_get_stream(self._h) or 0)

    @property
    def torch_stream(self):
        ts = getattr(self, "_torch_stream", None)
        if ts is None or ts.cuda_stream != self.stream_ptr:
            ts = self.torch.cuda.ExternalStream(self.stream_ptr, device=self.device)
            self._torch_stream = ts
        return ts

    def sync(self):
        self._chk(self._lib.dsact_sync(self._h))

    def set_action_limits(self, high, low):
        hi, lo = _f32(high), _f32(low)
        self._chk(self._lib.dsact_set_action_limits(self._h, _ffi.fptr(hi), _ffi.fptr(lo)))
        self.act_high, self.act_low = hi.reshape(-1).copy(), lo.reshape(-1).copy()

    def get_state(self):
        steps = (C.c_int32 * 3)()
        ms = (C.c_float * 2)()
        self._chk(self._lib.dsact_get_state(self._h, steps, ms))
        return {"adam_steps": [int(s) for s in steps], "mean_std": [float(ms[0]), float(ms[1])]}

    def set_state(self, adam_steps=None, mean_std=None):
        st = (C.c_int32 * 3)(*adam_steps) if adam_steps is not None else None
        ms = (C.c_float * 2)(*mean_std) if mean_std is not None else None
        self._chk(self._lib.dsact_set_state(self._h, st, ms))

    HYPER = {"gamma": 0, "tau": 1, "tau_b": 2, "auto_alpha": 3, "alpha": 4, "delay_update": 5, "TD_bound": 6, "bound": 7}

    def set_hyper(self, name: str, value):
        self._chk(self._lib.dsact_set_hyper(self._h, self.HYPER[name], float(value)))
        self._graph_steps = 0

    def buffer_create(self, capacity: int, codebook=None):
        if codebook is None:
            self._chk(self._lib.dsact_buffer_create(self._h, int(capacity)))
        else:
            book = np.ascontiguousarray(codebook, dtype=np.float32)
            self._chk(self._lib.dsact_buffer_create_coded(self._h, int(capacity), _ffi.fptr(book), int(book.shape[0])))
        self.buffer_capacity = int(capacity)
        self.buffer_coded = codebook is not None

    ring_digest_reference = staticmethod(ring_digest_reference)

    @property
    def ring_widths(self):
        return (self.obs_dim, self.obs_dim, self.act_dim, 1, 1, 1)

    def _ring_dtypes(self):
        o = np.uint8 if getattr(self, "buffer_coded", False) else np.float32
        return (o, o, np.float32, np.float32, np.float32, np.float32)

    def buffer_export(self, row0: int, n: int) -> Dict[str, np.ndarray]:
        rows = max(int(n), 0)
        out = {k: np.empty((rows, w) if i < 3 else (rows,), dt)
# ... 62 lines not shown
        if idx is None:
            self._chk(self._lib.dsact_gather(self._h, None, self.batch))
        else:
            idx = np.ascontiguousarray(np.asarray(idx, dtype=np.int64))
            self._chk(self._lib.dsact_gather(self._h, idx.ctypes.data_as(C.POINTER(C.c_int64)), int(idx.shape[0])))
        self.stage_serial += 1

    def read_batch(self, with_logp=True) -> Dict[str, np.ndarray]:
        B, O, A = self.batch, self.obs_dim, self.act_dim
        shp = (B,) + tuple(self.obs_shape)
        out = {"obs": np.empty(shp, np.float32), "act": np.empty((B, A), np.float32),
               "rew": np.empty(B, np.float32), "obs2": np.empty(shp, np.float32),
               "done": np.empty(B, np.float32)}
        lp = np.empty(B, np.float32) if with_logp else None
        self._chk(self._lib.dsact_read_batch(self._h, _ffi.fptr(out["obs"]), _ffi.fptr(out["act"]),
                                             _ffi.fptr(out["rew"]), _ffi.fptr(out["obs2"]),
                                             _ffi.fptr(out["done"]), _ffi.fptr(lp)))
        if with_logp:
            out["logp"] = lp
        return out

    def _src(self, a, n):
        torch = self.torch
        if isinstance(a, torch.Tensor) and a.is_cuda and a.device.index == self.device_index:
            t = a.detach().to(torch.float32).contiguous()
            assert t.numel() == n, (tuple(t.shape), n)
            return C.cast(C.c_void_p(t.data_ptr()), _ffi._FP), t
        if isinstance(a, torch.Tensor):
            a = a.detach().cpu().numpy()
        a = _f32(a)
        assert a.size == n, (a.shape, n)
        return _ffi.fptr(a), a

    def load_batch(self, obs, act, rew, obs2, done):
        torch, B = self.torch, self.batch
        srcs = [self._src(obs, B * self.obs_dim), self._src(act, B * self.act_dim), self._src(rew, B),
                self._src(obs2, B * self.obs_dim), self._src(done, B)]
        if any(isinstance(k, torch.Tensor) for _, k in srcs):
            torch.cuda.current_stream(self.device).synchronize()
        self._chk(self._lib.dsact_load_batch(self._h, *[p for p, _ in srcs]))
        self.stage_serial += 1

    def upload_index_table(self, idx):
        idx = np.ascontiguousarray(np.asarray(idx, dtype=np.int64))
        assert idx.ndim == 2 and idx.shape[1] == self.batch
        self._chk(self._lib.dsact_upload_index_table(self._h, idx.ctypes.data_as(C.POINTER(C.c_int64)),
                                                     int(idx.shape[0])))

    def set_index_rng(self, seed: int):
        self._chk(self._lib.dsact_set_index_rng(self._h, int(seed)))
        self.index_seed = int(seed)

    def draw_indices(self, first_iteration: int, n: int = 1):
        self._chk(self._lib.dsact_draw_indices(self._h, int(first_iteration), int(n)))

    def read_indices(self, rows: int = 1) -> np.ndarray:
        out = np.empty((int(rows), self.batch), np.int64)
        self._chk(self._lib.dsact_read_indices(self._h, out.ctypes.data_as(C.POINTER(C.c_int64)), int(rows)))
        return out

    def set_noise(self, eps_new, eps_2, z5, z6):
        a, b, c, d = _f32(eps_new), _f32(eps_2), _f32(z5), _f32(z6)
        assert a.shape == (self.batch, self.act_dim) and c.shape == (self.batch,)
        self._chk(self._lib.dsact_set_noise(self._h, _ffi.fptr(a), _ffi.fptr(b), _ffi.fptr(c), _ffi.fptr(d)))

    def set_device_rng(self, seed: int):
        self._chk(self._lib.dsact_set_device_rng(self._h, int(seed)))

    def compute_grads(self, iteration: int, flags: int = 0):
        self._chk(self._lib.dsact_compute_grads(self._h, int(iteration), int(flags)))

    def apply_update(self, iteration: int):
        self._chk(self._lib.dsact_apply_update(self._h, int(iteration)))

    def step(self, iteration: int, flags: int = 0):
        self._chk(self._lib.dsact_step(self._h, int(iteration), int(flags)))

    def graph_build(self, steps_per_graph: int = 2, flags: int = 0):
        self._chk(self._lib.dsact_graph_build(self._h, int(steps_per_graph), int(flags)))
        self._graph_steps = int(steps_per_graph)

    def graph_run(self, first_iteration: int, n_steps: int):
        self.stage_serial += 1
        self._chk(self._lib.dsact_graph_run(self._h, int(first_iteration), int(n_steps)))

    def run_group(self, first_iteration: int, idx_rows, noise_rows=None, flags: int = 0, n: int = None):
        if idx_rows is None:
            if n is None or int(n) < 1:
                raise ValueError("run_group(idx_rows=None) needs n, the number of updates the device draws indices for")
            n, idx_ptr = int(n), None
        else:
            idx = np.ascontiguousarray(np.asarray(idx_rows, dtype=np.int64))
            assert idx.ndim == 2 and idx.shape[1] == self.batch, idx.shape
            assert n is None or int(n) == idx.shape[0], (n, idx.shape)
            n, idx_ptr = int(idx.shape[0]), idx.ctypes.data_as(C.POINTER(C.c_int64))
        nz = None
        if noise_rows is not None:
            nz = _f32(noise_rows)
            assert nz.shape == (n, 2 * self.batch * self.act_dim + 2 * self.batch), nz.shape
        self.stage_serial += 1
        self._chk(self._lib.dsact_run_group(self._h, int(first_iteration), n, idx_ptr, _ffi.fptr(nz), int(flags)))
        self._graph_steps = n

    def dp_begin(self, first_iteration: int):
        self._chk(self._lib.dsact_dp_begin(self._h, int(first_iteration)))

    def dp_grads(self, flags: int = 0):
        self.stage_serial += 1
        self._chk(self._lib.dsact_dp_enqueue_grads(self._h, int(flags)))

    def dp_grads_critic(self, flags: int = 0):
        self.stage_serial += 1
        self._chk(self._lib.dsact_dp_enqueue_grads_critic(self._h, int(flags)))

    def dp_grads_actor(self, flags: int = 0):
        self._chk(self._lib.dsact_dp_enqueue_grads_actor(self._h, int(flags)))

    @property
    def critic_grad_count(self):
        return 2 * self.layout.n_q

    def dp_set_strict(self, enable: bool = True):
        if enable:
            self.std_sums = self.torch.zeros(2, dtype=self.torch.float32, device=self.device)
            self._chk(self._lib.dsact_dp_set_strict(self._h, self.std_sums.data_ptr()))
        else:
            self._chk(self._lib.dsact_dp_set_strict(self._h, None))
            self.std_sums = None

    def dp_forward(self, flags: int = 0):
        self.stage_serial += 1
        self._chk(self._lib.dsact_dp_enqueue_forward(self._h, int(flags)))

    def dp_backward(self, flags: int = 0):
        self._chk(self._lib.dsact_dp_enqueue_backward(self._h, int(flags)))

    def dp_apply(self):
        self._chk(self._lib.dsact_dp_enqueue_apply(self._h))

    @staticmethod
    def _rccl_path():
        import torch

        p = os.path.join(os.path.dirname(torch.__file__), "lib", "librccl.so")
        return p.encode() if os.path.exists(p) else None

    def comm_unique_id(self) -> bytes:
        buf = (C.c_uint8 * 128)()
        rc = self._lib.dsact_comm_unique_id(self._rccl_path(), buf)
        if rc != 0:
            raise DsactError("dsact_comm_unique_id failed (%s)" % _ffi.E_NAMES.get(rc, rc))
        return bytes(buf)

    def comm_init(self, rank: int, world: int, unique_id: bytes):
        assert len(unique_id) == 128
        buf = (C.c_uint8 * 128)(*unique_id)
        self._chk(self._lib.dsact_comm_init(self._h, int(rank), int(world), buf, self._rccl_path()))
        self.comm_world = int(world)

    def comm_destroy(self):
        self._chk(self._lib.dsact_comm_destroy(self._h))

    def dp_allreduce(self):
        self._chk(self._lib.dsact_dp_enqueue_allreduce(self._h))

    STATS_SLOTS = 16

    def stats_snapshot(self, slot: int):
        self._chk(self._lib.dsact_stats_snapshot(self._h, int(slot) % self.STATS_SLOTS))

    def read_stats(self, slot=None) -> Dict[str, float]:
        out = (C.c_float * 16)()
        if slot is None:
            self._chk(self._lib.dsact_read_stats(self._h, out))
        else:
            self._chk(self._lib.dsact_stats_read(self._h, int(slot) % self.STATS_SLOTS, out))
        d = {k: float(out[i]) for i, k in enumerate(STAT_KEYS)}
        d["_iteration"] = float(out[14])
        d["_device_ms"] = float(out[15]) if slot is None else -1.0
        return d

    def time_steps(self, first_iteration: int, n_steps: int, use_graph: bool = True, flags: int = 0) -> float:
        ms = C.c_float()
        self.stage_serial += 1
        self._chk(self._lib.dsact_time_steps(self._h, int(first_iteration), int(n_steps), int(flags),
                                             1 if use_graph else 0, C.byref(ms)))
        return float(ms.value)

    def time_stage(self, stage: int, reps: int = 200):
        ms, macs = C.c_float(), C.c_double()
        self._chk(self._lib.dsact_time_stage(self._h, int(stage), int(reps), C.byref(ms), C.byref(macs)))
        return float(ms.value), float(macs.value)

    @property
    def chain_active(self) -> bool:
        return bool(self._lib.dsact_chain_active(self._h))

    def profile_step(self, iteration: int, flags: int = 0):
        arr = (_ffi.KernelTime * 128)()
        n = C.c_int32()
        self.stage_serial += 1
        self._chk(self._lib.dsact_profile_step(self._h, int(iteration), int(flags), arr, 128, C.byref(n)))
        return [(arr[i].name.decode(), float(arr[i].ms), int(arr[i].blocks)) for i in range(n.value)]

    def profile_steps(self, first_iteration: int, n_steps: int, flags: int = 0):
        arr = (_ffi.KernelTime * 512)()
        n = C.c_int32()
        self.stage_serial += 1
        self._chk(self._lib.dsact_profile_steps(self._h, int(first_iteration), int(n_steps), int(flags), arr, 512, C.byref(n)))
        return [(arr[i].name.decode(), float(arr[i].ms), int(arr[i].blocks)) for i in range(n.value)]

    def debug_read(self, name: str, cap: int = 1 << 24) -> np.ndarray:
        buf = np.empty(cap, np.float32)
        n = C.c_size_t()
        self._chk(self._lib.dsact_debug_read(self._h, name.encode(), _ffi.fptr(buf), cap, C.byref(n)))
        return buf[: n.value].copy()

    def debug_set(self, name: str, value: float):
        self._chk(self._lib.dsact_debug_set(self._h, name.encode(), float(value)))
        if name in ("withhold_flag", "fwd_merge"):
            self._graph_steps = 0

    def debug_get(self, name: str) -> float:
        v = C.c_double()
        self._chk(self._lib.dsact_debug_get(self._h, name.encode(), C.byref(v)))
        return float(v.value)

    def policy_dirty(self):
        self._chk(self._lib.dsact_debug_set(self._h, b"policy_dirty", 1.0))

    def note_torch_writes(self, params):
        v = sum(p._version for p in params) + self.online._version
        if v != getattr(self, "_param_versions", None):
            self._param_versions = v
            self.policy_dirty()

    def act_sample(self, obs, eps):
        if getattr(self, "_act_out", None) is None:
            self._act_out = np.empty(self.act_dim, np.float32)
            self._act_lp = np.empty(1, np.float32)
            self._act_out_p, self._act_lp_p = _ffi.fptr(self._act_out), _ffi.fptr(self._act_lp)
        rc = self._lib.dsact_act_sample(self._h, obs.ctypes.data_as(_ffi._FP), eps.ctypes.data_as(_ffi._FP),
                                        self._act_out_p, self._act_lp_p)
        if rc != 0:
            self._chk(rc)
        return self._act_out, self._act_lp

    def _addr_fn(self, attr: str, symbol: str, argtypes):
        f = self._lib[symbol]
        f.restype, f.argtypes = C.c_int, argtypes
        setattr(self, attr, f)
        return f

    def act_sample_addr(self, obs_addr: int, eps_addr: int, act_addr: int, logp_addr: int):
        f = getattr(self, "_act_addr_fn", None) or self._addr_fn("_act_addr_fn", "dsact_act_sample", [C.c_void_p] * 5)
        rc = f(self._h, obs_addr, eps_addr, act_addr, logp_addr)
        if rc != 0:
            self._chk(rc)

    def act_sample_batch(self, obs, eps):
        torch = self.torch
        n = int(np.prod(np.shape(obs))) // self.obs_dim
        srcs = [self._src(obs, n * self.obs_dim), self._src(eps, n * self.act_dim)]
        if any(isinstance(k, torch.Tensor) for _, k in srcs):
            torch.cuda.current_stream(self.device).synchronize()
        act = np.empty((n, self.act_dim), np.float32)
        lp = np.empty(n, np.float32)
        self._chk(self._lib.dsact_act_sample_batch(self._h, srcs[0][0], n, srcs[1][0], _ffi.fptr(act), _ffi.fptr(lp)))
        return act, lp

    def act_sample_batch_addr(self, obs_addr: int, n: int, eps_addr: int, act_addr: int, logp_addr: int):
        f = getattr(self, "_act_batch_addr_fn", None) or self._addr_fn(
            "_act_batch_addr_fn", "dsact_act_sample_batch", [C.c_void_p, C.c_void_p, C.c_int32, C.c_void_p, C.c_void_p, C.c_void_p])
        rc = f(self._h, obs_addr, n, eps_addr, act_addr, logp_addr)
        if rc != 0:
            self._chk(rc)

    def act_mode_batch(self, obs) -> np.ndarray:
        torch = self.torch
        n = int(np.prod(np.shape(obs))) // self.obs_dim
        if self.conv_type and isinstance(obs, torch.Tensor):
            obs = obs.detach().cpu()
        src = self._src(obs, n * self.obs_dim)
        if isinstance(src[1], torch.Tensor):
            torch.cuda.current_stream(self.device).synchronize()
        act = np.empty((n, self.act_dim), np.float32)
        self._chk(self._lib.dsact_act_mode_batch(self._h, src[0], n, _ffi.fptr(act)))
        return act

    def act_mode_batch_addr(self, obs_addr: int, n: int, act_addr: int):
        f = getattr(self, "_act_mode_addr_fn", None) or self._addr_fn(
            "_act_mode_addr_fn", "dsact_act_mode_batch", [C.c_void_p, C.c_void_p, C.c_int32, C.c_void_p])
        rc = f(self._h, obs_addr, n, act_addr)
        if rc != 0:
            self._chk(rc)

    @staticmethod
    def _rows(t) -> int:
        return int(t.shape[0]) if hasattr(t, "shape") and len(t.shape) else 0

    def _dev(self, t, shape, dtypes, name):
        torch = self.torch
        if not isinstance(t, torch.Tensor) or not t.is_cuda or t.device.index != self.device_index:
            raise ValueError("%s must be a torch tensor on %s (got %s)" % (name, self.device, getattr(t, "device", type(t).__name__)))
        if t.dtype not in dtypes:
            raise ValueError("%s must have dtype %s (got %s)" % (name, " or ".join(str(d) for d in dtypes), t.dtype))
        if not t.is_contiguous():
            raise ValueError("%s must be contiguous" % name)
        if tuple(t.shape) != tuple(shape):
            raise ValueError("%s must have shape %r (got %r)" % (name, tuple(shape), tuple(t.shape)))
        return t.data_ptr()

# ... 123 lines not shown
```

Before: 18740.

## Add warm-replay pipe graphs that skip the head gather across consecutive launches

Each pipelined graph phase is now captured twice. The warm variant omits the head gather and relies on the previous launch's tail to have prefetched the next group's gathers (lookahead ride extends past the end). Host-side bookkeeping (epoch, graph id, expected iteration) decides whether a launch can use the warm graph, and nearly every API entry point or parameter write invalidates it. This removes the serialized gather at the start of each graph replay in steady-state timing loops, at the cost of doubled graph capture memory and a risk of stale-state bugs if an invalidation path is missed.

```diff
diff --git a/dsac-v2_amd/csrc/dsact_api.hip b/dsac-v2_amd/csrc/dsact_api.hip
--- a/dsac-v2_amd/csrc/dsact_api.hip
+++ b/dsac-v2_amd/csrc/dsact_api.hip
@@ -300,6 +300,10 @@
     hipGraph_t pgraph[kPipePhases] = {nullptr, nullptr, nullptr, nullptr};
     hipGraphExec_t pexec[kPipePhases] = {nullptr, nullptr, nullptr, nullptr};
     PipeFwd* pargs[kPipePhases] = {nullptr, nullptr, nullptr, nullptr};
+    hipGraph_t wgraph[kPipePhases] = {nullptr, nullptr, nullptr, nullptr};
+    hipGraphExec_t wexec[kPipePhases] = {nullptr, nullptr, nullptr, nullptr};
+    bool tail = false;
+    unsigned long long id = 0;
     bool pipe = false;
     bool merged = false;
     bool noise_table = false;
@@ -308,6 +312,16 @@
   };
   GraphSet active;
   std::vector<GraphSet> graph_cache;
+  struct WarmRec {
+    long long it = -1;
+    unsigned long long graph = 0;
+    unsigned long long epoch = 0;
+    bool drawn = false;
+  } warm;
+  unsigned long long warm_epoch = 1, graph_serial = 0;
+  bool env_no_warm = false;
+  unsigned long long warm_replays = 0, cold_replays = 0;
+  int last_replay_warm = 0;
   bool env_no_pipe_defer = false;
   std::string env_pipe_map;
   void* comm = nullptr;
@@ -2701,17 +2715,22 @@
   return launch(h, "adam_polyak", k_adam, dim3(blocks), dim3(kThreads), 0, a);
 }
 
+static void warm_clear(dsact_handle* h) { h->warm_epoch++; }
+
 static void destroy_graph_set(dsact_handle::GraphSet& g) {
   if (g.exec) hipGraphExecDestroy(g.exec);
   if (g.graph) hipGraphDestroy(g.graph);
   for (int p = 0; p < dsact_handle::kPipePhases; ++p) {
     if (g.pexec[p]) hipGraphExecDestroy(g.pexec[p]);
     if (g.pgraph[p]) hipGraphDestroy(g.pgraph[p]);
+    if (g.wexec[p]) hipGraphExecDestroy(g.wexec[p]);
+    if (g.wgraph[p]) hipGraphDestroy(g.wgraph[p]);
     if (g.pargs[p]) hipFree(g.pargs[p]);
   }
   g = dsact_handle::GraphSet();
 }
 static void stash_graph(dsact_handle* h) {
+  warm_clear(h);
   if (!h->active.present()) return;
   h->graph_cache.push_back(h->active);
   h->active = dsact_handle::GraphSet();
@@ -2726,8 +2745,9 @@
   }
   return false;
 }
-static void drop_active_graph(dsact_handle* h) { destroy_graph_set(h->active); }
+static void drop_active_graph(dsact_handle* h) { warm_clear(h); destroy_graph_set(h->active); }
 void drop_graphs(dsact_handle* h) {
+  warm_clear(h);
   destroy_graph_set(h->active);
   for (auto& g : h->graph_cache) destroy_graph_set(g);
   h->graph_cache.clear();
@@ -2740,6 +2760,7 @@
   volatile int* const w_act = w_upd ? w_upd + 1 : nullptr;
   if (!h->handoff_host || h->in_handoff || !(*w_upd | *w_act)) return DSACT_OK;
   h->in_handoff = true;
+  warm_clear(h);
   const hipError_t e_dev = hipSetDevice(h->device);
   const hipError_t e_sync = hipStreamSynchronize(h->stream);
   const int upd = *w_upd;
@@ -2969,6 +2990,7 @@
   if (const char* v = getenv("DSACT_TIMELINE_STAGE")) h->env_timeline_stage = v;
   { int v = 0; if (hipDeviceGetAttribute(&v, hipDeviceAttributeMultiprocessorCount, h->device) == hipSuccess && v > 0) h->n_cu = v; (void)hipGetLastError(); }
   h->env_no_pipe_defer = getenv("DSACT_NO_PIPE_DEFER") != nullptr;
+  h->env_no_warm = getenv("DSACT_NO_WARM_REPLAY") != nullptr;
   h->env_no_bqt = getenv("DSACT_NO_BQT_MERGE") != nullptr;
   h->env_no_bqp = getenv("DSACT_NO_BQP_MERGE") != nullptr;
   if (const char* v = getenv("DSACT_PIPE_MAP")) h->env_pipe_map = v;
@@ -3217,6 +3239,7 @@
 }
 
 int dsact_set_stream(dsact_handle* h, void* s) {
+  if (h) warm_clear(h);
   if (!h) return DSACT_E_INVALID;
   HIPCHK(h, hipSetDevice(h->device));
   if (any_graph(h)) return fail(h, DSACT_E_STATE, "cannot change stream after dsact_graph_build");
@@ -3242,6 +3265,7 @@
 size_t dsact_pi_count(const dsact_handle* h) { return h ? h->n_pi : 0; }
 
 int dsact_bind_arenas(dsact_handle* h, float* online, float* target, float* adam_m, float* adam_v, float* grads) {
+  if (h) warm_clear(h);
   if (!h) return DSACT_E_INVALID;
   if (!online || !target || !adam_m || !adam_v || !grads) return fail(h, DSACT_E_INVALID, "null arena pointer");
   HIPCHK(h, hipSetDevice(h->device));
@@ -3266,6 +3290,7 @@
 }
 
 int dsact_set_action_limits(dsact_handle* h, const float* high, const float* low) {
+  if (h) warm_clear(h);
   if (!h || !high || !low) return DSACT_E_INVALID;
   HIPCHK(h, hipSetDevice(h->device));
   std::vector<float> s(h->A), c(h->A);
@@ -3301,6 +3326,7 @@
 }
 
 int dsact_set_state(dsact_handle* h, const int32_t adam_steps[3], const float mean_std[2]) {
+  if (h) warm_clear(h);
   if (!h) return DSACT_E_INVALID;
   HIPCHK(h, hipSetDevice(h->device));
   HIPCHK(h, hipStreamSynchronize(h->stream));
@@ -3323,6 +3349,7 @@
 }
 
 int dsact_set_hyper(dsact_handle* h, int32_t which, double value) {
+  if (h) warm_clear(h);
   if (!h) return DSACT_E_INVALID;
   if (!(value == value)) return fail(h, DSACT_E_INVALID, "hyper-parameter is NaN");
   switch (which) {
@@ -3369,6 +3396,7 @@
 }
 
 int dsact_buffer_create(dsact_handle* h, int64_t capacity) {
+  if (h) warm_clear(h);
   if (!h || capacity < 1) return DSACT_E_INVALID;
   if (capacity > 2147483647LL) return fail(h, DSACT_E_INVALID, "capacity must fit int32 (device indices)");
   HIPCHK(h, hipSetDevice(h->device));
@@ -3382,6 +3410,7 @@
 }
 
 int dsact_buffer_create_coded(dsact_handle* h, int64_t capacity, const float* codebook, int32_t n_codes) {
+  if (h) warm_clear(h);
   if (!h || capacity < 1 || !codebook) return DSACT_E_INVALID;
   if (capacity > 2147483647LL) return fail(h, DSACT_E_INVALID, "capacity must fit int32 (device indices)");
   if (n_codes < 1 || n_codes > 256) return fail(h, DSACT_E_INVALID, "hip_obs_codebook: %d entries (1 .. 256)", (int)n_codes);
@@ -3451,6 +3480,7 @@
 
 int dsact_buffer_add(dsact_handle* h, int64_t n, const float* obs, const float* act, const float* rew,
                      const float* obs2, const float* done, const float* logp) {
+  if (h) warm_clear(h);
   if (!h || n < 0 || !obs || !act || !rew || !obs2 || !done) return DSACT_E_INVALID;
   if (!has_ring(h)) return fail(h, DSACT_E_STATE, "buffer not created");
   TRY(check_codes(h));
@@ -3514,6 +3544,7 @@
 
 int dsact_buffer_fill_device(dsact_handle* h, int64_t row0, int64_t n, const float* obs, const float* act,
                              const float* rew, const float* obs2, const float* done) {
+  if (h) warm_clear(h);
   if (!h || row0 < 0 || n < 0) return DSACT_E_INVALID;
   if (!has_ring(h)) return fail(h, DSACT_E_STATE, "buffer not created");
   if (row0 + n > h->cap) return fail(h, DSACT_E_INVALID, "fill exceeds capacity");
@@ -3549,6 +3580,7 @@
 
 int dsact_buffer_add_device(dsact_handle* h, int64_t n, const float* obs, const float* act, const float* rew, const float* obs2,
                             const uint8_t* terminated, const uint8_t* truncated, const float* logp, double reward_scale) {
+  if (h) warm_clear(h);
   if (!h || n < 0 || !obs || !act || !rew || !obs2 || !terminated || !truncated || !logp) return DSACT_E_INVALID;
   if (!has_ring(h)) return fail(h, DSACT_E_STATE, "buffer not created");
   if (h->rb_code) return fail(h, DSACT_E_INVALID, "dsact_buffer_add_device serves the fp32 MLP ring (coded rings: dsact_buffer_add)");
@@ -3626,6 +3658,7 @@
 
 int dsact_buffer_import(dsact_handle* h, int64_t row0, int64_t n, const void* obs, const void* obs2, const float* act,
                         const float* rew, const float* done, const float* logp) {
+  if (h) warm_clear(h);
   if (!h) return DSACT_E_INVALID;
   TRY(ring_entry(h, "dsact_buffer_import"));
   if (!obs || !obs2 || !act || !rew || !done || !logp) return fail(h, DSACT_E_INVALID, "dsact_buffer_import: a source column is NULL");
@@ -3652,6 +3685,7 @@
 }
 
 int dsact_buffer_set_cursor(dsact_handle* h, int64_t size, int64_t ptr) {
+  if (h) warm_clear(h);
   if (!h) return DSACT_E_INVALID;
   TRY(ring_entry(h, "dsact_buffer_set_cursor"));
   const bool ok = size >= 0 && size <= h->cap && (size < h->cap ? ptr == size % h->cap : (ptr >= 0 && ptr < h->cap));
@@ -3703,6 +3737,7 @@
 }
 
 int dsact_gather(dsact_handle* h, const int64_t* idx_host, int32_t batch) {
+  if (h) warm_clear(h);
   if (!h) return DSACT_E_INVALID;
   if (!has_ring(h)) return fail(h, DSACT_E_STATE, "buffer not created");
   TRY(check_codes(h));
@@ -3780,6 +3815,7 @@
 }
 
 int dsact_load_batch(dsact_handle* h, const float* obs, const float* act, const float* rew, const float* obs2, const float* done) {
+  if (h) warm_clear(h);
   if (!h || !obs || !act || !rew || !obs2 || !done) return DSACT_E_INVALID;
   HIPCHK(h, hipSetDevice(h->device));
   const size_t B = h->B, O = h->O, A = h->A, ld = h->ldx;
@@ -3810,6 +3846,7 @@
 }
 
 int dsact_upload_index_table(dsact_handle* h, const int64_t* idx_host, int32_t rows) {
+  if (h) warm_clear(h);
   if (!h || !idx_host || rows < 1) return DSACT_E_INVALID;
   if (!has_ring(h)) return fail(h, DSACT_E_STATE, "buffer not created");
   HIPCHK(h, hipSetDevice(h->device));
@@ -3833,6 +3870,7 @@
 }
 
 int dsact_set_noise(dsact_handle* h, const float* eps_new, const float* eps_2, const float* z5, const float* z6) {
+  if (h) warm_clear(h);
   if (!h || !eps_new || !eps_2 || !z5 || !z6) return DSACT_E_INVALID;
   HIPCHK(h, hipSetDevice(h->device));
   const size_t B = h->B, A = h->A;
@@ -3846,6 +3884,7 @@
 }
 
 int dsact_set_device_rng(dsact_handle* h, uint64_t seed) {
+  if (h) warm_clear(h);
   if (!h) return DSACT_E_INVALID;
   if (any_graph(h)) return fail(h, DSACT_E_STATE, "rng mode is baked into the captured graph");
   h->rng_seed = seed;
@@ -3853,12 +3892,14 @@
 }
 
 int dsact_set_index_rng(dsact_handle* h, uint64_t seed) {
+  if (h) warm_clear(h);
   if (!h) return DSACT_E_INVALID;
   h->idx_seed = seed;
   return DSACT_OK;
 }
 
 int dsact_draw_indices(dsact_handle* h, int64_t first_iteration, int32_t n) {
+  if (h) warm_clear(h);
   if (!h || n < 1) return DSACT_E_INVALID;
   if (!has_ring(h)) return fail(h, DSACT_E_STATE, "buffer not created");
   if (h->idx_seed == 0) return fail(h, DSACT_E_STATE, "no index seed (dsact_set_index_rng)");
@@ -3991,6 +4032,7 @@
 }
 
 int dsact_compute_grads(dsact_handle* h, int64_t iteration, uint32_t flags) {
+  if (h) warm_clear(h);
   TRY(check_ready(h, true));
   HIPCHK(h, hipSetDevice(h->device));
   TRY(mark_update(h, false));
@@ -4000,6 +4042,7 @@
 }
 
 int dsact_apply_update(dsact_handle* h, int64_t iteration) {
+  if (h) warm_clear(h);
   TRY(check_ready(h, false));
   HIPCHK(h, hipSetDevice(h->device));
   TRY(enqueue_prologue(h, 0, iteration, 1, 0));
@@ -4008,6 +4051,7 @@
 }
 
 int dsact_step(dsact_handle* h, int64_t iteration, uint32_t flags) {
+  if (h) warm_clear(h);
   TRY(check_ready(h, true));
   HIPCHK(h, hipSetDevice(h->device));
   TRY(mark_update(h, false));
@@ -4092,6 +4136,7 @@
   bool dp = false;
   bool skip = false;
   std::vector<char> leaves;
+  bool tail = false;
 };
 static int plan_updates_pipe(dsact_handle* h, int n, int phase, PipePlan& plan, PipeFwd* dev_args, uint32_t flags = 0) {
   const int D = h->cfg.delay_update;
@@ -4102,6 +4147,7 @@
   const bool can_defer = h->pi_merge && h->dw_chunks == 1 && !h->fat_bwd && rg_pi <= 2 && !h->env_no_pipe_defer;
   plan.dp = (flags & DSACT_F_DATA_PARALLEL) != 0;
   plan.skip = (flags & DSACT_F_SKIP_ACTOR_ON_OFF_ITERS) != 0 && !plan.dp;
+  plan.tail = !plan.dp && n >= dsact_handle::kPipeSets && n % dsact_handle::kPipeSets == 0;
   plan.leaves.assign((size_t)n, 0);
   const bool bqt = bqt_ok(h);
   const bool bqp = bqt && h->nq == 2 && !h->env_no_bqp && chain_rg(h, 4, true) == 1 && rg_pi == 2;
@@ -4135,13 +4181,13 @@
   HIPCHK(h, hipMemcpy(dev_args, plan.host.data(), (size_t)n * sizeof(PipeFwd), hipMemcpyHostToDevice));
   return DSACT_OK;
 }
-static int enqueue_updates_pipe(dsact_handle* h, int n, const PipePlan& plan, PipeFwd* dev_args) {
+static int enqueue_updates_pipe(dsact_handle* h, int n, const PipePlan& plan, PipeFwd* dev_args, bool head = true) {
   auto set_of = [&](int s) { return dsact_handle::pipe_set((s - (n - 1)) & (dsact_handle::kPipeSets - 1)); };
   const std::vector<PipeFwd>& host = plan.host;
   const std::vector<char>&pre_v = plan.pre, &do_v = plan.dop;
   int rc = DSACT_OK;
   h->mirror_w0 = true;
-  {
+  if (head) {
     Gather2Args g;
     select_set(h, set_of(0));
     g.a = gather_args(h, h->idx_table, h->idx_rows, 1, 0, 1);
@@ -4165,7 +4211,7 @@
     if (rc != DSACT_OK) break;
     RideArgs ride;
     memset(&ride, 0, sizeof(ride));
-    if (s + 2 < n) {
+    if (s + 2 < n || plan.tail) {
       select_set(h, set_of(s + 2));
       ride.g = gather_args(h, h->idx_table, h->idx_rows, 1, 0, 1);
       ride.g.lookahead = 2;
@@ -4191,16 +4237,20 @@
   return rc;
 }
 
-static int capture_updates_pipe(dsact_handle* h, int n, int phase, hipGraph_t* graph, hipGraphExec_t* exec, PipeFwd** dev_args, uint32_t flags) {
-  HIPCHK(h, hipMalloc((void**)dev_args, (size_t)n * sizeof(PipeFwd)));
+static int capture_updates_pipe(dsact_handle* h, int n, int ph, dsact_handle::GraphSet& g, uint32_t flags) {
+  HIPCHK(h, hipMalloc((void**)&g.pargs[ph], (size_t)n * sizeof(PipeFwd)));
   PipePlan plan;
-  TRY(plan_updates_pipe(h, n, phase, plan, *dev_args, flags));
-  HIPCHK(h, hipStreamBeginCapture(h->stream, hipStreamCaptureModeThreadLocal));
-  const int rc = enqueue_updates_pipe(h, n, plan, *dev_args);
-  hipError_t e = hipStreamEndCapture(h->stream, graph);
-  if (rc != DSACT_OK) return rc;
-  if (e != hipSuccess) return fail(h, DSACT_E_HIP, "hipStreamEndCapture: %s", hipGetErrorString(e));
-  HIPCHK(h, hipGraphInstantiate(exec, *graph, nullptr, nullptr, 0));
+  TRY(plan_updates_pipe(h, n, ph, plan, g.pargs[ph], flags));
+  for (int warm = 0; warm < (plan.tail ? 2 : 1); ++warm) {
+    hipGraph_t* graph = warm ? &g.wgraph[ph] : &g.pgraph[ph];
+    HIPCHK(h, hipStreamBeginCapture(h->stream, hipStreamCaptureModeThreadLocal));
+    const int rc = enqueue_updates_pipe(h, n, plan, g.pargs[ph], !warm);
+    hipError_t e = hipStreamEndCapture(h->stream, graph);
+    if (rc != DSACT_OK) return rc;
+    if (e != hipSuccess) return fail(h, DSACT_E_HIP, "hipStreamEndCapture: %s", hipGetErrorString(e));
+    HIPCHK(h, hipGraphInstantiate(warm ? &g.wexec[ph] : &g.pexec[ph], *graph, nullptr, nullptr, 0));
+  }
+  g.tail = plan.tail;
   return DSACT_OK;
 }
 
@@ -4238,7 +4288,7 @@
   int rc = DSACT_OK;
   if (pipe) {
     rc = alloc_pipe_sets(h);
-    for (int ph = 0; ph < D && rc == DSACT_OK; ++ph) rc = capture_updates_pipe(h, steps_per_graph, ph, &g.pgraph[ph], &g.pexec[ph], &g.pargs[ph], flags);
+    for (int ph = 0; ph < D && rc == DSACT_OK; ++ph) rc = capture_updates_pipe(h, steps_per_graph, ph, g, flags);
     g.pipe = rc == DSACT_OK;
     if (rc != DSACT_OK) {
       drop_active_graph(h);
@@ -4256,24 +4306,36 @@
   g.merged = merged; g.noise_table = noise_table;
   g.steps = steps_per_graph;
   g.flags = flags;
+  g.id = ++h->graph_serial;
   h->have_batch = true;
   return DSACT_OK;
 }
 
 int dsact_graph_build(dsact_handle* h, int32_t steps_per_graph, uint32_t flags) { return build_graph(h, steps_per_graph, flags, false, false); }
 
-static int launch_groups(dsact_handle* h, int64_t first_iteration, int64_t n_groups) {
+static int launch_groups(dsact_handle* h, int64_t first_iteration, int64_t n_groups, bool drawn = false, bool need_drawn = false) {
   h->uev_valid = false;
   int64_t i = 0;
   const dsact_handle::GraphSet& g = h->active;
   if (g.pipe) {
     const int D = h->cfg.delay_update;
     for (; i < n_groups; ++i) {
-      const int ph = (int)(((first_iteration + i * g.steps) % D + D) % D);
-      HIPCHK(h, hipGraphLaunch(g.pexec[ph], h->stream));
+      const long long it = first_iteration + i * g.steps;
+      const int ph = (int)((it % D + D) % D);
+      const dsact_handle::WarmRec& w = h->warm;
+      const bool warm = g.tail && !h->env_no_warm && w.graph == g.id && w.epoch == h->warm_epoch && w.it == it &&
+                        (i > 0 || h->dev_it_next == first_iteration) && (!need_drawn || w.drawn);
+      const hipError_t e = hipGraphLaunch(warm ? g.wexec[ph] : g.pexec[ph], h->stream);
+      if (e != hipSuccess) { warm_clear(h); HIPCHK(h, e); }
+      if (g.tail) {
+        h->warm.it = it + g.steps; h->warm.graph = g.id; h->warm.epoch = h->warm_epoch; h->warm.drawn = drawn;
+        (warm ? h->warm_replays : h->cold_replays)++;
+      }
+      h->last_replay_warm = warm ? 1 : 0;
     }
     return DSACT_OK;
   }
+  h->last_replay_warm = 0;
   for (; i < n_groups; ++i) HIPCHK(h, hipGraphLaunch(g.exec, h->stream));
   return DSACT_OK;
 }
@@ -4315,7 +4377,8 @@
   const size_t n_idx = (size_t)n_steps * B, nz_row = 2 * B * A + 2 * B;
   for (size_t i = 0; idx && i < n_idx; ++i)
     if (idx[i] < 0 || idx[i] >= h->size) return fail(h, DSACT_E_INVALID, "index %lld out of range [0,%lld)", (long long)idx[i], h->size);
-  TRY(ensure_group_tables(h, n_steps));
+  TRY(ensure_group_tables(h, n_steps + (idx ? 0 : 2)));
+  if (idx || noise) warm_clear(h);
   if (noise && !h->noise_table) {
     HIPCHK(h, hipMalloc(&h->noise_table, (size_t)h->idx_rows * nz_row * sizeof(float)));
     HIPCHK(h, hipMemset(h->noise_table, 0, (size_t)h->idx_rows * nz_row * sizeof(float)));
@@ -4328,7 +4391,7 @@
   }
   const size_t idx_bytes = idx ? n_idx * sizeof(int) : 0;
   const size_t need = idx_bytes + (noise ? (size_t)n_steps * nz_row * sizeof(float) : 0);
-  if (!idx) TRY(enqueue_draw_indices(h, first_iteration, n_steps));
+  if (!idx) TRY(enqueue_draw_indices(h, first_iteration, n_steps + 2));
   if (need) {
     if (need > h->grp_pin_bytes) {
       HIPCHK(h, hipStreamSynchronize(h->stream));
@@ -4356,19 +4419,23 @@
   }
   hipLaunchKernelGGL(k_set_counters, dim3(1), dim3(64), 0, h->stream, h->st, (long long)first_iteration, 0LL);
   if (hipGetLastError() != hipSuccess) return fail(h, DSACT_E_HIP, "launch k_set_counters failed");
-  TRY(launch_groups(h, first_iteration, 1));
+  h->dev_it_next = first_iteration;
+  TRY(launch_groups(h, first_iteration, 1, !idx, true));
+  if (idx || noise) warm_clear(h);
   h->dev_it_next = first_iteration + n_steps;
   h->have_batch = true;
   return policy_moved(h);
 }
 
 int dsact_dp_begin(dsact_handle* h, int64_t first_iteration) {
+  if (h) warm_clear(h);
   if (!h) return DSACT_E_INVALID;
   HIPCHK(h, hipSetDevice(h->device));
   return set_device_iteration(h, first_iteration);
 }
 
 int dsact_dp_enqueue_grads(dsact_handle* h, uint32_t flags) {
+  if (h) warm_clear(h);
   TRY(check_ready(h, false));
   if (!h->idx_table) return fail(h, DSACT_E_STATE, "upload an index table first");
   HIPCHK(h, hipSetDevice(h->device));
@@ -4379,6 +4446,7 @@
 }
 
 int dsact_dp_enqueue_grads_critic(dsact_handle* h, uint32_t flags) {
+  if (h) warm_clear(h);
   TRY(check_ready(h, false));
   if (!h->idx_table) return fail(h, DSACT_E_STATE, "upload an index table first");
   if (h->use_std_sums) return fail(h, DSACT_E_STATE, "the split gradient halves are for the one-collective mode (strict mode has its own halves)");
@@ -4390,6 +4458,7 @@
 }
 
 int dsact_dp_enqueue_grads_actor(dsact_handle* h, uint32_t flags) {
+  if (h) warm_clear(h);
   TRY(check_ready(h, true));
   HIPCHK(h, hipSetDevice(h->device));
   (void)flags;
@@ -4397,6 +4466,7 @@
 }
 
 int dsact_dp_set_strict(dsact_handle* h, float* std_sums_dev) {
+  if (h) warm_clear(h);
   if (!h) return DSACT_E_INVALID;
   HIPCHK(h, hipSetDevice(h->device));
   HIPCHK(h, hipStreamSynchronize(h->stream));
@@ -4408,6 +4478,7 @@
 }
 
 int dsact_dp_enqueue_forward(dsact_handle* h, uint32_t flags) {
+  if (h) warm_clear(h);
   TRY(check_ready(h, false));
   if (!h->idx_table) return fail(h, DSACT_E_STATE, "upload an index table first");
   if (!h->use_std_sums) return fail(h, DSACT_E_STATE, "dsact_dp_set_strict first");
@@ -4419,6 +4490,7 @@
 }
 
 int dsact_dp_enqueue_backward(dsact_handle* h, uint32_t flags) {
+  if (h) warm_clear(h);
   TRY(check_ready(h, true));
   if (!h->use_std_sums) return fail(h, DSACT_E_STATE, "dsact_dp_set_strict first");
   HIPCHK(h, hipSetDevice(h->device));
@@ -4427,6 +4499,7 @@
 }
 
 int dsact_dp_enqueue_apply(dsact_handle* h) {
+  if (h) warm_clear(h);
   TRY(check_ready(h, false));
   HIPCHK(h, hipSetDevice(h->device));
   TRY(enqueue_prologue(h, 1, 0, 1, 0));
@@ -4445,6 +4518,7 @@
 }
 
 int dsact_comm_init(dsact_handle* h, int32_t rank, int32_t world, const uint8_t id[128], const char* rccl_path) {
+  if (h) warm_clear(h);
   if (!h || !id || world < 1 || rank < 0 || rank >= world) return DSACT_E_INVALID;
   HIPCHK(h, hipSetDevice(h->device));
   if (any_graph(h)) return fail(h, DSACT_E_STATE, "the communicator is baked into the captured graph");
@@ -4459,6 +4533,7 @@
 }
 
 int dsact_comm_destroy(dsact_handle* h) {
+  if (h) warm_clear(h);
   if (!h) return DSACT_E_INVALID;
   if (h->comm) {
     hipSetDevice(h->device);
@@ -4470,6 +4545,7 @@
 }
 
 int dsact_dp_enqueue_allreduce(dsact_handle* h) {
+  if (h) warm_clear(h);
   TRY(check_ready(h, false));
   HIPCHK(h, hipSetDevice(h->device));
   return enqueue_allreduce(h, h->grads, h->n_online + 2, kNcclAvg);
@@ -4544,6 +4620,7 @@
     h->dev_it_next = first_iteration + n_steps;
   } else {
     h->dev_it_next = -1;
+    warm_clear(h);
     for (int64_t i = 0; i < n_steps; ++i) TRY(enqueue_graph_step(h, first_iteration + i, flags));
   }
   HIPCHK(h, hipEventRecord(h->tev1, h->stream));
@@ -4562,6 +4639,7 @@
 }
 
 int dsact_time_stage(dsact_handle* h, int32_t stage, int32_t reps, float* ms_total, double* macs) {
+  if (h) warm_clear(h);
   if (!h || !ms_total || reps < 1) return DSACT_E_INVALID;
   TRY(check_ready(h, false));
   const int L = h->L;
@@ -4592,6 +4670,7 @@
 }
 
 int dsact_profile_step(dsact_handle* h, int64_t iteration, uint32_t flags, dsact_kernel_time* out, int32_t cap, int32_t* n) {
+  if (h) warm_clear(h);
   if (!h || !out || !n) return DSACT_E_INVALID;
   h->pol_epoch++;
   TRY(check_ready(h, false));
@@ -4621,6 +4700,7 @@
 }
 
 int dsact_profile_steps(dsact_handle* h, int64_t first_iteration, int32_t n_steps, uint32_t flags, dsact_kernel_time* out, int32_t cap, int32_t* n) {
+  if (h) warm_clear(h);
   if (!h || !out || !n || n_steps < 1) return DSACT_E_INVALID;
   h->pol_epoch++;
   TRY(check_ready(h, false));
@@ -4758,6 +4838,8 @@
 int dsact_debug_set(dsact_handle* h, const char* name, double value) {
   if (!h || !name) return DSACT_E_INVALID;
   HIPCHK(h, hipSetDevice(h->device));
+  if (strcmp(name, "mode_host_rows") && strcmp(name, "beh_live_copy")) warm_clear(h);
+  if (!strcmp(name, "params_dirty")) return DSACT_OK;
   if (!strcmp(name, "withhold_flag")) {
     HIPCHK(h, hipStreamSynchronize(h->stream));
     drop_graphs(h);
@@ -4870,6 +4952,11 @@
   else if (!strcmp(name, "track_commit_calls")) *value = (double)h->track_commit_calls;
   else if (!strcmp(name, "track_reads")) *value = (double)h->track_reads;
   else if (!strcmp(name, "act_fast")) *value = act_fast_ok(h) ? 1.0 : 0.0;
+  else if (!strcmp(name, "warm_replays")) *value = (double)h->warm_replays;
+  else if (!strcmp(name, "cold_replays")) *value = (double)h->cold_replays;
+  else if (!strcmp(name, "last_replay_warm")) *value = (double)h->last_replay_warm;
+  else if (!strcmp(name, "warm_tail")) *value = h->active.tail ? 1.0 : 0.0;
+  else if (!strcmp(name, "warm_valid")) *value = (h->active.tail && h->warm.graph == h->active.id && h->warm.epoch == h->warm_epoch) ? 1.0 : 0.0;
   else if (!strcmp(name, "graph_cache")) *value = (double)h->graph_cache.size();
   else if (!strcmp(name, "graph_noise_table")) *value = h->active.noise_table ? 1.0 : 0.0;
   else if (!strcmp(name, "twin_par")) *value = (h->twin_par ? 1.0 : 0.0) + (h->twin_merged ? 2.0 : 0.0);
diff --git a/dsac-v2_amd/dsac_v2_hip.py b/dsac-v2_amd/dsac_v2_hip.py
--- a/dsac-v2_amd/dsac_v2_hip.py
+++ b/dsac-v2_amd/dsac_v2_hip.py
@@ -351,6 +351,7 @@
                 child.register_forward_pre_hook(lambda _m, _a, _e=engine: _e.sync())
                 child._dsact_sync_hook = True
         engine.set_action_limits(self.policy.act_high_lim.cpu().numpy(), self.policy.act_low_lim.cpu().numpy())
+        engine.watch_params([slot[0] for slot in self._named_param_slots()])
 
     def _apply(self, fn, *a, **k):
         if self._engine is not None:
@@ -367,6 +368,7 @@
             self._engine.set_action_limits(self.policy.act_high_lim.cpu().numpy(),
                                            self.policy.act_low_lim.cpu().numpy())
             self._engine.policy_dirty()
+            self._engine.params_dirty()
         return out
 
     def state_dict(self, *a, **k):
diff --git a/dsac-v2_amd/dsact/dp.py b/dsac-v2_amd/dsact/dp.py
--- a/dsac-v2_amd/dsact/dp.py
+++ b/dsac-v2_amd/dsact/dp.py
@@ -36,6 +36,8 @@
                 dist.broadcast(t, src=0, group=group)
         if hasattr(engine, "policy_dirty"):
             engine.policy_dirty()
+        if hasattr(engine, "params_dirty"):
+            engine.params_dirty()
 
     def _on_engine_stream(self):
         ts = getattr(self.engine, "torch_stream", None)
diff --git a/dsac-v2_amd/dsact/engine.py b/dsac-v2_amd/dsact/engine.py
--- a/dsac-v2_amd/dsact/engine.py
+++ b/dsac-v2_amd/dsact/engine.py
@@ -1,4 +1,5 @@
 import ctypes as C
+import operator
 import os
 from typing import Dict, List, Optional, Sequence
 
@@ -16,6 +17,9 @@
     "DSAC2/policy_mean-RL iter", "DSAC2/policy_std-RL iter", "DSAC2/entropy-RL iter",
     "DSAC2/alpha-RL iter", "DSAC2/mean_std1", "DSAC2/mean_std2",
 ]
+
+
+_VERSION = operator.attrgetter("_version")
 
 
 def _f32(a):
@@ -182,6 +186,8 @@
         self.rows_added = 0
         self.fill_epoch = 0
         self.index_seed = 0
+        self._watched = [self.online, self.target]
+        self._arena_versions = None
 
     def _chk(self, rc):
         if rc != 0:
@@ -410,6 +416,7 @@
 
     def graph_run(self, first_iteration: int, n_steps: int):
         self.stage_serial += 1
+        self._note_arena_writes()
         self._chk(self._lib.dsact_graph_run(self._h, int(first_iteration), int(n_steps)))
 
     def run_group(self, first_iteration: int, idx_rows, noise_rows=None, flags: int = 0, n: int = None):
@@ -427,6 +434,7 @@
             nz = _f32(noise_rows)
             assert nz.shape == (n, 2 * self.batch * self.act_dim + 2 * self.batch), nz.shape
         self.stage_serial += 1
+        self._note_arena_writes()
         self._chk(self._lib.dsact_run_group(self._h, int(first_iteration), n, idx_ptr, _ffi.fptr(nz), int(flags)))
         self._graph_steps = n
 
@@ -511,6 +519,7 @@
     def time_steps(self, first_iteration: int, n_steps: int, use_graph: bool = True, flags: int = 0) -> float:
         ms = C.c_float()
         self.stage_serial += 1
+        self._note_arena_writes()
         self._chk(self._lib.dsact_time_steps(self._h, int(first_iteration), int(n_steps), int(flags),
                                              1 if use_graph else 0, C.byref(ms)))
         return float(ms.value)
@@ -556,6 +565,19 @@
 
     def policy_dirty(self):
         self._chk(self._lib.dsact_debug_set(self._h, b"policy_dirty", 1.0))
+
+    def params_dirty(self):
+        self._chk(self._lib.dsact_debug_set(self._h, b"params_dirty", 1.0))
+
+    def watch_params(self, params):
+        self._watched = [self.online, self.target] + list(params)
+        self._arena_versions = None
+
+    def _note_arena_writes(self):
+        v = sum(map(_VERSION, self._watched))
+        if v != self._arena_versions:
+            self._arena_versions = v
+            self.params_dirty()
 
     def note_torch_writes(self, params):
         v = sum(p._version for p in params) + self.online._version
```

Measured after the change: 18840 (median of 6 runs). About the same (+0.5%).
